# robustrobotics/flame

Hardware: AMD Instinct MI355X
Metric: NLTGV2 primal-dual iters/sec on 640x480 Delaunay graph; depth RMS vs CPU (higher is better)
Workload: dtype f32

## Files before the change

flame_amd/csrc/flame_nltgv2_test_options.h:

```cpp
#ifndef FLAME_NLTGV2_TEST_OPTIONS_H_
#define FLAME_NLTGV2_TEST_OPTIONS_H_

enum {
  FLAME_NLTGV2_OPT_BLOCK_WAVES = 103,
  FLAME_NLTGV2_OPT_UNROLL = 104,
  FLAME_NLTGV2_OPT_DUAL_PUBLISH = 106,
  FLAME_NLTGV2_OPT_PRESLEEP = 108,
  FLAME_NLTGV2_OPT_XCDS = 109,
  FLAME_NLTGV2_OPT_FAULT_INJECT = 110,
  FLAME_NLTGV2_OPT_POLL_GAP = 113
};

#endif
```

flame_amd/csrc/nltgv2_context.hip:

```cpp
#include "nltgv2_context.hpp"

namespace flame_hip {
namespace host {

int fail(flame_nltgv2_ctx* ctx, int status) {
  if (ctx) ctx->last_error = status;
  return status;
}

void request_open_stop(flame_nltgv2_ctx* ctx) {
  if (!ctx->open_inflight || ctx->open_stop_sent || !ctx->stop_dev.p || !ctx->ctl_stream) return;
  *ctx->h_stop = ctx->open_tag0;
  if (hipMemcpyAsync(ctx->stop_dev.p, ctx->h_stop, sizeof(unsigned), hipMemcpyHostToDevice, ctx->ctl_stream) != hipSuccess) (void)hipGetLastError();
  ctx->open_stop_sent = true;
}

hipError_t wait_solver_stream(flame_nltgv2_ctx* ctx) {
  request_open_stop(ctx);
  return hipStreamSynchronize(ctx->stream);
}

int ensure(flame_nltgv2_ctx* ctx, DevBuf& b, size_t bytes) {
  if (bytes == 0) bytes = 16;
  if (b.cap >= bytes) return 0;
// ... 31 lines not shown
  HIPCHK(ctx, hipSetDevice(ctx->device));
  ++ctx->call_seq;
  return 0;
}

void refresh_args(flame_nltgv2_ctx* ctx) {
  CanonArgs& c = ctx->c;
  c.V = ctx->L.V, c.E = ctx->L.E;
  c.pos = (float2*)ctx->pos.p;
  c.x = (float*)ctx->x.p, c.w1 = (float*)ctx->w1.p, c.w2 = (float*)ctx->w2.p;
  c.xb = (float*)ctx->xb.p, c.w1b = (float*)ctx->w1b.p, c.w2b = (float*)ctx->w2b.p;
  c.xp = (float*)ctx->xp.p, c.w1p = (float*)ctx->w1p.p, c.w2p = (float*)ctx->w2p.p;
  c.data = (float*)ctx->data.p, c.weight = (float*)ctx->weight.p;
  c.src = (int32_t*)ctx->src.p, c.dst = (int32_t*)ctx->dst.p;
  c.alpha = (float*)ctx->alpha.p, c.beta = (float*)ctx->beta.p;
  c.q1 = (float*)ctx->q1.p, c.q2 = (float*)ctx->q2.p, c.q3 = (float*)ctx->q3.p;
  c.row_ptr = (int32_t*)ctx->row_ptr.p, c.half = (uint32_t*)ctx->half.p;
  c.err = (int*)ctx->err.p;
  FusedArgs& f = ctx->f;
  f.n_slices = ctx->L.n_slices;
  f.n_slots = (ctx->L.rows + kRowPad) * kWave;
  f.slice_row = (int32_t*)ctx->slice_row.p, f.perm = (int32_t*)ctx->perm.p, f.pdeg = (int32_t*)ctx->pdeg.p;
  f.rec_nbr = (uint32_t*)ctx->rec_nbr.p, f.rec_edge = (int32_t*)ctx->rec_edge.p;
  f.edge_src_slot = (int32_t*)ctx->edge_src_slot.p;
  f.hrec = (int4*)ctx->hrec.p, f.hq = (float4*)ctx->hq.p;
  f.vstate = (float4*)ctx->vstate.p, f.vaux = (float2*)ctx->vaux.p;
  f.hq_out = (float4*)ctx->hq_alt.p, f.vstate_out = (float4*)ctx->vstate_alt.p;
  f.bar[0] = (float4*)ctx->bar0.p, f.bar[1] = (float4*)ctx->bar1.p;
  f.vprev = (float4*)ctx->vprev.p;
  f.xbuf = ctx->xbuf.p;
  f.tv_waves = (ctx->tv_built && ctx->L.tv_ok) ? ctx->L.tv_waves : 0;
  f.tv_slot = (int32_t*)ctx->tv_slot.p, f.tv_vid = (int32_t*)ctx->tv_vid.p;
  f.tv_meta = (uint32_t*)ctx->tv_meta.p, f.tv_wave = (uint32_t*)ctx->tv_wave.p;
  f.wg_count = ctx->L.wg_ok ? ctx->L.wg_count : 0;
  f.n_rec = ctx->L.n_rec;
  f.wg_lcap = ctx->L.wg_lcap, f.wg_slab_slots = ctx->L.wg_slab_slots;
  f.wg_rowpack = ctx->L.wg_rowpack ? 1 : 0;
  f.wg_slot = (int32_t*)ctx->wg_slot.p, f.wg_vid = (int32_t*)ctx->wg_vid.p, f.wg_meta = (uint32_t*)ctx->wg_meta.p;
  f.wg_nbr = (int32_t*)ctx->wg_nbr.p, f.wg_fetch = (int32_t*)ctx->wg_fetch.p, f.wg_info = (int32_t*)ctx->wg_info.p;
  f.abort_flag = (int*)ctx->abort_flag.p;
  f.err = (int*)ctx->err.p;
}

int h2d(flame_nltgv2_ctx* ctx, DevBuf& b, const void* src, size_t bytes) {
  if (bytes == 0) return 0;
  HIPCHK(ctx, hipMemcpyAsync(b.p, src, bytes, hipMemcpyHostToDevice, ctx->stream));
  return 0;
}

size_t records_capacity(const PackedLayout& L) {
  const size_t n_packed = (size_t)L.n_slices * kWave, n_rec = ((size_t)L.n_rec + kWave - 1) / kWave * kWave;
  return std::max(n_packed, n_rec);
}

int wait_raster(flame_nltgv2_ctx* ctx) {
  if (ctx->raster_inflight) {
    HIPCHK(ctx, hipStreamWaitEvent(ctx->stream, ctx->ev_raster_done, 0));
    ctx->raster_inflight = false;
  }
  return 0;
}

int ensure_canon(flame_nltgv2_ctx* ctx, const std::function<int()>* behind, int* behind_state) {
  bool unpacked = false, launched = false;
  if (behind_state) *behind_state = kBehindNotLaunched;
  if (ctx->pending.active) {
    const int rc = finish(ctx, true, &unpacked, behind, &launched);
    if (behind_state && launched) *behind_state = unpacked ? kBehindDone : kBehindSpoiled;
    if (rc) {
      if (unpacked) ctx->canon_valid = true;
      return rc;
    }
  }
  int rc0 = wait_raster(ctx);
  if (rc0) return rc0;
  if (ctx->canon_valid) return 0;
  if (!unpacked) LAUNCHCHK(ctx, launch_unpack_state(ctx->c, ctx->f, ctx->parity, ctx->have_prev, ctx->stream));
  ctx->canon_valid = true;
  return 0;
}

int ensure_fused(flame_nltgv2_ctx* ctx) {
  if (ctx->fused_valid) return 0;
  LAUNCHCHK(ctx, launch_pack_state(ctx->c, ctx->f, ctx->parity, ctx->static_stale, ctx->stream));
  ctx->static_stale = false;
  ctx->fused_valid = true;
  ctx->have_prev = false;
  return 0;
}


int staged_h2d(flame_nltgv2_ctx* ctx, const StageCopy* cp, size_t n, const StageFill* fills, size_t n_fills, int slot, hipStream_t stream,
               size_t* host_off) {
  if (!stream) stream = ctx->stream;
  flame_nltgv2_ctx::StageSlot& st = ctx->stage[slot];
  size_t total = 0;
  for (size_t i = 0; i < n; ++i) total += (cp[i].bytes + 255) & ~size_t(255);
  if (total >= (size_t)0xffffff00u) return fail(ctx, FLAME_NLTGV2_ERR_INVALID_ARG);
  if (total > st.cap) {
    request_open_stop(ctx);
    if (st.h) (void)hipHostFree(st.h);
    st.h = nullptr, st.cap = 0;
    const size_t want = total + total / 2;
    if (hipHostMalloc(&st.h, want, hipHostMallocDefault) != hipSuccess) {
      (void)hipGetLastError();
      return fail(ctx, FLAME_NLTGV2_ERR_OOM);
    }
    st.cap = want;
  }
  int rc = ensure(ctx, st.d, st.cap);
  if (rc) return rc;
  std::vector<ScatterTable> tables(1);
  auto push = [&](const ScatterEntry& e) {
    if (tables.back().n == kScatterMax) tables.emplace_back();
    ScatterTable& t = tables.back();
    t.e[t.n++] = e;
  };
  size_t off = 0;
  for (size_t i = 0; i < n; ++i) {
    if (host_off) host_off[i] = off;
    if (cp[i].bytes == 0) continue;
    std::memcpy(static_cast<char*>(st.h) + off, cp[i].src, cp[i].bytes);
    push(ScatterEntry{cp[i].b->p, (uint32_t)off, 0u, cp[i].bytes});
    off += (cp[i].bytes + 255) & ~size_t(255);
  }
  for (size_t i = 0; i < n_fills; ++i)
    if (fills[i].bytes) push(ScatterEntry{fills[i].dst, kScatterFill, fills[i].word, fills[i].bytes});
  if (off) HIPCHK(ctx, hipMemcpyAsync(st.d.p, st.h, off, hipMemcpyHostToDevice, stream));
  for (const ScatterTable& t : tables) LAUNCHCHK(ctx, launch_scatter(t, st.d.p, stream));
  return 0;
}

int topology_buffers(flame_nltgv2_ctx* ctx, bool want_e2, size_t n_wg_info, size_t n_wg_v0, size_t n_wg_vfirst, size_t n_wg2_info,
                     size_t n_wg2_vfirst) {
  const PackedLayout& L = ctx->L;
  const int32_t V = L.V, E = L.E;
  const size_t n_slots = (size_t)(L.rows + kRowPad) * kWave;
  if (n_slots > (size_t)0x7fffffff) return fail(ctx, FLAME_NLTGV2_ERR_INVALID_ARG);
  const size_t n_packed = (size_t)L.n_slices * kWave;
  const size_t lanes = (size_t)L.wg_count * kWave;
  const size_t fV = sizeof(float) * (size_t)V, fE = sizeof(float) * (size_t)E, iV = sizeof(int32_t) * (size_t)V;
  struct { DevBuf* b; size_t bytes; } req[] = {
      {&ctx->pos, 2 * fV}, {&ctx->src, fE}, {&ctx->dst, fE},
      {&ctx->row_ptr, sizeof(int32_t) * ((size_t)V + 1)}, {&ctx->half, 2 * fE},
      {&ctx->slice_row, sizeof(int32_t) * ((size_t)L.n_slices + 1)}, {&ctx->perm, sizeof(int32_t) * n_packed},
      {&ctx->pdeg, sizeof(int32_t) * n_packed}, {&ctx->iperm, iV}, {&ctx->order_m, iV}, {&ctx->rid_of, iV},
      {&ctx->rec_nbr, sizeof(uint32_t) * n_slots}, {&ctx->rec_edge, sizeof(int32_t) * n_slots}, {&ctx->edge_src_slot, fE},
      {&ctx->hrec, sizeof(int4) * n_slots}, {&ctx->hq, sizeof(float4) * n_slots},
      {&ctx->vstate, sizeof(float4) * n_packed}, {&ctx->vaux, sizeof(float2) * n_packed},
      {&ctx->hq_alt, sizeof(float4) * n_slots}, {&ctx->vstate_alt, sizeof(float4) * n_packed}, {&ctx->photo_err, fV},
      {&ctx->bar0, sizeof(float4) * n_packed}, {&ctx->bar1, sizeof(float4) * n_packed},
      {&ctx->vprev, sizeof(float4) * n_packed}, {&ctx->xbuf, kXbufBytesPerVertex * records_capacity(L) + 64},
      {&ctx->wg_v0, sizeof(int32_t) * n_wg_v0},
      {&ctx->wg_vfirst, n_wg_vfirst + 16}, {&ctx->abort_flag, sizeof(int)}, {&ctx->err, kErrBytes}, {&ctx->cost_out, 2 * sizeof(float)},
      {&ctx->wg_slot, sizeof(int32_t) * lanes}, {&ctx->wg_vid, sizeof(int32_t) * lanes}, {&ctx->wg_meta, sizeof(uint32_t) * lanes},
      {&ctx->wg_nbr, sizeof(int32_t) * lanes}, {&ctx->wg_fetch, sizeof(int32_t) * lanes},
      {&ctx->wg_info, sizeof(int32_t) * n_wg_info}};
  for (auto& r : req) {
    const int rc = ensure(ctx, *r.b, r.bytes);
    if (rc) return rc;
  }
  if (want_e2) {
    const size_t lanes2 = (size_t)L.wg2_count * kWave;
    struct { DevBuf* b; size_t bytes; } req2[] = {
        {&ctx->wg2_info, sizeof(int32_t) * n_wg2_info}, {&ctx->wg2_vfirst, n_wg2_vfirst + 16}, {&ctx->wg2_rmax, 64},
        {&ctx->wg2_slot, sizeof(int32_t) * 2 * lanes2}, {&ctx->wg2_nbr, sizeof(int32_t) * 2 * lanes2}, {&ctx->wg2_vid, sizeof(int32_t) * lanes2},
        {&ctx->wg2_meta, sizeof(uint32_t) * lanes2}, {&ctx->wg2_fetch, sizeof(int32_t) * lanes2}};
    for (auto& r : req2) {
      const int rc = ensure(ctx, *r.b, r.bytes);
      if (rc) return rc;
    }
  }
  ctx->topo++;
  ctx->layout_pos_saved = false;
  ctx->tv_built = ctx->wg2_built = false;
  drop_graphs(ctx);
  refresh_args(ctx);
  return 0;
}

void expansion_fills(const PackedLayout& L, void* rec_edge, void* rec_nbr, void* wg2_rmax, std::vector<StageFill>* fills) {
  fills->push_back(StageFill{(char*)rec_edge + sizeof(int32_t) * (size_t)L.rows * kWave, sizeof(int32_t) * kRowPad * kWave, 0xffffffffu});
  fills->push_back(StageFill{(char*)rec_nbr + sizeof(uint32_t) * (size_t)L.rows * kWave, sizeof(uint32_t) * kRowPad * kWave, 0u});
  if (wg2_rmax) fills->push_back(StageFill{wg2_rmax, 64, 0u});
}

void topology_fills(flame_nltgv2_ctx* ctx, bool want_e2, std::vector<StageFill>* fills, bool early) {
  const PackedLayout& L = ctx->L;
  const size_t n_slots = (size_t)(L.rows + kRowPad) * kWave, n_packed = (size_t)L.n_slices * kWave;
  const StageFill base[] = {
      {ctx->err.p, kErrBytes, 0u}, {ctx->abort_flag.p, sizeof(int), 0u}, {ctx->xbuf.p, kXbufBytesPerVertex * records_capacity(L) + 64, 0u},
      {ctx->hq_alt.p, sizeof(float4) * n_slots, 0u}, {ctx->vstate_alt.p, sizeof(float4) * n_packed, 0u}};
  fills->insert(fills->end(), base, base + sizeof(base) / sizeof(base[0]));
  if (!early) expansion_fills(L, ctx->rec_edge.p, ctx->rec_nbr.p, want_e2 ? ctx->wg2_rmax.p : nullptr, fills);
  if (ctx->place_base) {
    fills->push_back(StageFill{ctx->place_base, (size_t)2 * kPlacePages * 4096, 0u});
    fills->push_back(StageFill{(int*)ctx->place_fill.p + 2 * kPlacePages, 64, 0u});
  }
}

bool placement_applies(const flame_nltgv2_ctx* ctx, const PackedLayout& L) {
  return L.wg_ok && ctx->place_state == 1 && ctx->opt_place && L.wg_count > 2 * (ctx->prop.multiProcessorCount / 8) &&
         (ctx->opt_xcds == 0 || ctx->opt_xcds == 8);
}

ExpandTables live_tables(flame_nltgv2_ctx* ctx) {
  ExpandTables t;
  t.c = ctx->c, t.f = ctx->f;
  t.iperm = (const int32_t*)ctx->iperm.p, t.wg_v0 = (const int32_t*)ctx->wg_v0.p, t.order_m = (const int32_t*)ctx->order_m.p;
  t.rid_of = (const int32_t*)ctx->rid_of.p, t.wg_vfirst = (const uint8_t*)ctx->wg_vfirst.p;
  t.wg2_info = (int32_t*)ctx->wg2_info.p, t.wg2_vfirst = (const uint8_t*)ctx->wg2_vfirst.p;
  t.wg2_slot = (int32_t*)ctx->wg2_slot.p, t.wg2_vid = (int32_t*)ctx->wg2_vid.p, t.wg2_nbr = (int32_t*)ctx->wg2_nbr.p;
  t.wg2_fetch = (int32_t*)ctx->wg2_fetch.p, t.wg2_meta = (uint32_t*)ctx->wg2_meta.p, t.wg2_rmax = (int*)ctx->wg2_rmax.p;
  return t;
}

int expand_launches(flame_nltgv2_ctx* ctx, const PackedLayout& L, const ExpandTables& t, bool want_e2, hipStream_t stream) {
  LAUNCHCHK(ctx, launch_build_sell(t.c, t.f, t.iperm, stream));
  if (L.wg_ok) LAUNCHCHK(ctx, launch_build_patches(t.c, t.f, t.wg_v0, t.order_m, t.rid_of, t.wg_vfirst, t.iperm, stream));
  if (want_e2)
    LAUNCHCHK(ctx, launch_build_patches2(t.c, t.f, L.wg2_count, t.wg2_info, t.order_m, t.rid_of, t.wg2_vfirst, t.iperm, t.wg2_slot, t.wg2_vid,
                                         t.wg2_meta, t.wg2_nbr, t.wg2_fetch, t.wg2_rmax, stream));
  if (t.rec_off)
    LAUNCHCHK(ctx, launch_place_records(t.c, t.f, t.per_xcd, t.order_m, t.rid_of, t.place_patch, (int8_t*)(t.place_patch + t.stride),
                                        (const uint16_t*)ctx->place_rank.p, kPlacePages, t.place_fill, t.rec_off, (int)t.stride, stream));
  return 0;
}

int topology_expand(flame_nltgv2_ctx* ctx, bool want_e2, bool launched) {
  const PackedLayout& L = ctx->L;
  if (!launched) {
    const int rc = expand_launches(ctx, L, live_tables(ctx), want_e2, ctx->stream);
    if (rc) return rc;
  }
  ctx->pv2_args = Pv2Args{};
  ctx->wg2_usable = false;
  if (want_e2) {
    ctx->pv2_args.slot = (const int32_t*)ctx->wg2_slot.p, ctx->pv2_args.vid = (const int32_t*)ctx->wg2_vid.p;
    ctx->pv2_args.meta = (const uint32_t*)ctx->wg2_meta.p, ctx->pv2_args.nbr = (const int32_t*)ctx->wg2_nbr.p;
    ctx->pv2_args.fetch = (const int32_t*)ctx->wg2_fetch.p, ctx->pv2_args.info = (const int32_t*)ctx->wg2_info.p;
    ctx->pv2_args.count = L.wg2_count, ctx->pv2_args.lcap = L.wg2_lcap;
    if (ctx->pv2_occ == 0 || ctx->pv2_occ_lcap != L.wg2_lcap)
      ctx->pv2_occ = pv2_patches_per_cu(L.wg2_lcap, false), ctx->pv2_occ_verify = pv2_patches_per_cu(L.wg2_lcap, true), ctx->pv2_occ_lcap = L.wg2_lcap;
    ctx->wg2_built = true;
  }
  if (!launched && placement_applies(ctx, L)) {
    refresh_args(ctx);
    const int rc = place_records(ctx, (L.wg_count + 7) / 8);
    if (rc) return rc;
  }
  ctx->pending = flame_nltgv2_ctx::PendingRun{};
  ctx->tag_next = 1;
  ctx->xbuf_form = 0;
  ctx->static_stale = false;
  return 0;
}

bool wants_e2(const flame_nltgv2_ctx* ctx) { return wants_e2(ctx, ctx->L); }
bool wants_e2(const flame_nltgv2_ctx* ctx, const PackedLayout& L) {
  const int cus = ctx->prop.multiProcessorCount;
  const int64_t est_patches = L.wg_rowpack ? (int64_t)L.wg_count : ((static_cast<int64_t>(2) * L.E + L.V / 32) / 54 + 1);
  return L.wg_ok && L.max_degree <= 32 && ctx->opt_probe == 0 &&
         (ctx->opt_persistent == 6 || (ctx->opt_persistent == 1 && est_patches > (int64_t)kPv2FromPerCu * cus));
}

int upload_topology(flame_nltgv2_ctx* ctx, const flame_nltgv2_graph* g, const StageCopy* extra, size_t n_extra, bool long_lived) {
  const int32_t V = g->V, E = g->E;
  (void)long_lived;
  int rc = cancel_prepared(ctx);
  if (!rc) rc = wait_raster(ctx);
  if (rc) return rc;
  rc = build_layout(g, &ctx->L, false, true,
                        ctx->opt_persistent == 4 ? 0x7fffffff : kPvDensePerCu * ctx->prop.multiProcessorCount);
  if (rc) return fail(ctx, rc);
  if (ctx->L.wg_ok && ctx->L.wg_rowpack && ctx->opt_persistent != 4 && ctx->L.wg_count > kPvDensePerCu * ctx->prop.multiProcessorCount) {
    rc = build_layout(g, &ctx->L, false, false, 0);
    if (rc) return fail(ctx, rc);
  }
  bool want_e2 = wants_e2(ctx);
  if (want_e2) {
    build_patch_walk2(&ctx->L);
    want_e2 = ctx->L.wg2_ok && ctx->L.wg2_count <= kPv2WavesPerCu * ctx->prop.multiProcessorCount * 4;
  }
  const PackedLayout& L = ctx->L;
  rc = topology_buffers(ctx, want_e2, L.wg_info.size(), L.wg_v0.size(), L.wg_vfirst.size(), L.wg2_info.size(), L.wg2_vfirst.size());
  if (rc) return rc;
  const size_t n_packed = (size_t)L.n_slices * kWave;
  const size_t fV = sizeof(float) * (size_t)V, fE = sizeof(float) * (size_t)E, iV = sizeof(int32_t) * (size_t)V;
  std::vector<StageCopy> cp = {
      {&ctx->pos, g->pos, 2 * fV}, {&ctx->src, g->src, fE}, {&ctx->dst, g->dst, fE},
      {&ctx->row_ptr, L.row_ptr.data(), sizeof(int32_t) * ((size_t)V + 1)}, {&ctx->half, L.half.data(), 2 * fE},
      {&ctx->slice_row, L.slice_row.data(), sizeof(int32_t) * ((size_t)L.n_slices + 1)},
      {&ctx->perm, L.perm.data(), sizeof(int32_t) * n_packed}, {&ctx->pdeg, L.pdeg.data(), sizeof(int32_t) * n_packed},
      {&ctx->iperm, L.iperm.data(), iV}, {&ctx->order_m, L.order_m.data(), iV}, {&ctx->rid_of, L.rid_of.data(), iV},
      {&ctx->wg_info, L.wg_info.data(), sizeof(int32_t) * L.wg_info.size()},
      {&ctx->wg_v0, L.wg_v0.data(), sizeof(int32_t) * L.wg_v0.size()},
      {&ctx->wg_vfirst, L.wg_vfirst.data(), L.wg_vfirst.size()}};
  if (want_e2) {
    cp.push_back(StageCopy{&ctx->wg2_info, L.wg2_info.data(), sizeof(int32_t) * L.wg2_info.size()});
    cp.push_back(StageCopy{&ctx->wg2_vfirst, L.wg2_vfirst.data(), L.wg2_vfirst.size()});
  }
  cp.insert(cp.end(), extra, extra + n_extra);
  std::vector<StageFill> fills;
  topology_fills(ctx, want_e2, &fills);
  rc = staged_h2d(ctx, cp.data(), cp.size(), fills.data(), fills.size());
  if (rc) return rc;
  rc = topology_expand(ctx, want_e2);
  if (rc) return rc;
  ctx->h_src.assign(g->src, g->src + E);
  ctx->h_dst.assign(g->dst, g->dst + E);
  ctx->host_layout_valid = true;
  ctx->feat_dev_valid = false;
  HIPCHK(ctx, hipEventRecord(ctx->ev_topo_ready, ctx->stream));
  return 0;
}

int ensure_form_rows(flame_nltgv2_ctx* ctx, int form) {
  PackedLayout& L = ctx->L;
  if ((form == 4 && !ctx->wg2_built) || (form == 2 && !ctx->tv_built)) {
    const int rc = ensure_host_layout(ctx);
    if (rc) return rc;
  }
  if (form == 4 && !ctx->wg2_built) {
    build_patch_rows2(&L);
    ctx->pv2_args = Pv2Args{};
    if (L.wg2_ok) {
      struct { DevBuf* b; const void* src; size_t bytes; } cp[] = {
          {&ctx->wg2_slot, L.wg2_slot.data(), sizeof(int32_t) * L.wg2_slot.size()}, {&ctx->wg2_vid, L.wg2_vid.data(), sizeof(int32_t) * L.wg2_vid.size()},
          {&ctx->wg2_meta, L.wg2_meta.data(), sizeof(uint32_t) * L.wg2_meta.size()}, {&ctx->wg2_nbr, L.wg2_nbr.data(), sizeof(int32_t) * L.wg2_nbr.size()},
          {&ctx->wg2_fetch, L.wg2_fetch.data(), sizeof(int32_t) * L.wg2_fetch.size()}, {&ctx->wg2_info, L.wg2_info.data(), sizeof(int32_t) * L.wg2_info.size()}};
      HIPCHK(ctx, wait_solver_stream(ctx));
      for (auto& c : cp) {
        int rc = ensure(ctx, *c.b, c.bytes);
        if (!rc) rc = h2d(ctx, *c.b, c.src, c.bytes);
        if (rc) return rc;
      }
      HIPCHK(ctx, wait_solver_stream(ctx));
      ctx->pv2_args.slot = (const int32_t*)ctx->wg2_slot.p, ctx->pv2_args.vid = (const int32_t*)ctx->wg2_vid.p, ctx->pv2_args.meta = (const uint32_t*)ctx->wg2_meta.p;
      ctx->pv2_args.nbr = (const int32_t*)ctx->wg2_nbr.p, ctx->pv2_args.fetch = (const int32_t*)ctx->wg2_fetch.p, ctx->pv2_args.info = (const int32_t*)ctx->wg2_info.p;
      ctx->pv2_args.count = L.wg2_count, ctx->pv2_args.lcap = L.wg2_lcap;
      ctx->pv2_occ = pv2_patches_per_cu(L.wg2_lcap, false), ctx->pv2_occ_verify = pv2_patches_per_cu(L.wg2_lcap, true), ctx->pv2_occ_lcap = L.wg2_lcap;
    }
    ctx->wg2_built = true;
    ctx->wg2_usable = L.wg2_ok, ctx->wg2_checked_topo = ctx->topo;
  }
  if (form == 2 && !ctx->tv_built) {
    build_tv_rows(&L);
    struct { DevBuf* b; const void* src; size_t bytes; } cp[] = {
        {&ctx->tv_slot, L.tv_slot.data(), sizeof(int32_t) * L.tv_slot.size()}, {&ctx->tv_vid, L.tv_vid.data(), sizeof(int32_t) * L.tv_vid.size()},
        {&ctx->tv_meta, L.tv_meta.data(), sizeof(uint32_t) * L.tv_meta.size()}, {&ctx->tv_wave, L.tv_wave.data(), sizeof(uint32_t) * L.tv_wave.size()}};
    HIPCHK(ctx, wait_solver_stream(ctx));
    for (auto& c : cp) {
      int rc = ensure(ctx, *c.b, c.bytes);
      if (!rc) rc = h2d(ctx, *c.b, c.src, c.bytes);
      if (rc) return rc;
    }
    HIPCHK(ctx, wait_solver_stream(ctx));
    ctx->tv_built = true;
    refresh_args(ctx);
  }
  return 0;
}

bool params_ok(const flame_nltgv2_params* p) { return p != nullptr; }

}
}

extern "C" {

int flame_nltgv2_abi_version(void) { return FLAME_NLTGV2_ABI_VERSION; }

void flame_nltgv2_default_params(flame_nltgv2_params* p) {
  if (!p) return;
  p->data_factor = 0.1f, p->step_x = 0.001f, p->step_q = 125.0f;
  p->theta = 0.25f, p->x_min = 0.0f, p->x_max = 10.0f;
}

const char* flame_nltgv2_status_string(int status) {
  switch (status) {
    case FLAME_NLTGV2_OK: return "ok";
    case FLAME_NLTGV2_ERR_INVALID_ARG: return "invalid argument";
    case FLAME_NLTGV2_ERR_NO_DEVICE: return "no usable HIP device";
    case FLAME_NLTGV2_ERR_HIP: return "HIP runtime error";
    case FLAME_NLTGV2_ERR_NO_GRAPH: return "no graph uploaded";
    case FLAME_NLTGV2_ERR_NAN: return "dual variable became NaN/Inf (reference FLAME_ASSERT, h:174)";
    case FLAME_NLTGV2_ERR_OOM: return "out of device memory";
    case FLAME_NLTGV2_ERR_TIMEOUT: return "persistent run: neighbour wait timed out";
    case FLAME_NLTGV2_ERR_ASSERT: return "input on which the reference asserts (FLAME_ASSERT)";
    default: return "unknown status";
  }
}

int flame_nltgv2_create(flame_nltgv2_ctx** out, int device) {
  if (!out) return FLAME_NLTGV2_ERR_INVALID_ARG;
  *out = nullptr;
  int count = 0;
  if (hipGetDeviceCount(&count) != hipSuccess || count <= 0) return FLAME_NLTGV2_ERR_NO_DEVICE;
  if (device < 0 || device >= count) return FLAME_NLTGV2_ERR_NO_DEVICE;
  flame_nltgv2_ctx* ctx = new (std::nothrow) flame_nltgv2_ctx();
  if (!ctx) return FLAME_NLTGV2_ERR_OOM;
  ctx->device = device;
  bool ok = hipSetDevice(device) == hipSuccess;
  ok = ok && hipGetDeviceProperties(&ctx->prop, device) == hipSuccess;
  int prio_least = 0, prio_greatest = 0;
  ok = ok && hipDeviceGetStreamPriorityRange(&prio_least, &prio_greatest) == hipSuccess;
  ok = ok && hipStreamCreateWithPriority(&ctx->own_stream, hipStreamNonBlocking, prio_greatest) == hipSuccess;
  ok = ok && hipEventCreate(&ctx->ev0) == hipSuccess && hipEventCreate(&ctx->ev1) == hipSuccess;
  ok = ok && hipStreamCreateWithFlags(&ctx->topo_stream, hipStreamNonBlocking) == hipSuccess;
  ok = ok && hipStreamCreateWithFlags(&ctx->raster_stream, hipStreamNonBlocking) == hipSuccess;
  ok = ok && hipEventCreateWithFlags(&ctx->ev_canon, hipEventDisableTiming) == hipSuccess;
  ok = ok && hipEventCreateWithFlags(&ctx->ev_snap, hipEventDisableTiming) == hipSuccess;
  ok = ok && hipEventCreateWithFlags(&ctx->ev_raster_done, hipEventDisableTiming) == hipSuccess;
  ok = ok && hipEventCreateWithFlags(&ctx->ev_topo_ready, hipEventDisableTiming) == hipSuccess;
  ok = ok && hipEventCreate(&ctx->ev_mesh0) == hipSuccess && hipEventCreate(&ctx->ev_mesh1) == hipSuccess;
  ok = ok && hipEventCreate(&ctx->ev_dbg0) == hipSuccess && hipEventCreate(&ctx->ev_dbg1) == hipSuccess;
  ok = ok && hipEventCreateWithFlags(&ctx->ev_expanded, hipEventDisableTiming) == hipSuccess;
  ok = ok && hipEventCreateWithFlags(&ctx->ev_run[0], hipEventDisableTiming) == hipSuccess;
  ok = ok && hipEventCreateWithFlags(&ctx->ev_run[1], hipEventDisableTiming) == hipSuccess;
  ok = ok && hipHostMalloc((void**)&ctx->h_err, kErrBytes, hipHostMallocDefault) == hipSuccess;
  ok = ok && hipHostMalloc((void**)&ctx->h_cost, 2 * sizeof(float), hipHostMallocDefault) == hipSuccess;
  ok = ok && hipHostMalloc((void**)&ctx->h_stop, 64, hipHostMallocDefault) == hipSuccess;
  if (ctx->h_stop) *ctx->h_stop = 0u;
  ok = ok && hipStreamCreateWithPriority(&ctx->ctl_stream, hipStreamNonBlocking, -1) == hipSuccess;
  if (!ok) {
    flame_nltgv2_destroy(ctx);
    return FLAME_NLTGV2_ERR_HIP;
  }
  ctx->stream = ctx->own_stream;
  *ctx->h_err = 0;
  {
    static std::once_flag warm;
    if (!std::getenv("FLAME_NLTGV2_NO_WARM"))
    std::call_once(warm, [ctx] {
      warm_module_kernels(), warm_module_persistent(ctx->own_stream, cooperative_allowed()), warm_module_persistent_tv(), warm_module_persistent_pv2();
      warm_module_layout(), warm_module_topo();
    });
    if (!std::getenv("FLAME_NLTGV2_LAZY_CALIBRATION") && ctx->prop.multiProcessorCount >= 64 && place_calibrate_at_create(device) && place_calibrate(ctx) != 0) {
      ctx->last_error = 0, ctx->last_hip = 0;
      (void)hipGetLastError();
    }
    if (ctx->place_state < 0) ctx->place_state = 0;
  }
  ctx->all = {&ctx->pos, &ctx->x, &ctx->w1, &ctx->w2, &ctx->xb, &ctx->w1b, &ctx->w2b, &ctx->xp, &ctx->w1p,
              &ctx->w2p, &ctx->data, &ctx->weight, &ctx->src, &ctx->dst, &ctx->alpha, &ctx->beta, &ctx->q1,
              &ctx->q2, &ctx->q3, &ctx->row_ptr, &ctx->half, &ctx->slice_row, &ctx->perm, &ctx->pdeg,
              &ctx->rec_nbr, &ctx->rec_edge, &ctx->edge_src_slot, &ctx->hrec, &ctx->hq, &ctx->vstate, &ctx->hq_alt, &ctx->vstate_alt, &ctx->cost_terms, &ctx->run_tail,
              &ctx->vaux, &ctx->bar0, &ctx->bar1, &ctx->vprev, &ctx->xbuf, &ctx->abort_flag, &ctx->tv_slot, &ctx->tv_vid, &ctx->tv_meta, &ctx->tv_wave, &ctx->wg2_slot, &ctx->wg2_vid, &ctx->wg2_meta, &ctx->wg2_nbr, &ctx->wg2_fetch, &ctx->wg2_info, &ctx->wg2_vfirst, &ctx->wg2_rmax, &ctx->err,
              &ctx->cost_out, &ctx->img_ref, &ctx->img_cmp, &ctx->photo_err, &ctx->r_tris, &ctx->r_valid, &ctx->r_tvalid, &ctx->r_keys,
              &ctx->r_img, &ctx->r_cov, &ctx->r_vtx, &ctx->r_val, &ctx->wg_slot, &ctx->wg_vid, &ctx->wg_meta, &ctx->wg_nbr,
              &ctx->wg_fetch, &ctx->wg_info, &ctx->wg_v0, &ctx->probe, &ctx->snap_hq, &ctx->snap_vstate, &ctx->snap_bar, &ctx->iperm,
              &ctx->order_m, &ctx->rid_of, &ctx->stage[0].d, &ctx->stage[1].d, &ctx->sync_init, &ctx->sync_vmap, &ctx->sync_emap, &ctx->sync_need,
              &ctx->wg_vfirst, &ctx->place_pool, &ctx->place_rank, &ctx->place_fill, &ctx->place_rec_off, &ctx->place_patch, &ctx->place_meas, &ctx->progress};
  for (DevBuf* b : {&ctx->feat_stamp_d, &ctx->feat_key_d, &ctx->feat_val_d, &ctx->topo_scratch, &ctx->topo_dims, &ctx->layout_pos}) ctx->all.push_back(b);
  for (auto& b : ctx->nx) ctx->all.push_back(&b);
  for (auto& b : ctx->ex) ctx->all.push_back(&b);
  ctx->all.push_back(&ctx->pos_undo);
  for (DevBuf* b : {&ctx->m_P, &ctx->m_idepth, &ctx->m_normals, &ctx->m_tvalid, &ctx->m_nvalid, &ctx->m_tnormal, &ctx->m_offset, &ctx->m_cursor,
                    &ctx->m_incident, &ctx->m_keys, &ctx->m_img, &ctx->m_cov})
    ctx->all.push_back(b);
  for (DevBuf* b : {&ctx->d_gray, &ctx->d_idimg, &ctx->d_nimg, &ctx->d_w1map, &ctx->d_w2map, &ctx->d_keys, &ctx->d_cov}) ctx->all.push_back(b);
  ctx->all.push_back(&ctx->stop_dev);
  ctx->all.push_back(&ctx->place_patch_nx), ctx->all.push_back(&ctx->place_fill_nx);
  for (auto& b : ctx->sp_v) ctx->all.push_back(&b);
  for (auto& b : ctx->sp_q) ctx->all.push_back(&b);
  for (auto& b : ctx->sp_ab) ctx->all.push_back(&b);
  *out = ctx;
  return FLAME_NLTGV2_OK;
}

int flame_nltgv2_destroy(flame_nltgv2_ctx* ctx) {
  if (!ctx) return FLAME_NLTGV2_OK;
  (void)hipSetDevice(ctx->device);
  request_open_stop(ctx);
  if (ctx->stream) (void)hipStreamSynchronize(ctx->stream);
  place_pool_release(ctx);
  drop_graphs(ctx);
  for (DevBuf* b : ctx->all)
    if (b->p) (void)hipFree(b->p);
  if (ctx->h_err) (void)hipHostFree(ctx->h_err);
  if (ctx->h_cost) (void)hipHostFree(ctx->h_cost);
  if (ctx->h_keep) (void)hipHostFree(ctx->h_keep);
  if (ctx->h_stop) (void)hipHostFree(ctx->h_stop);
  if (ctx->ctl_stream) (void)hipStreamSynchronize(ctx->ctl_stream), (void)hipStreamDestroy(ctx->ctl_stream);
  for (auto& st : ctx->stage)
    if (st.h) (void)hipHostFree(st.h);
  if (ctx->topo_stream) (void)hipStreamSynchronize(ctx->topo_stream), (void)hipStreamDestroy(ctx->topo_stream);
  if (ctx->ev_topo_ready) (void)hipEventDestroy(ctx->ev_topo_ready);
  if (ctx->ev_expanded) (void)hipEventDestroy(ctx->ev_expanded);
  if (ctx->raster_stream) (void)hipStreamSynchronize(ctx->raster_stream), (void)hipStreamDestroy(ctx->raster_stream);
  if (ctx->ev_canon) (void)hipEventDestroy(ctx->ev_canon);
  if (ctx->ev_snap) (void)hipEventDestroy(ctx->ev_snap);
  if (ctx->ev_raster_done) (void)hipEventDestroy(ctx->ev_raster_done);
  for (hipEvent_t e : ctx->ev_run)
    if (e) (void)hipEventDestroy(e);
  if (ctx->h_img) (void)hipHostFree(ctx->h_img);
  if (ctx->h_mesh) (void)hipHostFree(ctx->h_mesh);
  if (ctx->ev_mesh0) (void)hipEventDestroy(ctx->ev_mesh0);
  if (ctx->ev_mesh1) (void)hipEventDestroy(ctx->ev_mesh1);
  if (ctx->h_dbg) (void)hipHostFree(ctx->h_dbg);
  if (ctx->ev_dbg0) (void)hipEventDestroy(ctx->ev_dbg0);
  if (ctx->ev_dbg1) (void)hipEventDestroy(ctx->ev_dbg1);
  if (ctx->h_dims) (void)hipHostFree(ctx->h_dims);
  if (ctx->ev0) (void)hipEventDestroy(ctx->ev0);
  if (ctx->ev1) (void)hipEventDestroy(ctx->ev1);
  if (ctx->own_stream) (void)hipStreamDestroy(ctx->own_stream);
  delete ctx;
  return FLAME_NLTGV2_OK;
}

int flame_nltgv2_set_stream(flame_nltgv2_ctx* ctx, void* hip_stream) {
  int rc = enter(ctx);
  if (rc) return rc;
  HIPCHK(ctx, wait_solver_stream(ctx));
  ctx->stream = hip_stream ? (hipStream_t)hip_stream : ctx->own_stream;
  return FLAME_NLTGV2_OK;
}

int flame_nltgv2_set_option(flame_nltgv2_ctx* ctx, int option, int value) {
  if (!ctx) return FLAME_NLTGV2_ERR_INVALID_ARG;
  switch (option) {
    case FLAME_NLTGV2_OPT_SOLVER:
      if (value != 0 && value != 1) return fail(ctx, FLAME_NLTGV2_ERR_INVALID_ARG);
      ctx->opt_solver = value;
      return 0;
    case FLAME_NLTGV2_OPT_USE_HIPGRAPH:
      ctx->opt_use_graph = value ? 1 : 0;
      return 0;
    case FLAME_NLTGV2_OPT_BLOCK_WAVES:
      if (value != 0 && value != 1 && value != 2 && value != 4) return fail(ctx, FLAME_NLTGV2_ERR_INVALID_ARG);
      ctx->opt_block_waves = value;
      return 0;
    case FLAME_NLTGV2_OPT_PERSISTENT:
      if (value < 0 || value > 6 || value == 2 || value == 5) return fail(ctx, FLAME_NLTGV2_ERR_INVALID_ARG);
      ctx->opt_persistent = value;
      return 0;
    case FLAME_NLTGV2_OPT_PLACEMENT:
      if (value < 0 || value > 1) return fail(ctx, FLAME_NLTGV2_ERR_INVALID_ARG);
      ctx->opt_place = value;
      return 0;
    case FLAME_NLTGV2_OPT_POLL_GAP:
      if (value < 0 || value > 256) return fail(ctx, FLAME_NLTGV2_ERR_INVALID_ARG);
      ctx->opt_poll_gap = value;
      return 0;
    case FLAME_NLTGV2_OPT_VERIFY_RECORDS:
      if (value < 0 || value > 2) return fail(ctx, FLAME_NLTGV2_ERR_INVALID_ARG);
      ctx->opt_verify = value;
      if (value != 2) ctx->persist_refused_topo = ctx->persist_backoff_topo = ~0ull;
      return 0;
    case FLAME_NLTGV2_OPT_PROBE:
      ctx->opt_probe = value ? 1 : 0;
      return 0;
    case FLAME_NLTGV2_OPT_DUAL_PUBLISH:
      if (value < 0 || value > 2) return fail(ctx, FLAME_NLTGV2_ERR_INVALID_ARG);
      ctx->opt_dual = value;
      return 0;
    case FLAME_NLTGV2_OPT_FAULT_INJECT:
      if (value < 0 || value > (1 << 24)) return fail(ctx, FLAME_NLTGV2_ERR_INVALID_ARG);
      ctx->opt_fault = value;
      if (value == 0) ctx->persist_refused_topo = ctx->persist_backoff_topo = ~0ull;
      return 0;
    case FLAME_NLTGV2_OPT_XCDS:
      if (value < 0 || value > 8) return fail(ctx, FLAME_NLTGV2_ERR_INVALID_ARG);
      ctx->opt_xcds = value;
      ctx->coop_checked_key = ~0ull;
      return 0;
    case FLAME_NLTGV2_OPT_PRESLEEP:
      if (value < 0 || value > 256) return fail(ctx, FLAME_NLTGV2_ERR_INVALID_ARG);
      ctx->opt_presleep = value;
      return 0;
    case FLAME_NLTGV2_OPT_MESH_STATE:
      if (value < 0 || value > 1) return fail(ctx, FLAME_NLTGV2_ERR_INVALID_ARG);
      ctx->opt_mesh_state = value;
      return 0;
    case FLAME_NLTGV2_OPT_COST_SUM:
      if (value < 0 || value > 1) return fail(ctx, FLAME_NLTGV2_ERR_INVALID_ARG);
      ctx->opt_cost_sum = value;
      return 0;
    case FLAME_NLTGV2_OPT_SYNC_PATH:
      if (value < 0 || value > 2) return fail(ctx, FLAME_NLTGV2_ERR_INVALID_ARG);
      ctx->opt_sync_path = value;
      return 0;
    case FLAME_NLTGV2_OPT_UNROLL:
      if (value != 0 && value != 4 && value != 8 && value != 16) return fail(ctx, FLAME_NLTGV2_ERR_INVALID_ARG);
      ctx->opt_unroll = value;
      return 0;
    default:
      return fail(ctx, FLAME_NLTGV2_ERR_INVALID_ARG);
  }
}


int flame_nltgv2_get_info(flame_nltgv2_ctx* ctx, flame_nltgv2_info* info) {
  if (!ctx || !info) return FLAME_NLTGV2_ERR_INVALID_ARG;
  std::memset(info, 0, sizeof(*info));
  info->abi_version = FLAME_NLTGV2_ABI_VERSION;
  info->device = ctx->device;
  info->V = ctx->L.V, info->E = ctx->L.E;
  info->n_slices = ctx->L.n_slices;
  info->max_degree = ctx->L.max_degree;
  info->padded_half_edges = ctx->L.rows * kWave;
  info->device_bytes = (int64_t)ctx->device_bytes;
  info->algorithmic_bytes_per_iter = 64ll * ctx->L.V + 40ll * ctx->L.E;
  info->compute_units = ctx->prop.multiProcessorCount;
  std::snprintf(info->device_name, sizeof(info->device_name), "%s", ctx->prop.name);
  std::snprintf(info->gcn_arch, sizeof(info->gcn_arch), "%s", ctx->prop.gcnArchName);
  info->last_run_path = ctx->last_run_path;
  info->he_waves = 0;
  if (ctx->have_graph && !ctx->tv_built && ctx->tv_counted_topo != ctx->topo) {
    if (ensure_host_layout(ctx) == 0) {
      ctx->L.tv_waves = 0;
      build_tv_rows(&ctx->L);
      ctx->tv_counted_topo = ctx->topo;
    }
  }
  info->tv_waves = ctx->L.tv_ok ? ctx->L.tv_waves : 0;
  info->patches = ctx->L.wg_ok ? ctx->L.wg_count : 0;
  info->tv_wave_capacity = kTvLdsWavesPerCu * ctx->prop.multiProcessorCount;
  info->last_run_groups = ctx->last_run_groups;
  info->timeouts_recovered = ctx->timeouts_recovered;
  info->torn_records_detected = ctx->torn_records_detected;
  info->last_sync_path = ctx->last_sync_path;
  info->last_run_waves_per_cu = ctx->last_run_waves_per_cu;
  info->reserved0 = 0, info->reserved1 = 0;
  info->replays_per_step = ctx->replays_per_step;
  return FLAME_NLTGV2_OK;
}

int flame_nltgv2_last_error(flame_nltgv2_ctx* ctx) { return ctx ? ctx->last_error : FLAME_NLTGV2_ERR_INVALID_ARG; }
int flame_nltgv2_last_hip_error(flame_nltgv2_ctx* ctx) { return ctx ? ctx->last_hip : 0; }

int flame_nltgv2_read_probe(flame_nltgv2_ctx* ctx, uint32_t* out, int64_t max_words, int64_t* n_words) {
  int rc = enter(ctx);
  if (rc) return rc;
  if (ctx->pending.active) {
    rc = finish(ctx);
    if (rc) return rc;
  }
  HIPCHK(ctx, wait_solver_stream(ctx));
  const int64_t have = (int64_t)ctx->probe_words;
  if (n_words) *n_words = have;
  if (out && ctx->probe.p) {
    const int64_t n = std::min(have, max_words);
    if (n > 0) HIPCHK(ctx, hipMemcpy(out, ctx->probe.p, sizeof(uint32_t) * (size_t)n, hipMemcpyDeviceToHost));
  }
  return FLAME_NLTGV2_OK;
}

int flame_nltgv2_layout_selftest(flame_nltgv2_ctx* ctx, int64_t* mismatches) {
  int rc = enter(ctx);
  if (rc) return rc;
  if (!ctx->have_graph) return fail(ctx, FLAME_NLTGV2_ERR_NO_GRAPH);
  if (!mismatches) return fail(ctx, FLAME_NLTGV2_ERR_INVALID_ARG);
  rc = ensure_canon(ctx);
  if (!rc) rc = ensure_host_layout(ctx);
  if (rc) return rc;
  const int32_t V = ctx->L.V, E = ctx->L.E;
  std::vector<float> pos(2 * (size_t)V);
  HIPCHK(ctx, hipMemcpyAsync(pos.data(), ctx->layout_pos_saved ? ctx->layout_pos.p : ctx->pos.p, sizeof(float) * pos.size(), hipMemcpyDeviceToHost, ctx->stream));
  HIPCHK(ctx, wait_solver_stream(ctx));
  flame_nltgv2_graph g{};
  g.V = V, g.E = E, g.pos = pos.data(), g.src = ctx->h_src.data(), g.dst = ctx->h_dst.data();
  PackedLayout H;
  rc = build_layout(&g, &H, true, ctx->L.wg_rowpack);
  if (rc) return fail(ctx, rc);
  int64_t bad = 0;
  auto cmp = [&](const DevBuf& b, const void* host, size_t bytes) -> int {
    if (bytes == 0) return 0;
    std::vector<uint32_t> d(bytes / 4);
    if (hipMemcpy(d.data(), b.p, bytes, hipMemcpyDeviceToHost) != hipSuccess) return 1;
    const uint32_t* h = static_cast<const uint32_t*>(host);
    for (size_t i = 0; i < d.size(); ++i) bad += d[i] != h[i];
    return 0;
  };
  const PackedLayout& L = ctx->L;
  bad += (H.rows != L.rows) + (H.n_slices != L.n_slices) + (H.wg_ok != L.wg_ok) + (H.wg_count != L.wg_count) +
         (H.wg_lcap != L.wg_lcap) + (H.wg_slab_slots != L.wg_slab_slots) + (H.n_rec != L.n_rec) +
         (H.wg_v0 != L.wg_v0) + (H.wg_vfirst != L.wg_vfirst) + (H.wg_rowpack != L.wg_rowpack);
  if (bad == 0) {
    const size_t iV = 4 * (size_t)V;
    int e = cmp(ctx->row_ptr, H.row_ptr.data(), iV + 4) | cmp(ctx->half, H.half.data(), 8 * (size_t)E) | cmp(ctx->order_m, H.order_m.data(), iV) |
            cmp(ctx->rid_of, H.rid_of.data(), iV) | cmp(ctx->iperm, H.iperm.data(), iV) | cmp(ctx->pdeg, H.pdeg.data(), 4 * H.pdeg.size()) |
            cmp(ctx->wg_v0, H.wg_v0.data(), 4 * H.wg_v0.size()) | cmp(ctx->wg_vfirst, H.wg_vfirst.data(), H.wg_vfirst.size() & ~size_t(3));
    if (e) return fail(ctx, FLAME_NLTGV2_ERR_HIP);
    std::vector<int32_t> hs(ctx->h_src.size()), hd(ctx->h_dst.size());
    if (E && (hipMemcpy(hs.data(), ctx->src.p, 4 * (size_t)E, hipMemcpyDeviceToHost) != hipSuccess ||
              hipMemcpy(hd.data(), ctx->dst.p, 4 * (size_t)E, hipMemcpyDeviceToHost) != hipSuccess))
      return fail(ctx, FLAME_NLTGV2_ERR_HIP);
    bad += (hs != ctx->h_src) + (hd != ctx->h_dst);
  }
  if (bad == 0) {
    const size_t n = (size_t)L.rows * kWave, lanes = (size_t)L.wg_count * kWave;
    int e = cmp(ctx->rec_nbr, H.rec_nbr.data(), 4 * n) | cmp(ctx->rec_edge, H.rec_edge.data(), 4 * n) |
            cmp(ctx->edge_src_slot, H.edge_src_slot.data(), 4 * (size_t)E) | cmp(ctx->perm, H.perm.data(), 4 * H.perm.size()) |
            cmp(ctx->slice_row, H.slice_row.data(), 4 * H.slice_row.size());
    if (L.wg_ok)
      e |= cmp(ctx->wg_slot, H.wg_slot.data(), 4 * lanes) | cmp(ctx->wg_vid, H.wg_vid.data(), 4 * lanes) |
           cmp(ctx->wg_meta, H.wg_meta.data(), 4 * lanes) | cmp(ctx->wg_nbr, H.wg_nbr.data(), 4 * lanes) |
           cmp(ctx->wg_fetch, H.wg_fetch.data(), 4 * lanes) | cmp(ctx->wg_info, H.wg_info.data(), 4 * H.wg_info.size());
    if (ctx->wg2_built) {
      build_patch_rows2(&H);
      bad += (H.wg2_ok != L.wg2_ok) + (H.wg2_count != L.wg2_count) + (H.wg2_lcap != L.wg2_lcap) + (H.wg2_vfirst != L.wg2_vfirst);
      if (bad == 0 && H.wg2_ok) {
        const size_t lanes2 = (size_t)H.wg2_count * kWave;
        e |= cmp(ctx->wg2_slot, H.wg2_slot.data(), 8 * lanes2) | cmp(ctx->wg2_nbr, H.wg2_nbr.data(), 8 * lanes2) |
             cmp(ctx->wg2_vid, H.wg2_vid.data(), 4 * lanes2) | cmp(ctx->wg2_meta, H.wg2_meta.data(), 4 * lanes2) |
             cmp(ctx->wg2_fetch, H.wg2_fetch.data(), 4 * lanes2) | cmp(ctx->wg2_info, H.wg2_info.data(), 4 * H.wg2_info.size());
      }
    }
    if (e) return fail(ctx, FLAME_NLTGV2_ERR_HIP);
  }
  if (bad == 0 && ctx->place_state == 1 && ctx->place_topo == ctx->topo && L.wg_ok) {
    const size_t stride = records_capacity(L);
    std::vector<int32_t> off(2 * stride);
    if (hipMemcpy(off.data(), ctx->place_rec_off.p, sizeof(int32_t) * off.size(), hipMemcpyDeviceToHost) != hipSuccess)
      return fail(ctx, FLAME_NLTGV2_ERR_HIP);
    std::vector<int32_t> patch_of_rec((size_t)V, -1);
    for (int32_t q = 0; q < H.wg_count; ++q)
      for (int32_t i = 0; i < (H.wg_info[(size_t)q * 4 + 2] & 0xffff); ++i) patch_of_rec[(size_t)H.wg_info[(size_t)q * 4] + i] = q;
    const int32_t per = ctx->place_per_xcd;
    for (int par = 0; par < 2; ++par) {
      std::vector<int32_t> used;
      for (int32_t u = 0; u < V; ++u) {
        const int32_t r = H.rid_of[(size_t)u], a = patch_of_rec[(size_t)r] / per;
        bool crosses = false;
        for (int32_t h = H.row_ptr[(size_t)u]; h < H.row_ptr[(size_t)u + 1] && !crosses; ++h)
          crosses = patch_of_rec[(size_t)H.rid_of[(size_t)H.half_nbr[(size_t)h]]] / per != a;
        const int32_t o = off[(size_t)par * stride + r];
        bad += crosses != (o >= 0);
        if (o < 0) continue;
        bad += (o & 15) != 0 || o < par * kPlacePages * 4096 || o >= (par + 1) * kPlacePages * 4096;
        used.push_back(o);
      }
      std::sort(used.begin(), used.end());
      for (size_t i = 1; i < used.size(); ++i) bad += used[i] == used[i - 1];
    }
  }
  *mismatches = bad;
  return FLAME_NLTGV2_OK;
}

int flame_nltgv2_placement_info(flame_nltgv2_ctx* ctx, int32_t* state, int32_t* placed_records, float* us) {
  int rc = enter(ctx);
  if (rc) return rc;
  if (state) *state = ctx->place_state;
  if (us) us[0] = ctx->place_best_us, us[1] = ctx->place_mean_us, us[2] = ctx->place_worst_us;
  if (placed_records) {
    *placed_records = 0;
    if (ctx->have_graph && ctx->place_state == 1 && ctx->place_topo == ctx->topo) {
      std::vector<int32_t> off((size_t)ctx->L.V);
      HIPCHK(ctx, hipMemcpyAsync(off.data(), ctx->place_rec_off.p, sizeof(int32_t) * off.size(), hipMemcpyDeviceToHost, ctx->stream));
      HIPCHK(ctx, wait_solver_stream(ctx));
      for (int32_t o : off) *placed_records += o >= 0;
    }
  }
  return FLAME_NLTGV2_OK;
}

int flame_nltgv2_pack_probe(const flame_nltgv2_graph* g, int32_t* perm, int32_t* slice_row, int32_t* rec_nbr,
                            int32_t* rec_edge, int64_t capacity_rows, int64_t* rows_out) {
  PackedLayout L;
  int rc = build_layout(g, &L);
  if (rc) return rc;
  if (rows_out) *rows_out = L.rows;
  if (perm) std::memcpy(perm, L.perm.data(), sizeof(int32_t) * L.perm.size());
  if (slice_row) std::memcpy(slice_row, L.slice_row.data(), sizeof(int32_t) * L.slice_row.size());
  if ((rec_nbr || rec_edge) && capacity_rows < L.rows) return FLAME_NLTGV2_ERR_INVALID_ARG;
  const size_t n = (size_t)L.rows * kWave;
  if (rec_nbr) std::memcpy(rec_nbr, L.rec_nbr.data(), sizeof(int32_t) * n);
  if (rec_edge) std::memcpy(rec_edge, L.rec_edge.data(), sizeof(int32_t) * n);
  return L.n_slices;
}

}
```

flame_amd/csrc/nltgv2_context.hpp:

```cpp
#ifndef FLAME_AMD_NLTGV2_CONTEXT_HPP_
#define FLAME_AMD_NLTGV2_CONTEXT_HPP_

#include <hip/hip_runtime.h>

#include <cstdio>
#include <cstdlib>
#include <cstring>
#include <algorithm>
#include <chrono>
#include <cmath>
#include <new>
#include <memory>
#include <mutex>
#include <functional>
#include <vector>

#include "flame_nltgv2.h"
#include "flame_nltgv2_test_options.h"
#include "nltgv2_kernels.h"
#include "nltgv2_pack.hpp"
#include "roctx_ranges.hpp"

namespace flame_hip {
namespace host {

constexpr int kGraphChunk = 256;
constexpr int kMaxCachedGraphs = 6;
constexpr int kTvLdsWavesPerCu = 16;
constexpr size_t kXbufBytesPerVertex = 8 * 16 + 4;
constexpr int kPv2FromPerCu = 14;
constexpr int kPv2PaceAbovePerCu = 10, kPv2DensePreSleep = 2, kPv2DenseGap = 2;
constexpr int kPv2MaxGroups = 2;
constexpr int kPv2WavesPerCu = 19;
constexpr int kCrowdedWavesPerCu = 16, kCrowdedTopologies = 64;
constexpr int kPvDensePerCu = 27;
constexpr int kPvPaceAbovePerCu = 13;
constexpr int kPvDensePreSleep = 3, kPvDenseGap = 2;
constexpr int kPvPaceMoreAbovePerCu = 23;
constexpr int kPvDenserPreSleep = 5, kPvDenserGap = 4;
constexpr int kPvPreSleep = 0;
constexpr int kPvPollGap = 2;
constexpr int kDualMinWavesPerCu = 0;
constexpr int kPreSleepTv = 2;
constexpr int32_t kFeatDirectMax = 1 << 22;
constexpr size_t kErrBytes = 16 * sizeof(int);
constexpr unsigned kMaxSpins = 1u << 20;

struct DevBuf {
  void* p = nullptr;
  size_t cap = 0;
};

struct CachedGraph {
  hipGraphExec_t exec = nullptr;
  int n = 0, parity = 0, unroll = 0, wpb = 0, gen = 0;
  uint64_t topo = 0;
  flame_nltgv2_params params{};
  uint64_t stamp = 0;
};

class FlatMap {
 public:
  FlatMap() = default;
  explicit FlatMap(size_t n) { reset(n); }
  void reset(size_t n) {
    size_t cap = 16;
    while (cap < 2 * n + 2) cap <<= 1;
    if (cap > slots_.size() || gen_ == 0xffffffffu) {
      slots_.assign(std::max(cap, slots_.size()), Slot{0, 0, 0});
      gen_ = 0;
    }
    mask_ = slots_.size() - 1;
    ++gen_;
  }
  std::pair<int32_t*, bool> emplace(uint64_t k, int32_t v) {
    size_t i = hash(k) & mask_;
    for (;; i = (i + 1) & mask_) {
      Slot& s = slots_[i];
      if (s.gen != gen_) {
        s = Slot{k, v, gen_};
        return {&s.val, true};
      }
      if (s.key == k) return {&s.val, false};
    }
  }
  const int32_t* find(uint64_t k) const {
    size_t i = hash(k) & mask_;
    for (;; i = (i + 1) & mask_) {
      const Slot& s = slots_[i];
      if (s.gen != gen_) return nullptr;
      if (s.key == k) return &s.val;
    }
  }

 private:
  struct Slot {
    uint64_t key;
    int32_t val;
    uint32_t gen;
  };
  static size_t hash(uint64_t z) {
    z = (z ^ (z >> 30)) * 0xbf58476d1ce4e5b9ull;
    z = (z ^ (z >> 27)) * 0x94d049bb133111ebull;
    return (size_t)(z ^ (z >> 31));
  }
  size_t mask_ = 0;
  uint32_t gen_ = 0;
  std::vector<Slot> slots_;
};

}
}

using namespace flame_hip;
using namespace flame_hip::host;

struct flame_nltgv2_ctx {
  int device = 0;
  hipStream_t own_stream = nullptr;
  hipStream_t stream = nullptr;
  hipEvent_t ev0 = nullptr, ev1 = nullptr;
  int last_error = 0;
  int last_hip = 0;
  hipDeviceProp_t prop{};

  bool have_graph = false;
  bool canon_valid = false, fused_valid = false, have_prev = false;
  DevBuf sp_v[9], sp_q[3], sync_init, sync_vmap, sync_emap, sync_need;
  DevBuf sp_ab[2];
  std::vector<int32_t> h_old_of_new, h_old_of_new_edge, h_old_edge_of_pair, h_first_pair_of_old, h_bucket_start, h_bucket_item, h_bucket_at;
  FlatMap feat_maps[3];
  int feat_cur = 0;
  bool feat_map_valid = false;
  std::vector<int32_t> feat_tab;
  std::vector<uint32_t> feat_stamp;
  uint32_t feat_stamp_now = 0;
  bool feat_tab_valid = false;
  int parity = 0;
  uint64_t topo = 0, stamp = 0;

  int opt_solver = 0, opt_use_graph = 1, opt_block_waves = 0, opt_unroll = 0, opt_persistent = 1, opt_dual = 1;
  int xbuf_form = 0;
  int opt_xcds = 0;
  bool photo_fused = false;
  PhotoGeometry photo_geo{};
  float photo_scale = 1.0f;
  int photo_border = 3;
  bool photo_fresh = false;
  float* export_ptr = nullptr;
  float export_scale = 1.0f;
  int opt_fault = 0;
  int opt_presleep = 0;
  int opt_poll_gap = 0;
  mutable int pv_occ = 0;
  mutable uint64_t pv_occ_topo = ~0ull;
  int opt_probe = 0;
  size_t probe_words = 0;
  uint32_t tag_next = 1;
  int last_run_path = 0, last_run_groups = 0;
  uint64_t persist_refused_topo = ~0ull;
  uint64_t persist_backoff_topo = ~0ull;
  int persist_backoff_left = 0, persist_timeout_streak = 0;
  int replaying = 0;
  uint64_t crowded_until_topo = 0;
  int last_run_waves_per_cu = 0;
  bool static_stale = false;
  uint64_t coop_checked_key = 0;
  int buf_gen = 0;
  int replay_attempt = 0;
  int replays_per_step = 0;
  int timeouts_recovered = 0;
  int torn_records_detected = 0;
  int opt_verify = 0;
  int opt_place = 1;
  int place_state = 0;
  uint64_t place_topo = ~0ull;
  int place_per_xcd = 0;
  char* place_base = nullptr;
  float place_best_us = 0.0f, place_mean_us = 0.0f, place_worst_us = 0.0f;
  DevBuf place_pool, place_rank, place_fill, place_rec_off, place_patch, place_meas;
  std::vector<uint16_t> place_rank_host;
  struct PendingOp {
    int kind = 0;
    flame_nltgv2_params params{};
    int n = 0;
    bool open = false;
    uint32_t tag0 = 0;
    float* dst = nullptr;
    float scale = 1.0f;
  };
  struct PendingRun {
    bool active = false;
    bool snapshotted = false;
    int parity_before = 0;
    bool have_prev_before = false;
    std::vector<PendingOp> ops;
  } pending;
  DevBuf snap_hq, snap_vstate, snap_bar;
  DevBuf iperm, order_m, rid_of;
  bool tv_built = false;
  bool wg2_built = false;
  Pv2Args pv2_args;
  int pv2_occ_lcap = -1;
  int pv2_occ = 0, pv2_occ_verify = 0;
  uint64_t wg2_checked_topo = ~0ull;
  bool wg2_usable = false;
  struct StageSlot {
    void* h = nullptr;
    size_t cap = 0;
    DevBuf d;
  } stage[2];

  PackedLayout L;
  std::vector<int32_t> h_src, h_dst, h_feat;
  DevBuf layout_pos;
  bool layout_pos_saved = false;
  bool host_layout_valid = true;
  uint64_t tv_counted_topo = ~0ull;
  int opt_mesh_state = 0;
  uint64_t snap_topo = ~0ull;
  hipEvent_t ev_snap = nullptr;
  int opt_cost_sum = 0;
  int opt_sync_path = 0;
  int last_sync_path = 0;
  DevBuf feat_stamp_d, feat_key_d, feat_val_d, topo_scratch, topo_dims;
  std::vector<int32_t> dup_key;
  std::vector<uint32_t> dup_stamp;
  uint32_t dup_now = 0;
  enum { NX_POS, NX_SRC, NX_DST, NX_ROW_PTR, NX_HALF, NX_ORDER_M, NX_RID_OF, NX_PERM, NX_IPERM, NX_PDEG, NX_SLICE_ROW, NX_WG_INFO, NX_WG_V0,
         NX_WG_VFIRST, NX_WG2_INFO, NX_WG2_VFIRST, NX_DATA, NX_WEIGHT, NX_COUNT };
  DevBuf nx[NX_COUNT];
  DevBuf* nx_live(int i) {
    DevBuf* const live[NX_COUNT] = {&pos, &src, &dst, &row_ptr, &half, &order_m, &rid_of, &perm, &iperm, &pdeg, &slice_row, &wg_info, &wg_v0,
                                    &wg_vfirst, &wg2_info, &wg2_vfirst, &data, &weight};
    return live[i];
  }
  enum { EX_REC_NBR, EX_REC_EDGE, EX_EDGE_SRC_SLOT, EX_WG_SLOT, EX_WG_VID, EX_WG_META, EX_WG_NBR, EX_WG_FETCH, EX_WG2_SLOT, EX_WG2_NBR,
         EX_WG2_VID, EX_WG2_META, EX_WG2_FETCH, EX_WG2_RMAX, EX_PLACE_REC_OFF, EX_COUNT };
  DevBuf ex[EX_COUNT];
  DevBuf* ex_live(int i) {
    DevBuf* const live[EX_COUNT] = {&rec_nbr, &rec_edge, &edge_src_slot, &wg_slot, &wg_vid, &wg_meta, &wg_nbr, &wg_fetch, &wg2_slot, &wg2_nbr,
                                    &wg2_vid, &wg2_meta, &wg2_fetch, &wg2_rmax, &place_rec_off};
    return live[i];
  }
  DevBuf place_patch_nx, place_fill_nx;
  hipEvent_t ev_expanded = nullptr;
  std::vector<char> prep_host;
  const void *prep_vmap = nullptr, *prep_emap = nullptr, *prep_init = nullptr;
  hipStream_t raster_stream = nullptr;
  hipEvent_t ev_canon = nullptr, ev_raster_done = nullptr;
  bool raster_inflight = false;
  float* h_img = nullptr;
  size_t h_img_cap = 0;
  int map_rows = 0, map_cols = 0;
  int img_pending_rows = 0, img_pending_cols = 0;
  int32_t tris_T = -1;
  uint64_t tris_topo = ~0ull;
  DevBuf m_P, m_idepth, m_normals, m_tvalid, m_nvalid, m_tnormal, m_offset, m_cursor, m_incident, m_keys, m_img, m_cov;
  char* h_mesh = nullptr;
  size_t h_mesh_cap = 0;
  struct MeshPending {
    bool active = false;
    int32_t V = 0, T = 0;
    int rows = 0, cols = 0;
    size_t off_idepth = 0, off_counts = 0, off_map = 0, off_valid = 0;
  } mesh_pending;
  hipEvent_t ev_mesh0 = nullptr, ev_mesh1 = nullptr;
  uint64_t tris_gen = 0, keys_gen = 0;
  DevBuf d_gray, d_idimg, d_nimg, d_w1map, d_w2map, d_keys, d_cov;
  char* h_dbg = nullptr;
  size_t h_dbg_cap = 0;
  struct DebugPending {
    bool active = false;
    int rows = 0, cols = 0;
    bool want_idepth = false, want_normals = false;
    size_t off_nimg = 0, off_w1 = 0, off_w2 = 0, off_gray = 0;
  } debug_pending;
  hipEvent_t ev_dbg0 = nullptr, ev_dbg1 = nullptr;
  hipStream_t topo_stream = nullptr;
  hipEvent_t ev_topo_ready = nullptr;
  struct PreparedSync {
    bool active = false, device = false;
    uint64_t topo = 0;
    int32_t V = 0, E = 0;
    bool has_init = false;
    int32_t check_sticky = 0, edges_unique = 0, init_from_map = 0;
    float sticky_threshold = 0.0f, init_graph_scale = 0.0f;
    size_t off[6] = {};
    std::chrono::steady_clock::time_point t_begin, t_enqueued;
  } prepared;
  int feat_tab_bits_d = 0;
  uint32_t feat_gen = 0;
  bool feat_dev_valid = false;
  TopoDims* h_dims = nullptr;
  CanonArgs c;
  FusedArgs f;
  std::vector<DevBuf*> all;
  DevBuf pos, x, w1, w2, xb, w1b, w2b, xp, w1p, w2p, data, weight, src, dst, alpha, beta, q1, q2, q3, row_ptr, half;
  DevBuf slice_row, perm, pdeg, rec_nbr, rec_edge, edge_src_slot, hrec, hq, vstate, vaux, bar0, bar1, vprev;
  DevBuf cost_terms;
  static constexpr int kTailSlots = 4;
  DevBuf run_tail;
  RunTail tail_sent[kTailSlots]{};
  bool tail_valid[kTailSlots] = {false, false, false, false};
  int tail_next = 0;
  hipEvent_t ev_run[2] = {nullptr, nullptr};
  int run_ev_pick = -1, run_ev_last = 0;
  bool run_ev_valid[2] = {false, false};
  bool track_runs = false;
  bool run_event_bound = false;
  uint64_t call_seq = 0, run_event_seq = 0;
  std::vector<float> h_terms;
  DevBuf hq_alt, vstate_alt;
  DevBuf xbuf, abort_flag, tv_slot, tv_vid, tv_meta, tv_wave, wg2_slot, wg2_vid, wg2_meta, wg2_nbr, wg2_fetch, wg2_info, wg2_vfirst, wg2_rmax;
  DevBuf wg_slot, wg_vid, wg_meta, wg_nbr, wg_fetch, wg_info, wg_v0, wg_vfirst, probe, progress;
  DevBuf err, cost_out, img_ref, img_cmp, photo_err, r_tris, r_valid, r_tvalid, r_keys, r_img, r_cov, r_vtx, r_val;
  int img_rows = 0, img_cols = 0, img_step = 0;
  int* h_err = nullptr;
  int last_expired[16] = {0};
  float* h_cost = nullptr;
  uint8_t* h_keep = nullptr;
  unsigned* h_stop = nullptr;
  DevBuf stop_dev;
  hipStream_t ctl_stream = nullptr;
  bool open_inflight = false;
  bool open_stop_sent = false;
  uint32_t open_tag0 = 0;
// ... 119 lines not shown
```

flame_amd/csrc/nltgv2_kernels.h:

```cpp
#pragma once

#include <hip/hip_runtime.h>
#include <hip/hip_ext.h>
#include <stdint.h>

namespace flame_hip {

struct SolverParams {
  float data_factor, step_x, step_q, theta, x_min, x_max;
};

struct PhotoGeometry {
  float KRKinv[9];
  float Kt[3];
};

struct PhotoFuse {
  const float2* pos = nullptr;
  const uint8_t* ref = nullptr;
  const uint8_t* cmp = nullptr;
  float* err = nullptr;
  PhotoGeometry geo{};
  float graph_scale = 1.0f;
  int rows = 0, cols = 0, step = 0, border = 0;
};

struct RunTail {
  float* export_out = nullptr;
  float export_scale = 1.0f;
  int reserved_ = 0;
  PhotoFuse photo;
  unsigned* progress = nullptr;
  const unsigned* stop_req = nullptr;
};

struct ProjectGeometry {
  float K[9], Kinv[9], KRKinv[9];
  float q[4];
  float t[3];
  float rx, ry, rw, rh;
};

struct CanonArgs {
  int V = 0, E = 0;
  float2* pos = nullptr;
  float *x = nullptr, *w1 = nullptr, *w2 = nullptr;
  float *xb = nullptr, *w1b = nullptr, *w2b = nullptr;
  float *xp = nullptr, *w1p = nullptr, *w2p = nullptr;
  float *data = nullptr, *weight = nullptr;
  int32_t *src = nullptr, *dst = nullptr;
  float *alpha = nullptr, *beta = nullptr;
  float *q1 = nullptr, *q2 = nullptr, *q3 = nullptr;
  int32_t* row_ptr = nullptr;
  uint32_t* half = nullptr;
  int* err = nullptr;
};

struct FusedArgs {
  hipEvent_t stop_event = nullptr;
  int open_run = 0;
  int n_slices = 0;
  int64_t n_slots = 0;
  int32_t* slice_row = nullptr;
  int32_t* perm = nullptr;
  int32_t* pdeg = nullptr;
  uint32_t* rec_nbr = nullptr;
  int32_t* rec_edge = nullptr;
  int32_t* edge_src_slot = nullptr;
  int4* hrec = nullptr;
  float4* hq = nullptr;
  float4* vstate = nullptr;
  float4* hq_out = nullptr;
  float4* vstate_out = nullptr;
  float2* vaux = nullptr;
  float4* bar[2] = {nullptr, nullptr};
  float4* vprev = nullptr;
  void* xbuf = nullptr;
  int tv_waves = 0;
  int32_t* tv_slot = nullptr;
  int32_t* tv_vid = nullptr;
  uint32_t* tv_meta = nullptr;
  uint32_t* tv_wave = nullptr;
  int wg_count = 0, wg_lcap = 0, wg_slab_slots = 0;
  int wg_rowpack = 0;
  int32_t* wg_slot = nullptr;
  int32_t* wg_vid = nullptr;
  uint32_t* wg_meta = nullptr;
  int32_t* wg_nbr = nullptr;
  int32_t* wg_fetch = nullptr;
  int32_t* wg_info = nullptr;
  int n_rec = 0;
  int wg_poll_gap = 1;
  char* place_pool = nullptr;
  const int32_t* rec_off = nullptr;
  int rec_off_stride = 0;
  unsigned* rot_word = nullptr;
  unsigned* probe = nullptr;
  int* abort_flag = nullptr;
  int* err = nullptr;
};
inline int persistent_rec_bytes(const FusedArgs& a) { return (a.n_rec > a.n_slices * 64 ? a.n_rec : a.n_slices * 64) * 16; }

int launch_fused_step(const FusedArgs& a, const SolverParams& p, int parity, bool write_prev, int unroll,
                      int waves_per_block, hipStream_t stream);
int launch_persistent_run(const FusedArgs& a, const SolverParams& p, int form, int wave_begin, int n_waves,
                          int parity_in, unsigned tag0, int n_iters, int waves_per_block, unsigned max_spins,
                          int presleep, int dual, int xcds, const RunTail* tail, bool cooperative,
                          hipStream_t stream);
constexpr int kPlacePages = 96;
int launch_place_calibrate(char* pool, int n_pages, int iters, unsigned* out, int* xcc_out, int* fail, hipStream_t s);
int launch_place_records(const CanonArgs& c, const FusedArgs& a, int per_xcd, const int32_t* order_m, const int32_t* rid_of,
                         int32_t* patch_of_rec, int8_t* cls, const uint16_t* ranking, int n_pages, int* fill, int32_t* rec_off,
                         int stride, hipStream_t s);
constexpr uint32_t kScatterFill = 0xffffffffu;
struct ScatterEntry {
  void* dst;
  uint32_t src_off;
  uint32_t fill;
  size_t bytes;
};
constexpr int kScatterMax = 48;
struct ScatterTable {
  int n = 0;
  ScatterEntry e[kScatterMax];
};
int launch_scatter(const ScatterTable& t, const void* blob, hipStream_t s);
struct CopyTable {
  int n = 0;
  struct { void* dst; const void* src; size_t bytes; } e[4];
};
int launch_copy_arrays(const CopyTable& t, hipStream_t s);
struct SyncArgs {
  int V = 0, E = 0;
  const int32_t* old_of_new = nullptr;
  const int32_t* old_of_new_edge = nullptr;
  const float* data = nullptr;
  const float* weight = nullptr;
  const float* init_x = nullptr;
  const float* init_map = nullptr;
  int map_rows = 0, map_cols = 0;
  int check_sticky = 0;
  float sticky_threshold = 0.0f;
  float graph_scale = 0.0f;
  const float* o[9] = {};
  float* n[9] = {};
  const float* oq[3] = {};
  float* nq[3] = {};
  const int32_t *src = nullptr, *dst = nullptr, *row_ptr = nullptr;
  const uint32_t* half = nullptr;
  const float2* pos = nullptr;
  float *alpha = nullptr, *beta = nullptr;
  uint8_t* need_nbr = nullptr;
};
int launch_sync_state(const SyncArgs& a, hipStream_t s);
int pv_patches_per_cu(const FusedArgs& a, bool verify);
struct Pv2Args {
  const int32_t* slot = nullptr;
  const int32_t* vid = nullptr;
  const uint32_t* meta = nullptr;
  const int32_t* nbr = nullptr;
  const int32_t* fetch = nullptr;
  const int32_t* info = nullptr;
  int count = 0, lcap = 0;
};
int launch_build_patches2(const CanonArgs& c, const FusedArgs& a, int n_patches, int32_t* wg_info, const int32_t* order_m, const int32_t* rid_tab,
                          const uint8_t* vfirst, const int32_t* iperm, int32_t* wg_slot, int32_t* wg_vid, uint32_t* wg_meta, int32_t* wg_nbr,
                          int32_t* wg_fetch, int* rmax, hipStream_t s);
int pv2_patches_per_cu(int lcap, bool verify);
int launch_persistent_pv2(const FusedArgs& a, const Pv2Args& w, const SolverParams& p, int wg_begin, int n_wgs, int parity_in, unsigned tag0,
                          int n_iters, unsigned max_spins, int poll_gap, int dual, const RunTail* tail, bool cooperative, hipStream_t stream);
int pv_real_waves_per_simd(bool verify_or_probe);
const void* persistent_tv_kernel(int waves_per_block, unsigned* lds_bytes);
int launch_build_sell(const CanonArgs& c, const FusedArgs& a, const int32_t* iperm, hipStream_t s);
int launch_build_patches(const CanonArgs& c, const FusedArgs& a, const int32_t* wg_v0, const int32_t* order_m,
                         const int32_t* rid_tab, const uint8_t* vfirst, const int32_t* iperm, hipStream_t s);
struct TopoDims {
  int32_t n_edges;
  int32_t n_keep;
  int32_t rows;
  int32_t max_degree;
  int32_t wg_count, wg_lcap;
  int32_t wg2_count, wg2_lcap;
  int32_t flags;
  int32_t pad_[7];
};
constexpr int32_t kTopoBadDegree = 1;
constexpr int32_t kTopoBadEdges = 2;
constexpr int kTopoInf = 0x7f7f7f7f;
struct TopoBuild {
  int V = 0, E = 0;
  int Vo = 0, Eo = 0;
  int n_slices = 0;
  const int32_t* fid = nullptr;
  const float2* pos = nullptr;
  const int32_t* tri_edges = nullptr;
  float minx = 0, miny = 0, sx = 0, sy = 0;
  const int32_t* o_row_ptr = nullptr;
  const uint32_t* o_half = nullptr;
  const int32_t *o_src = nullptr, *o_dst = nullptr;
  uint32_t* feat_stamp = nullptr;
  int32_t* feat_key = nullptr;
  int32_t* feat_val = nullptr;
  int tab_bits = 0;
  uint32_t gen_prev = 0, gen_new = 0;
  int32_t *old_edge = nullptr, *first_k = nullptr;
  int32_t* scan = nullptr;
  int32_t *deg = nullptr, *cur = nullptr;
  int cc_bits = 1;
  int32_t *parent = nullptr, *minid = nullptr;
  uint32_t* morton = nullptr;
  uint64_t* key_out = nullptr;
  int32_t* width = nullptr;
  uint8_t* wflag = nullptr;
  uint8_t* vf[2] = {nullptr, nullptr};
  int32_t* seg_count[2] = {nullptr, nullptr};
  void* sort_tmp = nullptr;
  size_t sort_tmp_bytes = 0;
  int* counters = nullptr;
  int32_t* old_of_new = nullptr;
  int32_t* old_of_new_edge = nullptr;
  int32_t *src = nullptr, *dst = nullptr;
  int32_t* row_ptr = nullptr;
  uint32_t* half = nullptr;
  int32_t *order_m = nullptr, *rid_of = nullptr, *perm = nullptr, *iperm = nullptr, *pdeg = nullptr, *slice_row = nullptr;
  int32_t *wg_info = nullptr, *wg_v0 = nullptr, *wg2_info = nullptr, *wg2_v0 = nullptr;
  uint8_t *wg_vfirst = nullptr, *wg2_vfirst = nullptr;
  TopoDims* dims = nullptr;
};
size_t topo_sort_temp_bytes(int V, int n_scan);
int launch_topo_feat_build(const int32_t* feat, int V, uint32_t* stamp, int32_t* key, int32_t* val, int tab_bits, uint32_t gen, hipStream_t s);
int launch_topo_sync_front(const TopoBuild& t, hipStream_t s);
int launch_topo_upload_front(const TopoBuild& t, hipStream_t s);
int launch_topo_back(const TopoBuild& t, hipStream_t s);

void warm_module_kernels();
void warm_module_persistent(hipStream_t stream, bool cooperative);
void warm_module_persistent_tv();
void warm_module_persistent_pv2();
void warm_module_layout();
void warm_module_topo();

int launch_save_prev(const CanonArgs& c, hipStream_t s);
int launch_dual(const CanonArgs& c, const SolverParams& p, hipStream_t s);
int launch_primal(const CanonArgs& c, const SolverParams& p, hipStream_t s);
int launch_extragradient(const CanonArgs& c, const SolverParams& p, hipStream_t s);
int launch_pack_static(const CanonArgs& c, const FusedArgs& a, hipStream_t s);
int launch_pack_state(const CanonArgs& c, const FusedArgs& a, int parity, bool with_static, hipStream_t s);
int launch_unpack_state(const CanonArgs& c, const FusedArgs& a, int parity, bool have_prev, hipStream_t s);
int launch_export(const CanonArgs& c, const FusedArgs& a, bool packed_current, float scale, float* dst,
                  hipStream_t s);
// ... 13 lines not shown
```

flame_amd/csrc/nltgv2_persistent.hip:

```cpp
#include "nltgv2_persistent_common.hpp"

namespace flame_hip {

namespace {


template <bool PROBE, bool VERIFY, bool OPEN = false>
__global__ void __launch_bounds__(64) __attribute__((amdgpu_num_sgpr(92)))
k_persistent_pv(const int wg_begin, const int n_wgs, const int wgs_per_xcd, const int lcap, const int slab_slots,
                const int32_t* __restrict__ wg_slot, const int32_t* __restrict__ wg_vid,
                const uint32_t* __restrict__ wg_meta, const int32_t* __restrict__ wg_nbr,
                const int32_t* __restrict__ wg_fetch, const int32_t* __restrict__ wg_info, const int4* hrec,
                const float4* hq, const float4* vstate,
                float4* hq_out, float4* vstate_out, const float2* vaux, const float4* bar_in, float4* bar_out, float4* vprev,
                void* xbuf, const int rec_bytes, const int dual_arg, const unsigned tag0, const int n_iters,
                const unsigned max_spins_arg, const int poll_gap_arg, const SolverParams p,
                int* __restrict__ err, int* __restrict__ abort_flag, const int32_t* __restrict__ perm,
                const RunTail* __restrict__ tail, unsigned* __restrict__ probe, char* place_pool,
                const int32_t* __restrict__ rec_off, const int rec_off_stride, unsigned* rot_word) {
  extern __shared__ float4 lds[];
  constexpr int T = 64;
  const unsigned max_spins = max_spins_arg & 0x7fffffffu;
  const int dual = dual_arg & 1, verify = VERIFY ? dual_arg >> 1 : 0;
  const int poll_gap = poll_gap_arg & 255, pv_presleep = (poll_gap_arg >> 8) & 255;
  const int lane = (int)threadIdx.x;
  int b = blockIdx.x;
  if (rot_word) {
    const unsigned want = (tag0 & 0x0fffffffu) << 4;
    if (b == 0 && lane == 0) __hip_atomic_store(rot_word, want | read_xcc_id(), __ATOMIC_RELAXED, __HIP_MEMORY_SCOPE_AGENT);
    unsigned v = 0;
    for (unsigned spins = 0;; ++spins) {
      v = __builtin_amdgcn_readfirstlane(__hip_atomic_load(rot_word, __ATOMIC_RELAXED, __HIP_MEMORY_SCOPE_AGENT));
      if ((v & ~15u) == want) break;
      if (spins > (max_spins_arg & 0x7fffffffu)) {
        if (lane == 0) {
          give_up(abort_flag, err, false);
          report_expired(err, 1, (int)blockIdx.x, -1, 0ull, -1, v, want);
        }
        return;
      }
      __builtin_amdgcn_s_sleep(2);
    }
    b += (int)(v & 7u);
    if (b >= (int)gridDim.x) b -= (int)gridDim.x;
  }
  const int xcd = b & 7, idx = b >> 3;
  if (idx >= wgs_per_xcd) return;
  if (xcd * wgs_per_xcd + idx >= n_wgs) return;
  const int wg = wg_begin + xcd * wgs_per_xcd + idx;
  const int rid_base = wg_info[4 * wg], n_fetch = wg_info[4 * wg + 1];
  const int count_flags = wg_info[4 * wg + 2];
  if ((count_flags & 0xffff) == 0) return;
  if (unsigned* const pg = tail->progress) {
    if (lane == 0) pg[n_wgs + (wg - wg_begin)] = (unsigned)(wall_clock64() / 100u) | 1u;
  }
  const int stride = wg_info[4 * wg + 3];
  const int rec_stride = lcap + T;
  const int o_ovfA = 2 * rec_stride + slab_slots;
  const __amdgpu_buffer_rsrc_t rx = make_rsrc(xbuf);

  constexpr int kPar = 2;
  const int S = rec_bytes, par = 2 * rec_bytes, tab_off = kPar * par;
  const unsigned xcc_want = (tag0 & 0x0fffffffu) << 4;
  const unsigned p0 = tag0 & 1u;

  const size_t hl = (size_t)wg * T + lane;
  const unsigned meta = wg_meta[hl];
  const int slot = wg_slot[hl];
  const int pv = wg_vid[hl];
  const int nbr_code = wg_nbr[hl];
  const int frid = (lane < n_fetch) ? wg_fetch[hl] : -1;
  const int loc = (int)((meta >> 13) & 2047u);
  const bool active = (meta & kWgActiveBit) != 0u;
  const bool valid = (meta & kWgValidBit) != 0u, publishes = (meta & kWgPublishBit) != 0u;
  const bool state_lane = (meta & kWgHeadBit) != 0u;
  const unsigned degx = (meta & kWgHeadBit) ? ((meta >> 6) & 127u) : (active ? 255u : 0u);
  const unsigned long long rm1 = __ballot(degx > 1u), rm2 = __ballot(degx > 2u), rm3 = __ballot(degx > 3u), rm4 = __ballot(degx > 4u),
                           rm5 = __ballot(degx > 5u), rm6 = __ballot(degx > 6u), rm7 = __ballot(degx > 7u), rm8 = __ballot(degx > 8u);
  const int nbr_idx = active ? ((nbr_code < 0) ? lcap + (nbr_code & 0x7fffffff) : nbr_code) : (valid ? loc : 0);

  int4 rec = make_int4(0, 0, 0, 0);
  float4 q = make_float4(0.f, 0.f, 0.f, 0.f);
  if (active) {
    rec = hrec[slot];
    q = hq[slot];
  }
  const bool is_target = rec.x < 0;
  const float alpha = __int_as_float(rec.y), dx = __int_as_float(rec.z), dy = __int_as_float(rec.w);
  const float beta = q.w;
  float q1 = q.x;
  v2f_t q23 = {q.y, q.z};
  const float as = is_target ? -alpha : alpha, bs = is_target ? -beta : beta, ac = is_target ? alpha : -alpha;
  const v2f_t P12 = {alpha * dx, alpha * dy};
  const v2f_t C2 = !active ? v2f_t{0.0f, 0.0f} : is_target ? v2f_t{beta, beta} : v2f_t{-dx, -dy};
  const float nbeta = -beta;

  float4 st = make_float4(0.f, 0.f, 0.f, 0.f), bs4 = make_float4(0.f, 0.f, 0.f, 0.f);
  float2 aux = make_float2(0.f, 0.f);
  if (valid) {
    st = vstate[pv];
    aux = vaux[pv];
    bs4 = bar_in[pv];
  }
  const float data = st.w;
  const float thr = p.step_x * (p.data_factor * aux.x);
  float x = st.x;
  v2f_t w12 = {st.y, st.z};
  float xb = bs4.x;
  v2f_t wb12 = {bs4.y, bs4.z};
  float x_prev = x;
  v2f_t w_prev = w12;
  bool ok = true;
  bool timed_out = n_fetch > T;
  bool torn = false;

  const int my_off = (rid_base + loc) << 4;
  const int rec_w = valid ? loc : o_ovfA + lane, rec_wstride = valid ? rec_stride : 0;

  lds[lcap + lane] = make_float4(0.f, 0.f, 0.f, 0.f);
  lds[rec_stride + lcap + lane] = make_float4(0.f, 0.f, 0.f, 0.f);

  int off0 = (frid >= 0) ? (frid << 4) : 0;
  bool fetch_remote = frid >= 0;
  if (dual) {
    const unsigned my_xcc = read_xcc_id();
    if (state_lane && publishes)
      __builtin_amdgcn_raw_buffer_store_b32((int)(xcc_want | my_xcc), rx, tab_off + (my_off >> 2), 0, kAuxSc1);
    if (n_fetch > 0 && !timed_out) {
      bool pend = frid >= 0;
      unsigned g0 = 0, spins = 0;
      for (;;) {
        if (pend) {
          int o = tab_off + (frid << 2);
          asm volatile("" : "+v"(o)::"memory");
          g0 = (unsigned)__builtin_amdgcn_raw_buffer_load_b32(rx, o, 0, kAuxSc1);
          pend = ((g0 & ~15u) != xcc_want);
        }
        if (!__any(pend)) break;
        if (++spins > max_spins) {
          timed_out = true;
          const unsigned long long pm = __ballot(pend);
          const int fl = __ffsll((long long)pm) - 1;
          const int ff = __shfl(frid, fl, 64);
          const unsigned gs = (unsigned)__shfl((int)g0, fl, 64);
          if (lane == 0) report_expired(err, 2, wg, -1, pm, ff, gs, xcc_want);
          break;
        }
        __builtin_amdgcn_s_sleep(2);
      }
      if (!timed_out && frid >= 0 && (g0 & 15u) == my_xcc) off0 += S, fetch_remote = false;
    }
  }
  const unsigned long long fetch_mask = __ballot(frid >= 0);
  const bool mute = (max_spins_arg >> 31) != 0u && wg == wg_begin;
  const bool pub_lane = state_lane && publishes;
  const char* const xb_base = static_cast<const char*>(xbuf);
  const bool placed = place_pool != nullptr;
  int pub0 = -1, pub1 = -1;
  const char* src0 = xb_base + off0;
  const char* src1 = xb_base + off0 + par;
  if (placed) {
    if (pub_lane) pub0 = rec_off[rid_base + loc], pub1 = rec_off[rec_off_stride + rid_base + loc];
    if (fetch_remote) {
      const int o0 = rec_off[frid], o1 = rec_off[rec_off_stride + frid];
      if (o0 >= 0) src0 = place_pool + o0;
      if (o1 >= 0) src1 = place_pool + o1;
    }
  }
  char* const xb_w = static_cast<char*>(xbuf);
  char* const pa0 = pub0 >= 0 ? place_pool + pub0 : xb_w + my_off;
  char* const pa1 = pub1 >= 0 ? place_pool + pub1 : xb_w + my_off + par;
  auto publish = [&](const v4i_t o, char* pa, const int so) {
    asm volatile("global_store_dwordx4 %0, %1, off sc1" ::"v"(pa), "v"(o) : "memory");
    if (dual) __builtin_amdgcn_raw_buffer_store_b128(o, rx, my_off + S, so, 0);
  };
  {
    lds[(p0 ? rec_wstride : 0) + rec_w] = make_float4(xb, wb12.x, wb12.y, __uint_as_float(tag0));
    if (pub_lane && !mute) {
      v4i_t o;
      o.x = __float_as_int(xb), o.y = __float_as_int(wb12.x), o.z = __float_as_int(wb12.y), o.w = (int)tag0;
      publish(o, p0 ? pa1 : pa0, (int)(tag0 & (kPar - 1)) * par);
    }
  }
  lds_wave_sync();
  const unsigned lds_addr0 = (unsigned)(size_t)(lds);
  unsigned pr_t0 = 0;
  if (PROBE) pr_t0 = (unsigned)clock64();

  auto step = [&](const unsigned s, const unsigned rd_nbr, const unsigned dst, const int wr_rec, const int fetch_area, const int it,
                  const char* const src2, char* const pub2, const int rd_rec) {
    float4 own = make_float4(0.f, 0.f, 0.f, 0.f);
    own = lds[rd_rec];
    const int so_out = (int)((s + 1u) & (kPar - 1)) * par;
    const char* const src = src2;
    v4f_t nbv;
    unsigned rounds = 0;
    for (int z = 0; z < pv_presleep; ++z) __builtin_amdgcn_s_sleep(1);
    {
      unsigned cnt, keep, pend_lo, tagv, tagf, gapk;
      unsigned long long pnarrow, exec_saved;
      const unsigned own_slot = dst + 16u * (unsigned)lane;
      const unsigned f_sleep = (poll_gap & 1) ? 1u + (((unsigned)poll_gap >> 4) & 15u) : 0u, f_narrow = (unsigned)((poll_gap >> 1) & 1);
#define PV_POLL_U                                                                                         \
  asm volatile("s_setprio 0\n\t"                                                                        \
               "s_mov_b64 %[ex], exec\n\t"                                                             \
               "s_mov_b32 %[keep], m0\n\t"                                                              \
               "s_mov_b32 m0, %[dst]\n\t"                                                               \
               "s_mov_b32 %[cnt], 0\n\t"                                                                \
               "s_mov_b64 %[pn], %[fm]\n\t"                                                             \
               "1:\n\t"                                                                                 \
               "s_mov_b64 exec, %[pn]\n\t"                                                              \
               "global_load_lds_dwordx4 %[src], off sc1\n\t"                                            \
               "s_mov_b64 exec, %[ex]\n\t"                                                              \
               "s_mov_b32 %[k], %[fs]\n\t"                                                             \
               "4:\n\t"                                                                                 \
               "s_cmp_eq_u32 %[k], 0\n\t"                                                               \
               "s_cbranch_scc1 3f\n\t"                                                                  \
               "s_sleep 1\n\t"                                                                          \
               "s_sub_u32 %[k], %[k], 1\n\t"                                                            \
               "s_branch 4b\n\t"                                                                        \
               "3:\n\t"                                                                                 \
               "ds_read_b32 %[t], %[ra] offset:12\n\t"                                                  \
               "ds_read_b32 %[t2], %[fa] offset:12\n\t"                                                 \
               "ds_read_b128 %[nb], %[ra]\n\t"                                                          \
               "s_add_u32 %[cnt], %[cnt], 1\n\t"                                                        \
               "s_waitcnt lgkmcnt(0)\n\t"                                                               \
               "v_cmp_ne_u32_e32 vcc, %[tag], %[t2]\n\t"                                                \
               "s_and_b64 %[pn], vcc, %[fm]\n\t"                                                        \
               "s_cmp_eq_u32 %[fn], 0\n\t"                                                              \
               "s_cselect_b64 %[pn], %[fm], %[pn]\n\t"                                                  \
               "v_cmp_ne_u32_e32 vcc, %[tag], %[t]\n\t"                                                 \
               "s_cmp_lt_u32 %[cnt], 64\n\t"                                                            \
               "s_cbranch_vccz 2f\n\t"                                                                  \
               "s_cbranch_scc1 1b\n\t"                                                                  \
               "2:\n\t"                                                                                 \
               "s_setprio 3\n\t"                                                                        \
               "s_or_b32 %[pl], vcc_lo, vcc_hi\n\t"                                                     \
               "s_mov_b32 m0, %[keep]"                                                                   \
               : [keep] "=&s"(keep), [cnt] "=&s"(cnt), [pl] "=&s"(pend_lo), [nb] "=&v"(nbv), [t] "=&v"(tagv), \
                 [t2] "=&v"(tagf), [pn] "=&s"(pnarrow), [k] "=&s"(gapk), [ex] "=&s"(exec_saved)            \
               : [src] "v"(src), [dst] "s"(dst), [ra] "v"(rd_nbr), [fa] "v"(own_slot), [tag] "s"(s), [fm] "s"(fetch_mask), \
                 [fs] "s"(f_sleep), [fn] "s"(f_narrow)                                                     \
               : "vcc", "scc", "memory")
      PV_POLL_U;
      rounds += cnt;
      if (__builtin_expect(pend_lo != 0u, 0)) {
        for (unsigned outer = 0;;) {
          const int ab = __hip_atomic_load(abort_flag, __ATOMIC_RELAXED, __HIP_MEMORY_SCOPE_AGENT);
          if (ab != 0 || ++outer > (max_spins >> 4)) {
            timed_out = true;
            if (ab == 0) {
              const unsigned long long pm = __ballot(tagv != s);
              const int fl = __ffsll((long long)pm) - 1;
              const int ni = __shfl(nbr_idx, fl, 64);
              const int ff = ni >= lcap ? __shfl(frid, ni - lcap, 64) : -2 - ni;
              const unsigned gs = (unsigned)__shfl((int)tagv, fl, 64);
              if (lane == 0) report_expired(err, 3, wg, it, pm, ff, gs, s);
            }
            break;
          }
          PV_POLL_U;
          rounds += cnt;
          if (pend_lo == 0u) break;
        }
      }
#undef PV_POLL_U
    }
    if (VERIFY && verify && !timed_out) {
      const bool bad = fetch_record_torn(frid, src, &lds[fetch_area + lane], s, verify, it, wg, wg_begin, lane);
      if (__any(bad)) torn = timed_out = true;
    }
    unsigned pr_t1 = 0;
    if (PROBE) pr_t1 = (unsigned)clock64();
    xb = own.x, wb12 = v2f_t{own.y, own.z};
    const v2f_t nbw = {nbv.y, nbv.z};
    const float d0 = xb - nbv.x;
    const v2f_t d12 = wb12 - nbw;
    const v2f_t wbi = is_target ? nbw : wb12;
    float K1 = as * d0;
    const v2f_t m12 = P12 * wbi;
    K1 -= m12.x;
    K1 -= m12.y;
    const v2f_t K23 = bs * d12;
    const float q1r = q1 + p.step_q * K1;
    const v2f_t q23r = q23 + p.step_q * K23;
    q1 = __builtin_fminf(__builtin_fmaxf(q1r, -1.0f), 1.0f);
    q23.x = __builtin_fminf(__builtin_fmaxf(q23r.x, -1.0f), 1.0f);
    q23.y = __builtin_fminf(__builtin_fmaxf(q23r.y, -1.0f), 1.0f);
    const float u1 = q1 * p.step_x;
    const v2f_t u23 = q23 * p.step_x;
    const float cx = u1 * ac;
    const v2f_t M2 = is_target ? u23 : v2f_t{cx, cx};
    const v2f_t a12 = M2 * C2;
    v2f_t b12 = u23 * nbeta;
    b12 = is_target ? v2f_t{-0.0f, -0.0f} : b12;
    float X = x;
    v2f_t Wa = w12;
    {
      float W1 = (w12.x + a12.x) + b12.x, W2 = (w12.y + a12.y) + b12.y;
      X = x + cx;
#define PV_ADDS(J)                                                                                    \
  "v_add_f32_dpp %[X], %[cx], %[X] row_shl:" #J " row_mask:0xf bank_mask:0xf\n\t"                      \
  "v_add_f32_dpp %[W1], %[a1], %[W1] row_shl:" #J " row_mask:0xf bank_mask:0xf\n\t"                    \
  "v_add_f32_dpp %[W2], %[a2], %[W2] row_shl:" #J " row_mask:0xf bank_mask:0xf\n\t"                    \
  "v_add_f32_dpp %[W1], %[b1], %[W1] row_shl:" #J " row_mask:0xf bank_mask:0xf\n\t"                    \
  "v_add_f32_dpp %[W2], %[b2], %[W2] row_shl:" #J " row_mask:0xf bank_mask:0xf\n\t"
#define PV_RM(J, M) "s_mov_b64 exec, %[" #M "]\n\t" PV_ADDS(J)
#define PV_ROW(L)                                                                                     \
  "s_nop 1\n\t"                                                                                       \
  "v_readlane_b32 %[s0], %[X], 0\n\t"                                                                 \
  "v_readlane_b32 %[s1], %[W1], 0\n\t"                                                                \
  "v_readlane_b32 %[s2], %[W2], 0\n\t"                                                                \
  "s_nop 3\n\t"                                                                                       \
  "v_writelane_b32 %[X], %[s0], " #L "\n\t"                                                           \
  "v_writelane_b32 %[W1], %[s1], " #L "\n\t"                                                          \
  "v_writelane_b32 %[W2], %[s2], " #L "\n\t"                                                          \
  "s_sub_u32 %[s0], %[md], " #L "\n\t"                                                                \
  "s_min_u32 %[s0], %[s0], 16\n\t"                                                                    \
  "s_bfm_b64 exec, %[s0], " #L "\n\t"                                                                 \
  "s_nop 4\n\t"                                                                                       \
  "v_add_f32 %[X], %[X], %[cx]\n\t"                                                                   \
  "v_add_f32 %[W1], %[W1], %[a1]\n\t"                                                                 \
  "v_add_f32 %[W2], %[W2], %[a2]\n\t"                                                                 \
  "v_add_f32 %[W1], %[W1], %[b1]\n\t"                                                                 \
  "v_add_f32 %[W2], %[W2], %[b2]\n\t"                                                                 \
  "s_nop 1\n\t"                                                                                       \
  PV_ADDS(1)                                                                                          \
  "s_cmp_le_u32 %[s0], 2\n\t"                                                                         \
  "s_cbranch_scc1 1" #L "f\n\t"                                                                       \
  PV_ADDS(2) PV_ADDS(3)                                                                               \
  "s_cmp_le_u32 %[s0], 4\n\t"                                                                         \
  "s_cbranch_scc1 1" #L "f\n\t"                                                                       \
  PV_ADDS(4) PV_ADDS(5) PV_ADDS(6) PV_ADDS(7)                                                         \
  "s_cmp_le_u32 %[s0], 8\n\t"                                                                         \
  "s_cbranch_scc1 1" #L "f\n\t"                                                                       \
  PV_ADDS(8) PV_ADDS(9) PV_ADDS(10) PV_ADDS(11) PV_ADDS(12) PV_ADDS(13) PV_ADDS(14) PV_ADDS(15)       \
  "1" #L ":\n\t"                                                                                      \
  "s_nop 1\n\t"                                                                                       \
  "v_readlane_b32 %[s0], %[X], " #L "\n\t"                                                            \
  "v_readlane_b32 %[s1], %[W1], " #L "\n\t"                                                           \
  "v_readlane_b32 %[s2], %[W2], " #L "\n\t"                                                           \
  "s_nop 3\n\t"                                                                                       \
  "v_writelane_b32 %[X], %[s0], 0\n\t"                                                                \
  "v_writelane_b32 %[W1], %[s1], 0\n\t"                                                               \
  "v_writelane_b32 %[W2], %[s2], 0\n\t"
      unsigned long long exec_saved;
      unsigned row_s0, row_s1, row_s2;
      asm volatile("s_mov_b64 %[ex], exec\n\t"
                   "s_nop 1\n\t"
                   PV_RM(1, m1) PV_RM(2, m2) PV_RM(3, m3) PV_RM(4, m4) PV_RM(5, m5) PV_RM(6, m6) PV_RM(7, m7)
                   "s_cmp_le_u32 %[md], 8\n\t"
                   "s_cbranch_scc1 9f\n\t"
                   PV_RM(8, m8) PV_ADDS(9)
                   "s_cmp_le_u32 %[md], 10\n\t"
                   "s_cbranch_scc1 9f\n\t"
                   PV_ADDS(10) PV_ADDS(11)
                   "s_cmp_le_u32 %[md], 12\n\t"
                   "s_cbranch_scc1 9f\n\t"
                   PV_ADDS(12) PV_ADDS(13) PV_ADDS(14) PV_ADDS(15)
                   "s_cmp_le_u32 %[md], 16\n\t"
                   "s_cbranch_scc1 9f\n\t"
                   PV_ROW(16)
                   "s_cmp_le_u32 %[md], 32\n\t"
                   "s_cbranch_scc1 9f\n\t"
                   PV_ROW(32)
                   "s_cmp_le_u32 %[md], 48\n\t"
                   "s_cbranch_scc1 9f\n\t"
                   PV_ROW(48)
                   "9:\n\t"
                   "s_mov_b64 exec, %[ex]"
                   : [X] "+v"(X), [W1] "+v"(W1), [W2] "+v"(W2), [ex] "=&s"(exec_saved), [s0] "=&s"(row_s0), [s1] "=&s"(row_s1), [s2] "=&s"(row_s2)
                   : [cx] "v"(cx), [a1] "v"(a12.x), [a2] "v"(a12.y), [b1] "v"(b12.x), [b2] "v"(b12.y), [md] "s"(stride),
                     [m1] "s"(rm1), [m2] "s"(rm2), [m3] "s"(rm3), [m4] "s"(rm4), [m5] "s"(rm5), [m6] "s"(rm6), [m7] "s"(rm7), [m8] "s"(rm8)
                   : "scc");
#undef PV_ROW
#undef PV_RM
#undef PV_ADDS
      Wa = v2f_t{W1, W2};
    }
    const VertexNext vn = vertex_update(p, X, Wa, x, w12, data, thr);
    const float xn = vn.xn, nb = vn.nb;
    const v2f_t wbn = vn.wbn;
    if (pub_lane) {
      v4i_t o;
      o.x = __float_as_int(nb), o.y = __float_as_int(wbn.x), o.z = __float_as_int(wbn.y), o.w = (int)(s + 1u);
      publish(o, pub2, so_out);
    }
    __builtin_amdgcn_s_setprio(0);
    if (state_lane || !valid) lds[wr_rec] = make_float4(nb, wbn.x, wbn.y, __uint_as_float(s + 1u));
    ok = ok && (__builtin_fabsf(q1r) <= 3.402823466e+38f) && (__builtin_fabsf(q23r.x) <= 3.402823466e+38f) &&
         (__builtin_fabsf(q23r.y) <= 3.402823466e+38f);
    x_prev = x, w_prev = w12;
    x = xn, w12 = Wa;
    xb = nb, wb12 = wbn;
    if (PROBE) {
      const unsigned pr_t2 = (unsigned)clock64();
      if (lane == 0 && probe) {
        unsigned* o = probe + ((size_t)wg * n_iters + it) * 8;
        o[0] = read_hw_id(), o[1] = read_xcc_id(), o[2] = pr_t1 - pr_t0, o[3] = pr_t2 - pr_t1;
        o[4] = rounds, o[5] = pr_t0, o[6] = (unsigned)wall_clock64(), o[7] = (unsigned)stride | ((unsigned)n_fetch << 8);
      }
      pr_t0 = pr_t2;
    }
  };

  const int areaA = p0 ? rec_stride : 0, areaB = p0 ? 0 : rec_stride;
  const unsigned rdA_nbr = lds_addr0 + 16u * (unsigned)(areaA + nbr_idx), rdB_nbr = lds_addr0 + 16u * (unsigned)(areaB + nbr_idx);
  const unsigned dstA = __builtin_amdgcn_readfirstlane(lds_addr0 + 16u * (unsigned)(areaA + lcap));
  const unsigned dstB = __builtin_amdgcn_readfirstlane(lds_addr0 + 16u * (unsigned)(areaB + lcap));
  const int wrA_rec = (valid ? areaA : 0) + rec_w, wrB_rec = (valid ? areaB : 0) + rec_w;
  const char* const srcA = p0 ? src1 : src0;
  const char* const srcB = p0 ? src0 : src1;
  char* const pubA = p0 ? pa1 : pa0;
  char* const pubB = p0 ? pa0 : pa1;
  int it = 0;
  if (OPEN) {
    const bool decides = wg == wg_begin + n_wgs / 2;
    const unsigned* const stop_req = tail->stop_req;
    unsigned* const stop_word = reinterpret_cast<unsigned*>(err) + 12;
    unsigned stop_at = 0u;
    for (; it + 1 < n_iters && !timed_out; it += 2) {
      if (((unsigned)it & (kOpenCheck - 1u)) == 0u) open_run_check(stop_at, decides, stop_req, stop_word, tag0, it, n_iters, lane);
      if (stop_at != 0u && stop_at - tag0 <= (unsigned)it) break;
      step(tag0 + (unsigned)it, rdA_nbr, dstA, wrB_rec, areaA + lcap, it, srcA, pubB, wrA_rec);
      if (timed_out) break;
      step(tag0 + (unsigned)it + 1u, rdB_nbr, dstB, wrA_rec, areaB + lcap, it + 1, srcB, pubA, wrB_rec);
    }
    if (decides && lane == 0 && !timed_out) reinterpret_cast<unsigned*>(err)[13] = tag0 + (unsigned)it;
  } else {
    for (; it + 1 < n_iters && !timed_out; it += 2) {
      step(tag0 + (unsigned)it, rdA_nbr, dstA, wrB_rec, areaA + lcap, it, srcA, pubB, wrA_rec);
      if (timed_out) break;
      step(tag0 + (unsigned)it + 1u, rdB_nbr, dstB, wrA_rec, areaB + lcap, it + 1, srcB, pubA, wrB_rec);
    }
    if (it < n_iters && !timed_out) step(tag0 + (unsigned)it, rdA_nbr, dstA, wrB_rec, areaA + lcap, it, srcA, pubB, wrA_rec);
  }
  asm volatile("s_waitcnt vmcnt(0)" ::: "memory");

  if (timed_out) {
    if (lane == 0) {
      give_up(abort_flag, err, torn);
      unsigned* const pg = tail->progress;
      if (pg) pg[wg - wg_begin] = 0x80000000u | (unsigned)(it + 1);
    }
    return;
  }

  if (state_lane) write_back_vertex(pv, x, w12, xb, wb12, x_prev, w_prev, data, vstate_out, bar_out, vprev, perm, tail);
  if (active) hq_out[slot] = make_float4(q1, q23.x, q23.y, beta);
  if (!ok && active) atomicOr(err, 1);
}

}

int pv_real_waves_per_simd(bool verify_or_probe) {
  return verify_or_probe ? 5 : 7;
}

static unsigned pv_lds_bytes(int lcap, int slab_slots) { return 16u * (unsigned)(2 * (lcap + 64) + slab_slots + 64); }

int pv_patches_per_cu(const FusedArgs& a, bool verify) {
  if (!a.wg_rowpack) return 0;
  const size_t ldsv = pv_lds_bytes(a.wg_lcap, a.wg_slab_slots);
  int n = 0;
  const void* fv = verify ? (const void*)k_persistent_pv<false, true> : (const void*)k_persistent_pv<false, false>;
  if (hipOccupancyMaxActiveBlocksPerMultiprocessor(&n, fv, 64, ldsv) != hipSuccess) {
    (void)hipGetLastError();
    return 0;
  }
  return n < 4 * pv_real_waves_per_simd(verify) ? n : 4 * pv_real_waves_per_simd(verify);
}

int launch_persistent_run(const FusedArgs& a, const SolverParams& p, int form, int wave_begin, int n_waves,
                          int parity_in, unsigned tag0, int n_iters, int waves_per_block, unsigned max_spins,
                          int presleep, int dual, int xcds, const RunTail* tail, bool cooperative,
                          hipStream_t stream) {
  if (n_waves <= 0 || n_iters <= 0) return (int)hipSuccess;
  if (xcds < 1 || xcds > 8) xcds = 8;
  int wpx = (n_waves + xcds - 1) / xcds;
  const int bpx = (wpx + waves_per_block - 1) / waves_per_block;
  const dim3 grid((unsigned)(bpx * 8)), block((unsigned)(64 * waves_per_block));
  if (form != 2 && form != 3) return (int)hipErrorInvalidValue;
  const int32_t* i0 = a.tv_slot;
  const int32_t* i1 = a.tv_vid;
  const uint32_t* i2 = a.tv_meta;
  const void* i3 = (const void*)a.tv_wave;
  const int4* hrec = a.hrec;
  const float4* hq = a.hq;
  const float4* vstate = a.vstate;
  float4* hq_out = a.hq_out;
  float4* vstate_out = a.vstate_out;
  const float2* vaux = a.vaux;
  const float4* bin = a.bar[parity_in];
  float4* bout = a.bar[parity_in ^ 1];
  float4* vprev = a.vprev;
  void* xbuf = a.xbuf;
  int rec_bytes = persistent_rec_bytes(a);
  SolverParams pp = p;
  int* err = a.err;
  int* abort_flag = a.abort_flag;
  const int32_t* perm = a.perm;
  void* args[] = {&wave_begin, &n_waves, &wpx, &i0, &i1, &i2, &i3, &hrec, &hq, &vstate, &hq_out, &vstate_out, &vaux,
                  &bin, &bout, &vprev, &xbuf, &rec_bytes, &dual, &tag0, &n_iters, &max_spins, &presleep, &pp, &err,
                  &abort_flag, &perm, &tail};
  if (form == 3) {
    int wgx = (n_waves + xcds - 1) / xcds;
    const dim3 gv((unsigned)(wgx * 8)), bv(64u);
    int lcap = a.wg_lcap, slab_slots = a.wg_slab_slots, poll_gap = a.wg_poll_gap;
    const int32_t *w0 = a.wg_slot, *w1 = a.wg_vid, *w3 = a.wg_nbr, *w4 = a.wg_fetch, *w5 = a.wg_info;
    const uint32_t* w2 = a.wg_meta;
    unsigned* probe = a.probe;
    char* place_pool = (a.rec_off && wave_begin == 0 && xcds == 8) ? a.place_pool : nullptr;
    const int32_t* rec_off = a.rec_off;
    int rec_off_stride = a.rec_off_stride;
    unsigned* rot_word = place_pool ? a.rot_word : nullptr;
    const unsigned ldsv = pv_lds_bytes(lcap, slab_slots);
    void* vargs[] = {&wave_begin, &n_waves, &wgx, &lcap, &slab_slots, &w0, &w1, &w2, &w3, &w4, &w5, &hrec, &hq, &vstate,
                     &hq_out, &vstate_out, &vaux, &bin, &bout, &vprev, &xbuf, &rec_bytes, &dual, &tag0, &n_iters,
                     &max_spins, &poll_gap, &pp, &err, &abort_flag, &perm, &tail, &probe, &place_pool, &rec_off, &rec_off_stride, &rot_word};
    const bool vr = (dual >> 1) != 0;
    if (!a.wg_rowpack) return (int)hipErrorInvalidConfiguration;
    const void* fv = probe ? (const void*)k_persistent_pv<true, true>
                           : vr ? (const void*)k_persistent_pv<false, true>
                                : a.open_run ? (const void*)k_persistent_pv<false, false, true> : (const void*)k_persistent_pv<false, false>;
    if (cooperative) return (int)hipLaunchCooperativeKernel(fv, gv, bv, vargs, ldsv, stream);
    return (int)hipExtLaunchKernel(fv, gv, bv, vargs, ldsv, stream, nullptr, a.stop_event, 0);
  }
  unsigned lds_bytes = 0u;
  const void* fn = persistent_tv_kernel(waves_per_block, &lds_bytes);
  if (cooperative) return (int)hipLaunchCooperativeKernel(fn, grid, block, args, lds_bytes, stream);
  return (int)hipExtLaunchKernel(fn, grid, block, args, lds_bytes, stream, nullptr, a.stop_event, 0);
}

namespace {
__global__ void k_warm_cooperative() {}
}
void warm_module_persistent(hipStream_t stream, bool cooperative) {
  hipFuncAttributes fa;
  if (hipFuncGetAttributes(&fa, (const void*)k_persistent_pv<false, false>) != hipSuccess) (void)hipGetLastError();
  FusedArgs a;
  a.wg_rowpack = 1, a.wg_lcap = 16;
  (void)pv_patches_per_cu(a, false);
  void* no_args[] = {nullptr};
  if (cooperative && hipLaunchCooperativeKernel((const void*)k_warm_cooperative, dim3(8), dim3(64), no_args, 0, stream) != hipSuccess) (void)hipGetLastError();
}

}
```

flame_amd/csrc/nltgv2_persistent_common.hpp:

```cpp
#ifndef FLAME_AMD_NLTGV2_PERSISTENT_COMMON_HPP_
#define FLAME_AMD_NLTGV2_PERSISTENT_COMMON_HPP_

#include "nltgv2_device.hpp"

namespace flame_hip {
namespace {

constexpr unsigned kWgActiveBit = 1u << 25, kWgValidBit = 1u << 26, kWgPublishBit = 1u << 27, kWgHeadBit = 1u << 28;
typedef float v2f_t __attribute__((ext_vector_type(2)));
typedef float v4f_t __attribute__((ext_vector_type(4)));

__device__ __forceinline__ void lds_wave_sync() {
  asm volatile("s_waitcnt lgkmcnt(0)" ::: "memory");
}
__device__ __forceinline__ unsigned read_hw_id() {
  unsigned v;
  asm volatile("s_getreg_b32 %0, hwreg(HW_REG_HW_ID)" : "=s"(v));
  return v;
}

__device__ __forceinline__ void report_expired(int* err, int which, int wg, int it, unsigned long long pend, int frid, unsigned seen,
                                               unsigned want) {
  if (atomicCAS(&err[1], 0, which) == 0) {
    err[2] = wg, err[3] = it, err[4] = (int)(unsigned)pend, err[5] = (int)(unsigned)(pend >> 32), err[6] = frid;
    err[7] = (int)seen, err[8] = (int)want, err[9] = (int)read_xcc_id(), err[10] = (int)read_hw_id();
  }
}

__device__ __forceinline__ void give_up(int* abort_flag, int* err, bool torn) {
  __hip_atomic_store(abort_flag, 1, __ATOMIC_RELAXED, __HIP_MEMORY_SCOPE_AGENT);
  atomicOr(err, torn ? 4 : 2);
}

constexpr unsigned kOpenMargin = 128u, kOpenCheck = 64u;

__device__ __forceinline__ void open_run_check(unsigned& stop_at, const bool decides, const unsigned* const stop_req, unsigned* const stop_word,
                                               const unsigned tag0, const int it, const int n_iters, const int lane) {
  if (decides && stop_at == 0u && stop_req &&
      (unsigned)__builtin_amdgcn_readfirstlane((int)__hip_atomic_load(stop_req, __ATOMIC_RELAXED, __HIP_MEMORY_SCOPE_AGENT)) == tag0) {
    stop_at = tag0 + (unsigned)it + kOpenMargin;
    if (lane == 0) {
      __hip_atomic_store(stop_word, stop_at, __ATOMIC_RELAXED, __HIP_MEMORY_SCOPE_AGENT);
      __hip_atomic_store(const_cast<unsigned*>(stop_req), 0u, __ATOMIC_RELAXED, __HIP_MEMORY_SCOPE_AGENT);
    }
  }
  if (stop_at == 0u) {
    const unsigned w = (unsigned)__builtin_amdgcn_readfirstlane((int)__hip_atomic_load(stop_word, __ATOMIC_RELAXED, __HIP_MEMORY_SCOPE_AGENT));
    if (w > tag0 && w - tag0 <= (unsigned)n_iters + kOpenMargin) stop_at = w;
  }
}

__device__ __forceinline__ bool fetch_record_torn(const int frid, const char* const src, const float4* const lds_slot, const unsigned s,
                                                  const int verify, const int it, const int wg, const int wg_begin, const int lane) {
  v4i_t g2 = {0, 0, 0, 0};
  if (frid >= 0) {
    asm volatile("global_load_dwordx4 %0, %1, off sc1\n\ts_waitcnt vmcnt(0)" : "=&v"(g2) : "v"(src) : "memory");
  }
  const float4 l4 = *lds_slot;
  if ((verify & 2) && it == 2 && wg == wg_begin && lane == 0) g2.x ^= 0x00400000;
  return frid >= 0 && (g2.x != __float_as_int(l4.x) || g2.y != __float_as_int(l4.y) || g2.z != __float_as_int(l4.z) ||
                       (unsigned)g2.w != s || __float_as_uint(l4.w) != s);
}

struct VertexNext {
  float xn, nb;
  v2f_t wbn;
};
__device__ __forceinline__ VertexNext vertex_update(const SolverParams& p, const float X, const v2f_t Wa, const float x, const v2f_t w12,
                                                    const float data, const float thr) {
  VertexNext n;
  const float diff = X - data, x_dn = X - thr, x_up = X + thr;
  float xn = (diff < -thr) ? x_up : data;
  xn = (diff > thr) ? x_dn : xn;
  xn = (xn < p.x_min) ? p.x_min : xn;
  xn = (xn > p.x_max) ? p.x_max : xn;
  float nb = xn + p.theta * (xn - x);
  nb = (nb < p.x_min) ? p.x_min : nb;
  nb = (nb > p.x_max) ? p.x_max : nb;
  n.xn = xn, n.nb = nb;
  n.wbn = Wa + p.theta * (Wa - w12);
  return n;
}

__device__ __forceinline__ void write_back_vertex(const int pv, const float x, const v2f_t w12, const float xb, const v2f_t wb12,
                                                  const float x_prev, const v2f_t w_prev, const float data, float4* vstate_out,
                                                  float4* bar_out, float4* vprev, const int32_t* __restrict__ perm,
                                                  const RunTail* __restrict__ tail) {
  vstate_out[pv] = make_float4(x, w12.x, w12.y, data);
  bar_out[pv] = make_float4(xb, wb12.x, wb12.y, 0.0f);
  vprev[pv] = make_float4(x_prev, w_prev.x, w_prev.y, 0.0f);
  float* const export_out = tail->export_out;
  float* const photo_err = tail->photo.err;
  if (export_out || photo_err) {
    const int o = perm[pv];
    if (o >= 0 && export_out) export_out[o] = x * tail->export_scale;
    if (o >= 0 && photo_err) {
      const PhotoFuse& photo = tail->photo;
      photo_err[o] = photo_residual_at(photo.pos[o], x * photo.graph_scale, photo.geo, photo.ref, photo.cmp, photo.rows,
                                       photo.cols, photo.step, photo.border);
    }
  }
}

}
}

#endif
```

flame_amd/csrc/nltgv2_run.hip:

```cpp
#include "nltgv2_context.hpp"

namespace flame_hip {
namespace host {

void pick_config(const flame_nltgv2_ctx* ctx, int* unroll, int* wpb) {
  const bool small = ctx->L.n_slices <= 8 * ctx->prop.multiProcessorCount;
  *unroll = ctx->opt_unroll ? ctx->opt_unroll : (small ? 8 : 4);
  *wpb = ctx->opt_block_waves ? ctx->opt_block_waves : (small ? 1 : 4);
}

struct WaveGroup {
  int begin, count;
};

int ensure_form_rows(flame_nltgv2_ctx* ctx, int form);
int plan_groups(flame_nltgv2_ctx* ctx, int form, int total, int cap, const std::vector<int32_t>& cw, std::vector<WaveGroup>* groups);

bool cooperative_allowed() {
  static const bool ok = [] {
    if (std::getenv("FLAME_NLTGV2_NO_COOPERATIVE")) return false;
    if (std::getenv("FLAME_NLTGV2_COOPERATIVE")) return true;
    if (std::getenv("ROCP_TOOL_LIBRARIES")) return false;
    if (void* h = dlopen("librocprofiler-sdk.so.1", RTLD_NOLOAD | RTLD_LAZY)) {
      dlclose(h);
// ... 231 lines not shown
  std::vector<uint16_t> rank;
  float best = 0.f, mean = 0.f, worst = 0.f;
};
std::mutex& g_place_mu = *new std::mutex;
std::vector<PlacePool>& g_place_free = *new std::vector<PlacePool>;
std::vector<int>& g_place_seen = *new std::vector<int>;
}

bool place_calibrate_at_create(int device) {
  std::lock_guard<std::mutex> lock(g_place_mu);
  bool first = true;
  for (int d : g_place_seen) first = first && d != device;
  if (first) g_place_seen.push_back(device);
  for (const PlacePool& e : g_place_free)
    if (e.device == device) return true;
  return first;
}

void place_pool_release(flame_nltgv2_ctx* ctx) {
  if (!ctx->place_pool.p || ctx->place_state != 1 || ctx->place_rank_host.empty()) return;
  PlacePool e;
  e.device = ctx->device, e.mem = ctx->place_pool.p, e.rank.swap(ctx->place_rank_host);
  e.best = ctx->place_best_us, e.mean = ctx->place_mean_us, e.worst = ctx->place_worst_us;
  ctx->device_bytes -= ctx->place_pool.cap;
  ctx->place_pool = DevBuf{};
  ctx->place_base = nullptr, ctx->place_state = 0;
  std::lock_guard<std::mutex> lock(g_place_mu);
  g_place_free.push_back(std::move(e));
}

int place_calibrate(flame_nltgv2_ctx* ctx) {
  ctx->place_state = -1;
  constexpr int P = kPlacePages, kIters = 12;
  const size_t pool_bytes = (size_t)2 * P * 4096;
  if (!ctx->place_pool.p && !std::getenv("FLAME_NLTGV2_RECALIBRATE")) {
    PlacePool e;
    {
      std::lock_guard<std::mutex> lock(g_place_mu);
      for (size_t i = 0; i < g_place_free.size(); ++i)
        if (g_place_free[i].device == ctx->device) {
          e = std::move(g_place_free[i]);
          g_place_free.erase(g_place_free.begin() + (long)i);
          break;
        }
    }
    if (e.mem) {
      ctx->place_pool.p = e.mem, ctx->place_pool.cap = pool_bytes + 4096;
      ctx->device_bytes += ctx->place_pool.cap;
      ctx->place_best_us = e.best, ctx->place_mean_us = e.mean, ctx->place_worst_us = e.worst;
      ctx->place_rank_host.swap(e.rank);
      int rc = ensure(ctx, ctx->place_rank, sizeof(uint16_t) * 2 * 64 * P);
      if (!rc) rc = ensure(ctx, ctx->place_fill, sizeof(int) * (2 * P + 16 + 128));
      if (rc) return rc;
      ctx->place_base = reinterpret_cast<char*>((reinterpret_cast<uintptr_t>(ctx->place_pool.p) + 4095) & ~uintptr_t(4095));
      HIPCHK(ctx, hipMemsetAsync(ctx->place_base, 0, pool_bytes, ctx->stream));
      HIPCHK(ctx, hipMemsetAsync(ctx->place_fill.p, 0, sizeof(int) * (2 * P + 16 + 128), ctx->stream));
      HIPCHK(ctx, hipMemcpyAsync(ctx->place_rank.p, ctx->place_rank_host.data(), sizeof(uint16_t) * ctx->place_rank_host.size(), hipMemcpyHostToDevice,
                                 ctx->stream));
      HIPCHK(ctx, wait_solver_stream(ctx));
      ctx->place_state = 1;
      return 0;
    }
  }
  int rc = ensure(ctx, ctx->place_pool, pool_bytes + 4096);
  if (!rc) rc = ensure(ctx, ctx->place_meas, sizeof(unsigned) * 64 * 2 * P + sizeof(int) * 64 + sizeof(int));
  if (!rc) rc = ensure(ctx, ctx->place_rank, sizeof(uint16_t) * 2 * 64 * P);
  if (!rc) rc = ensure(ctx, ctx->place_fill, sizeof(int) * (2 * P + 16 + 128));
  if (rc) return rc;
  ctx->place_base = reinterpret_cast<char*>((reinterpret_cast<uintptr_t>(ctx->place_pool.p) + 4095) & ~uintptr_t(4095));
  unsigned* d_out = (unsigned*)ctx->place_meas.p;
  int* d_xcc = (int*)(d_out + (size_t)64 * 2 * P);
  int* d_fail = d_xcc + 64;
  HIPCHK(ctx, hipMemsetAsync(ctx->place_base, 0, pool_bytes, ctx->stream));
  HIPCHK(ctx, hipMemsetAsync(ctx->place_meas.p, 0, sizeof(unsigned) * 64 * 2 * P + sizeof(int) * 65, ctx->stream));
  HIPCHK(ctx, hipMemsetAsync(ctx->place_fill.p, 0, sizeof(int) * (2 * P + 16 + 128), ctx->stream));
  LAUNCHCHK(ctx, launch_place_calibrate(ctx->place_base, 2 * P, kIters, d_out, d_xcc, d_fail, ctx->stream));
  std::vector<unsigned> out((size_t)64 * 2 * P);
  int xcc[65];
  HIPCHK(ctx, hipMemcpyAsync(out.data(), d_out, sizeof(unsigned) * out.size(), hipMemcpyDeviceToHost, ctx->stream));
  HIPCHK(ctx, hipMemcpyAsync(xcc, d_xcc, sizeof(int) * 65, hipMemcpyDeviceToHost, ctx->stream));
  HIPCHK(ctx, wait_solver_stream(ctx));
  HIPCHK(ctx, hipMemsetAsync(ctx->place_base, 0, pool_bytes, ctx->stream));
  if (xcc[64] != 0) return 0;
  std::vector<unsigned> lat((size_t)64 * 2 * P, 0u);
  bool have[64] = {false};
  for (int b = 8; b < 64; ++b) {
    const int x = b & 7, j = b >> 3, pb = ((8 - j) & 7) * 8 + ((x + j) & 7);
    const int from = xcc[pb], to = xcc[b];
    if (from < 0 || from > 7 || to < 0 || to > 7 || from == to) return 0;
    for (int pg = 0; pg < 2 * P; ++pg) {
      const unsigned t = out[(size_t)b * 2 * P + pg];
      if (t == 0u || t > (1u << 24)) return 0;
      lat[(size_t)(from * 8 + to) * 2 * P + pg] = t;
    }
    have[from * 8 + to] = true;
  }
  for (int a = 0; a < 8; ++a)
    for (int b = 0; b < 8; ++b)
      if (a != b && !have[a * 8 + b]) return 0;
  std::vector<uint16_t> rank((size_t)2 * 64 * P);
  double best = 0.0, mean = 0.0, worst = 0.0;
  for (int par = 0; par < 2; ++par)
    for (int c = 0; c < 64; ++c) {
      uint16_t* r = &rank[((size_t)par * 64 + c) * P];
      for (int t = 0; t < P; ++t) r[t] = (uint16_t)t;
      if (c / 8 == c % 8) continue;
      const unsigned* l = &lat[(size_t)c * 2 * P + (size_t)par * P];
      std::stable_sort(r, r + P, [&](uint16_t u, uint16_t v) { return l[u] < l[v]; });
      double m = 0.0;
      for (int t = 0; t < P; ++t) m += l[t];
      best += l[r[0]], worst += l[r[P - 1]], mean += m / P;
    }
  if (std::getenv("FLAME_NLTGV2_TRACE")) {
    for (int a = 0; a < 8; ++a) {
      std::fprintf(stderr, "[flame_nltgv2] hand-off from XCD %d to 0..7, best page (us):", a);
      for (int b = 0; b < 8; ++b) {
        if (a == b) { std::fprintf(stderr, "   -  "); continue; }
        const unsigned* l = &lat[(size_t)(a * 8 + b) * 2 * P];
        unsigned best_t = ~0u, worst_t = 0u;
        for (int t = 0; t < P; ++t) best_t = std::min(best_t, l[t]), worst_t = std::max(worst_t, l[t]);
        std::fprintf(stderr, " %.3f/%.3f", best_t / (100.0 * kIters), worst_t / (100.0 * kIters));
      }
      std::fprintf(stderr, "\n");
    }
  }
  const double to_us = 1.0 / (100.0 * kIters) / (2.0 * 56.0);
  ctx->place_best_us = (float)(best * to_us), ctx->place_mean_us = (float)(mean * to_us), ctx->place_worst_us = (float)(worst * to_us);
  HIPCHK(ctx, hipMemcpyAsync(ctx->place_rank.p, rank.data(), sizeof(uint16_t) * rank.size(), hipMemcpyHostToDevice, ctx->stream));
  HIPCHK(ctx, wait_solver_stream(ctx));
  ctx->place_state = 1;
  ctx->place_rank_host.swap(rank);
  return 0;
}

int place_records(flame_nltgv2_ctx* ctx, int per_xcd) {
  const size_t stride = records_capacity(ctx->L);
  int rc = ensure(ctx, ctx->place_rec_off, sizeof(int32_t) * 2 * stride);
  if (!rc) rc = ensure(ctx, ctx->place_patch, sizeof(int32_t) * stride + stride);
  if (rc) return rc;
  LAUNCHCHK(ctx, launch_place_records(ctx->c, ctx->f, per_xcd, (const int32_t*)ctx->order_m.p, (const int32_t*)ctx->rid_of.p,
                                      (int32_t*)ctx->place_patch.p, (int8_t*)((int32_t*)ctx->place_patch.p + stride),
                                      (const uint16_t*)ctx->place_rank.p, kPlacePages, (int*)ctx->place_fill.p,
                                      (int32_t*)ctx->place_rec_off.p, (int)stride, ctx->stream));
  ctx->place_topo = ctx->topo, ctx->place_per_xcd = per_xcd;
  return 0;
}

static bool open_run_applies(const flame_nltgv2_ctx* ctx, int form, const std::vector<WaveGroup>& groups) {
  if (groups.size() != 1) return false;
  const int cus = ctx->prop.multiProcessorCount;
  return (form == 3 && groups[0].count <= 20 * cus) || (form == 4 && groups[0].count <= 14 * cus);
}

int enqueue_run(flame_nltgv2_ctx* ctx, const flame_nltgv2_params* p, int n) {
  if (n <= 0) return 0;
  if (ctx->open_inflight) {
    const int rc0 = finish(ctx);
    if (rc0) return rc0;
  }
  if (ctx->opt_solver == 1) {
    int rc = ensure_canon(ctx);
    if (rc) return rc;
    const SolverParams sp = to_sp(p);
    for (int it = 0; it < n; ++it) {
      LAUNCHCHK(ctx, launch_save_prev(ctx->c, ctx->stream));
      LAUNCHCHK(ctx, launch_dual(ctx->c, sp, ctx->stream));
      LAUNCHCHK(ctx, launch_primal(ctx->c, sp, ctx->stream));
      LAUNCHCHK(ctx, launch_extragradient(ctx->c, sp, ctx->stream));
    }
    ctx->fused_valid = false;
    ctx->last_run_path = 4;
    if (ctx->replaying == 0) ctx->iters_total += n;
    if (ctx->export_ptr) LAUNCHCHK(ctx, launch_export(ctx->c, ctx->f, false, ctx->export_scale, ctx->export_ptr, ctx->stream));
    return enqueue_photo_sweep(ctx, false);
  }
  if (ctx->opt_mesh_state == 1 && ctx->canon_valid) {
    HIPCHK(ctx, hipEventRecord(ctx->ev_snap, ctx->stream));
    ctx->snap_topo = ctx->topo;
  }
  int rc = ensure_fused(ctx);
  if (rc) return rc;
  if (ctx->pending.active) {
    if (ctx->pending.ops.size() >= kMaxChain) {
      rc = finish(ctx);
    } else {
      rc = snapshot_chain_start(ctx);
    }
    if (rc) return rc;
  }
  int unroll, wpb;
  pick_config(ctx, &unroll, &wpb);
  std::vector<WaveGroup> groups;
  const int form = plan_persistent(ctx, n, &groups, true);
  const bool open_run = ctx->want_open != 0 && open_run_applies(ctx, form, groups) && !ctx->pending.active && ctx->opt_probe == 0 &&
                        ctx->opt_verify == 0 && ctx->replaying == 0 && (n & 1) == 0 && ctx->h_stop != nullptr && ctx->ctl_stream != nullptr;
  if (ctx->want_open != 0 && !open_run) {
    ctx->want_open = 0;
    return 0;
  }
  if (form != 0) {
    if ((uint64_t)ctx->tag_next + (uint64_t)n >= 0x07ff0000ull || (ctx->xbuf_form != 0 && ctx->xbuf_form != form)) {
      const size_t bytes = kXbufBytesPerVertex * records_capacity(ctx->L);
      HIPCHK(ctx, hipMemsetAsync(ctx->xbuf.p, 0, bytes, ctx->stream));
      if (ctx->place_base) {
        HIPCHK(ctx, hipMemsetAsync(ctx->place_base, 0, (size_t)2 * kPlacePages * 4096, ctx->stream));
        HIPCHK(ctx, hipMemsetAsync((int*)ctx->place_fill.p + 2 * kPlacePages, 0, 64, ctx->stream));
      }
      HIPCHK(ctx, hipMemsetAsync((int*)ctx->err.p + 12, 0, 2 * sizeof(int), ctx->stream));
      ctx->tag_next = 1;
    }
    ctx->xbuf_form = form;
    const uint32_t tag0 = ctx->tag_next + 2;
    const uint64_t key = ctx->topo * 1024 + (uint64_t)form * 64 + (ctx->opt_verify != 0 ? 16 : 0) + (ctx->opt_probe != 0 ? 8 : 0) +
                         (ctx->opt_dual == 2 ? 4 : ctx->opt_dual == 1 ? 2 : 0) + (ctx->opt_xcds > 0 ? 1 : 0);
    const RunTail* tail_dev = nullptr;
    {
      RunTail want;
      std::memset(static_cast<void*>(&want), 0, sizeof want);
      want.export_out = ctx->export_ptr, want.export_scale = ctx->export_scale;
      if (open_run) {
        const bool fresh = ctx->stop_dev.p == nullptr;
        rc = ensure(ctx, ctx->stop_dev, 64);
        if (rc) return rc;
        if (fresh) HIPCHK(ctx, hipMemsetAsync(ctx->stop_dev.p, 0, 64, ctx->stream));
        ctx->open_tag0 = tag0;
      }
      want.stop_req = open_run ? (const unsigned*)ctx->stop_dev.p : nullptr;
      const PhotoFuse pf = photo_target(ctx);
      std::memcpy(static_cast<void*>(&want.photo), &pf, sizeof pf);
      if (form == 3 && std::getenv("FLAME_NLTGV2_TRACE")) {
        rc = ensure(ctx, ctx->progress, 2 * sizeof(unsigned) * (size_t)ctx->L.wg_count);
        if (rc) return rc;
        HIPCHK(ctx, hipMemsetAsync(ctx->progress.p, 0, 2 * sizeof(unsigned) * (size_t)ctx->L.wg_count, ctx->stream));
        want.progress = (unsigned*)ctx->progress.p;
      }
      constexpr size_t kTailStride = (sizeof(RunTail) + 255) / 256 * 256;
      rc = ensure(ctx, ctx->run_tail, kTailStride * flame_nltgv2_ctx::kTailSlots);
      if (rc) return rc;
      int slot = -1;
      for (int i = 0; i < flame_nltgv2_ctx::kTailSlots && slot < 0; ++i)
        if (ctx->tail_valid[i] && std::memcmp(&want, &ctx->tail_sent[i], sizeof(RunTail)) == 0) slot = i;
      if (slot < 0) {
        slot = ctx->tail_next, ctx->tail_next = (ctx->tail_next + 1) % flame_nltgv2_ctx::kTailSlots;
        HIPCHK(ctx, hipMemcpyAsync((char*)ctx->run_tail.p + kTailStride * (size_t)slot, &want, sizeof(RunTail), hipMemcpyHostToDevice, ctx->stream));
        ctx->tail_sent[slot] = want;
        ctx->tail_valid[slot] = true;
      }
      tail_dev = (const RunTail*)((const char*)ctx->run_tail.p + kTailStride * (size_t)slot);
    }
    int e = 0;
    for (const WaveGroup& gr : groups) {
      const bool carries = &gr == &groups.back() && ctx->coop_checked_key == key && ctx->run_ev_pick >= 0 && ctx->ev_run[ctx->run_ev_pick] != nullptr;
      ctx->f.stop_event = carries ? ctx->ev_run[ctx->run_ev_pick] : nullptr;
      const int pw = gr.count <= 4 * ctx->prop.multiProcessorCount ? 1 : 4;
      const int dual = (ctx->opt_dual == 2 || (ctx->opt_dual == 1 && gr.count > kDualMinWavesPerCu * ctx->prop.multiProcessorCount) ? 1 : 0) |
                       (ctx->opt_verify == 2 ? 6 : ctx->opt_verify == 1 ? 2 : 0);
      const int cus_per_xcd = ctx->prop.multiProcessorCount / 8;
      const bool one_xcd = form == 3 && gr.count <= 2 * cus_per_xcd;
      const int xcds = ctx->opt_xcds > 0 ? ctx->opt_xcds : one_xcd ? 1 : 8;
      const int presleep = ctx->opt_presleep > 0 ? ctx->opt_presleep - 1 : kPreSleepTv;
      const unsigned spins_arg = (ctx->opt_fault > 0 && (ctx->replaying == 0 || ctx->opt_fault >= (1 << 22)))
                                     ? (0x80000000u | (unsigned)(ctx->opt_fault & ((1 << 22) - 1))) : kMaxSpins;
      if (form == 3) {
        const bool dense = gr.count > kPvPaceAbovePerCu * ctx->prop.multiProcessorCount;
        const bool denser = gr.count > kPvPaceMoreAbovePerCu * ctx->prop.multiProcessorCount;
        const int dense_gap = denser ? kPvDenserGap : kPvDenseGap, dense_pre = denser ? kPvDenserPreSleep : kPvDensePreSleep;
        const int gap = ctx->opt_poll_gap > 0 ? ctx->opt_poll_gap - 1 : dense ? (3 | ((dense_gap - 1) << 4)) : kPvPollGap;
        ctx->f.wg_poll_gap = gap | ((ctx->opt_presleep > 0 ? ctx->opt_presleep - 1 : dense ? dense_pre : kPvPreSleep) << 8);
        ctx->f.rec_off = nullptr, ctx->f.place_pool = nullptr;
        if (ctx->opt_place && groups.size() == 1 && gr.begin == 0 && xcds == 8 && (dual & 1)) {
          if (ctx->place_state == 0) {
            rc = place_calibrate(ctx);
            if (rc) return rc;
          }
          const int per_xcd = (gr.count + xcds - 1) / xcds;
          if (ctx->place_state == 1 && (ctx->place_topo != ctx->topo || ctx->place_per_xcd != per_xcd)) {
            rc = place_records(ctx, per_xcd);
            if (rc) return rc;
          }
          if (ctx->place_state == 1) {
            ctx->f.place_pool = ctx->place_base, ctx->f.rec_off = (const int32_t*)ctx->place_rec_off.p;
            ctx->f.rec_off_stride = (int)records_capacity(ctx->L);
            ctx->f.rot_word = (unsigned*)ctx->place_fill.p + 2 * kPlacePages;
          }
        }
        ctx->f.probe = nullptr;
        if (ctx->opt_probe) {
          const size_t words = (size_t)ctx->L.wg_count * (size_t)n * 8;
          rc = ensure(ctx, ctx->probe, words * sizeof(unsigned));
          if (rc) return rc;
          ctx->f.probe = (unsigned*)ctx->probe.p;
          ctx->probe_words = words;
          HIPCHK(ctx, hipMemsetAsync(ctx->probe.p, 0, words * sizeof(unsigned), ctx->stream));
        }
      }
      if (form == 4) {
        const bool dense = gr.count > kPv2PaceAbovePerCu * ctx->prop.multiProcessorCount;
        const int gap = ctx->opt_poll_gap > 0 ? ctx->opt_poll_gap - 1 : dense ? (3 | ((kPv2DenseGap - 1) << 4)) : kPvPollGap;
        const int poll_gap = gap | ((ctx->opt_presleep > 0 ? ctx->opt_presleep - 1 : dense ? kPv2DensePreSleep : kPvPreSleep) << 8);
        ctx->f.open_run = open_run ? 1 : 0;
        e = launch_persistent_pv2(ctx->f, ctx->pv2_args, to_sp(p), gr.begin, gr.count, ctx->parity, tag0, n, spins_arg, poll_gap, dual,
                                  tail_dev, cooperative_allowed() && ctx->coop_checked_key != key, ctx->stream);
        ctx->f.open_run = 0;
        if (e != 0) break;
        continue;
      }
      ctx->f.open_run = open_run ? 1 : 0;
      e = launch_persistent_run(ctx->f, to_sp(p), form, gr.begin, gr.count, ctx->parity, tag0, n, pw, spins_arg, presleep, dual,
                                xcds, tail_dev, cooperative_allowed() && ctx->coop_checked_key != key, ctx->stream);
      ctx->f.open_run = 0;
      if (e != 0) break;
    }
    ctx->run_event_bound = e == 0 && ctx->f.stop_event != nullptr;
    ctx->f.stop_event = nullptr;
    ctx->tag_next = tag0 + (uint32_t)n;
    if (e == 0) {
      if (!ctx->pending.active) {
        ctx->pending.active = true, ctx->pending.snapshotted = false;
        ctx->pending.ops.clear();
        ctx->pending.parity_before = ctx->parity, ctx->pending.have_prev_before = ctx->have_prev;
      }
      {
        flame_nltgv2_ctx::PendingOp op;
        op.kind = 0, op.params = *p, op.n = n;
        op.open = open_run, op.tag0 = tag0;
        op.dst = ctx->export_ptr, op.scale = ctx->export_scale;
        ctx->pending.ops.push_back(op);
      }
      ctx->photo_fresh = photo_target(ctx).err != nullptr;
      ctx->open_inflight = open_run, ctx->open_stop_sent = false;
      if (open_run) ctx->want_open = 2;
      if (!open_run && ctx->replaying == 0) ctx->iters_total += n;
      std::swap(ctx->hq, ctx->hq_alt);
      std::swap(ctx->vstate, ctx->vstate_alt);
      ctx->buf_gen ^= 1;
      refresh_args(ctx);
      ctx->coop_checked_key = key;
      ctx->last_run_path = form == 4 ? 7 : form == 3 ? 6 : 5;
      ctx->last_run_groups = (int)groups.size();
      ctx->last_run_waves_per_cu = 0;
      for (const WaveGroup& gr : groups) ctx->last_run_waves_per_cu = std::max(ctx->last_run_waves_per_cu, (gr.count + ctx->prop.multiProcessorCount - 1) / ctx->prop.multiProcessorCount);
      ctx->parity ^= 1;
      ctx->have_prev = true;
      ctx->canon_valid = false;
      return 0;
    }
    if (std::getenv("FLAME_NLTGV2_TRACE")) std::fprintf(stderr, "[flame_nltgv2] persistent launch refused: hip error %d (%s), form %d, pv_occ %d\n", e, hipGetErrorString((hipError_t)e), form, ctx->pv_occ);
    (void)hipGetLastError();
    ctx->persist_refused_topo = ctx->topo;
    if (groups.size() > 1 && !ctx->pending.active) {
      HIPCHK(ctx, hipMemsetAsync(ctx->abort_flag.p, 0xff, sizeof(int), ctx->stream));
      HIPCHK(ctx, wait_solver_stream(ctx));
      HIPCHK(ctx, hipMemsetAsync(ctx->err.p, 0, kErrBytes, ctx->stream));
      HIPCHK(ctx, hipMemsetAsync(ctx->abort_flag.p, 0, sizeof(int), ctx->stream));
    }
  }
  if (ctx->pending.active) {
    flame_nltgv2_ctx::PendingOp op;
    op.kind = 0, op.params = *p, op.n = n;
    op.dst = ctx->export_ptr, op.scale = ctx->export_scale;
    ctx->pending.ops.push_back(op);
  }
  int left = n;
  while (left > 0) {
    const int chunk = left >= kGraphChunk ? kGraphChunk : left;
    if (ctx->opt_use_graph && chunk >= 4) {
      hipGraphExec_t exec = nullptr;
      rc = get_graph(ctx, p, chunk, ctx->parity, unroll, wpb, &exec);
      if (rc) return rc;
      HIPCHK(ctx, hipGraphLaunch(exec, ctx->stream));
      ctx->last_run_path = 2;
    } else {
      rc = enqueue_fused_eager(ctx, p, chunk, ctx->parity, unroll, wpb, true);
      if (rc) return rc;
      ctx->last_run_path = 3;
    }
    ctx->parity ^= (chunk & 1);
    left -= chunk;
  }
  ctx->have_prev = true;
  ctx->canon_valid = false;
  if (ctx->replaying == 0) ctx->iters_total += n;
  if (ctx->export_ptr) LAUNCHCHK(ctx, launch_export(ctx->c, ctx->f, true, ctx->export_scale, ctx->export_ptr, ctx->stream));
  return enqueue_photo_sweep(ctx, true);
}

void trace_expired_wait(flame_nltgv2_ctx* ctx) {
  const int* e = ctx->h_err;
  static const char* const kWhich[] = {"?", "rotation word", "XCC table", "step records"};
  std::fprintf(stderr, "[flame_nltgv2] persistent run taken back (flags %d): first expired wait = %s, patch %d, step %d, lanes waiting %08x%08x, "
               "first of them for record %d (tag seen %u, wanted %u), on XCC %d hw_id %08x\n", e[0], kWhich[e[1] & 3], e[2], e[3], (unsigned)e[5],
               (unsigned)e[4], e[6], (unsigned)e[7], (unsigned)e[8], e[9], (unsigned)e[10]);
  if (!ctx->progress.p || ctx->L.wg_count <= 0) return;
  std::vector<unsigned> pg((size_t)2 * ctx->L.wg_count);
  if (hipMemcpy(pg.data(), ctx->progress.p, sizeof(unsigned) * pg.size(), hipMemcpyDeviceToHost) != hipSuccess) return;
  size_t silent = 0, left = 0;
  unsigned lo = ~0u, hi = 0;
  int first_silent = -1;
  const size_t n_p = (size_t)ctx->L.wg_count;
  {
    unsigned t_lo = ~0u, t_hi = 0;
    size_t started = 0, late = 0;
    for (size_t i = 0; i < n_p; ++i)
      if (pg[n_p + i]) ++started, t_lo = std::min(t_lo, pg[n_p + i]), t_hi = std::max(t_hi, pg[n_p + i]);
    int first_late = -1;
    for (size_t i = 0; i < n_p; ++i)
      if (pg[n_p + i] && pg[n_p + i] - t_lo > 10000u) {
        if (first_late < 0) first_late = (int)i;
        ++late;
      }
    std::fprintf(stderr, "[flame_nltgv2]   %zu of %zu patches started, over %u us; %zu of them more than 10 ms after the first (first such patch: %d)\n",
                 started, n_p, started ? t_hi - t_lo : 0u, late, first_late);
  }
  for (size_t i = 0; i < n_p; ++i) {
    if (pg[i] == 0) {
      if (first_silent < 0) first_silent = (int)i;
      ++silent;
    } else {
      ++left, lo = std::min(lo, pg[i] & 0x7fffffffu), hi = std::max(hi, pg[i] & 0x7fffffffu);
    }
  }
  std::fprintf(stderr, "[flame_nltgv2]   %zu patches left through an expired wait (in steps %u..%u), %zu wrote nothing (finished, or never ran; first: %d)\n",
               left, left ? lo - 1 : 0, left ? hi - 1 : 0, silent, first_silent);
}

int finish(flame_nltgv2_ctx* ctx, bool unpack_behind, bool* unpacked, const std::function<int()>* behind_fn, bool* behind_launched) {
  const bool open_run = ctx->open_inflight;
  if (open_run) {
    request_open_stop(ctx);
    ctx->open_inflight = false, ctx->open_stop_sent = false;
  }
  HIPCHK(ctx, hipMemcpyAsync(ctx->h_err, ctx->err.p, kErrBytes, hipMemcpyDeviceToHost, ctx->stream));
  bool behind = false;
  if (unpack_behind && ctx->pending.active && !ctx->canon_valid && !ctx->replaying) {
    const int rc = wait_raster(ctx);
    if (rc) return rc;
    LAUNCHCHK(ctx, launch_unpack_state(ctx->c, ctx->f, ctx->parity, ctx->have_prev, ctx->stream));
    behind = true;
    if (behind_fn) {
      const int rc2 = (*behind_fn)();
      if (rc2) return rc2;
      if (behind_launched) *behind_launched = true;
    }
  }
  HIPCHK(ctx, wait_solver_stream(ctx));
  flame_nltgv2_ctx::PendingRun run;
  std::swap(run, ctx->pending);
  if (open_run && !run.ops.empty() && run.ops.back().open) {
    flame_nltgv2_ctx::PendingOp& op = run.ops.back();
    const uint32_t done = (uint32_t)ctx->h_err[13], decided = (uint32_t)ctx->h_err[12];
    int n_done = op.n;
    if (!(*ctx->h_err & 6)) {
      if (done > op.tag0 && done - op.tag0 <= (uint32_t)op.n) n_done = (int)(done - op.tag0);
    } else {
      n_done = (decided > op.tag0 && decided - op.tag0 <= (uint32_t)op.n) ? (int)(decided - op.tag0) : std::min(op.n, 256);
    }
    op.n = n_done, op.open = false;
    ctx->iters_total += n_done;
    ctx->last_open_iters = n_done;
  }
  if (*ctx->h_err & 6) {
    if (*ctx->h_err & 4) ctx->torn_records_detected++;
    std::memcpy(ctx->last_expired, ctx->h_err, kErrBytes);
    if (std::getenv("FLAME_NLTGV2_TRACE")) trace_expired_wait(ctx);
    if (!run.active) {
      ctx->have_graph = false;
      return fail(ctx, FLAME_NLTGV2_ERR_TIMEOUT);
    }
    if (run.snapshotted) {
      const size_t n_slots = (size_t)(ctx->L.rows + kRowPad) * kWave, n_packed = (size_t)ctx->L.n_slices * kWave;
      HIPCHK(ctx, hipMemcpyAsync(ctx->hq.p, ctx->snap_hq.p, sizeof(float4) * n_slots, hipMemcpyDeviceToDevice, ctx->stream));
      HIPCHK(ctx, hipMemcpyAsync(ctx->vstate.p, ctx->snap_vstate.p, sizeof(float4) * n_packed, hipMemcpyDeviceToDevice, ctx->stream));
      HIPCHK(ctx, hipMemcpyAsync(ctx->f.bar[run.parity_before], ctx->snap_bar.p, sizeof(float4) * n_packed, hipMemcpyDeviceToDevice,
                                 ctx->stream));
    } else {
      std::swap(ctx->hq, ctx->hq_alt);
      std::swap(ctx->vstate, ctx->vstate_alt);
      ctx->buf_gen ^= 1;
      refresh_args(ctx);
    }
    ctx->parity = run.parity_before;
    ctx->have_prev = run.have_prev_before;
    ctx->fused_valid = true, ctx->canon_valid = false;
    const int attempt = ctx->replay_attempt;
    if (attempt == 0) {
      ctx->persist_timeout_streak = (ctx->persist_backoff_topo == ctx->topo) ? std::min(ctx->persist_timeout_streak + 1, 9) : 1;
      ctx->persist_backoff_topo = ctx->topo;
      ctx->persist_backoff_left = 4 << (ctx->persist_timeout_streak - 1);
      if (!(*ctx->h_err & 4)) {
        ctx->timeouts_recovered++;
        if (ctx->last_run_waves_per_cu > kCrowdedWavesPerCu) ctx->crowded_until_topo = ctx->topo + 1 + kCrowdedTopologies;
      }
    } else {
      ctx->replays_per_step++;
    }
    HIPCHK(ctx, hipMemsetAsync(ctx->err.p, 0, kErrBytes, ctx->stream));
    HIPCHK(ctx, hipMemsetAsync(ctx->abort_flag.p, 0, sizeof(int), ctx->stream));
    ctx->replaying = (attempt == 0 && !(*ctx->h_err & 4) && ctx->opt_persistent != 0 && !std::getenv("FLAME_NLTGV2_REPLAY_PER_STEP")) ? 1 : 2;
    ctx->replay_attempt = attempt + 1;
    int replay_rc = 0;
    float* const export_now = ctx->export_ptr;
    const float export_scale_now = ctx->export_scale;
    for (const flame_nltgv2_ctx::PendingOp& op : run.ops) {
      if (op.kind == 0) {
        ctx->export_ptr = op.dst, ctx->export_scale = op.scale;
        replay_rc = enqueue_run(ctx, &op.params, op.n);
        ctx->export_ptr = export_now, ctx->export_scale = export_scale_now;
      } else {
        const int e = launch_export(ctx->c, ctx->f, true, op.scale, op.dst, ctx->stream);
        if (e) ctx->last_hip = e, ctx->last_error = FLAME_NLTGV2_ERR_HIP, replay_rc = FLAME_NLTGV2_ERR_HIP;
      }
      if (replay_rc) break;
    }
    ctx->replaying = 0;
    if (replay_rc) {
      ctx->replay_attempt = 0;
      return replay_rc;
    }
    const int rc2 = finish(ctx);
    ctx->replay_attempt = 0;
    return rc2;
  }
  if (run.active && ctx->last_run_path >= 5) ctx->persist_timeout_streak = 0;
  if (*ctx->h_err != 0) {
    HIPCHK(ctx, hipMemsetAsync(ctx->err.p, 0, kErrBytes, ctx->stream));
    if (unpacked) *unpacked = behind && !(behind_launched && *behind_launched);
    return fail(ctx, FLAME_NLTGV2_ERR_NAN);
  }
  if (unpacked) *unpacked = behind;
  return 0;
}

int snapshot_chain_start(flame_nltgv2_ctx* ctx) {
  if (!ctx->pending.active || ctx->pending.snapshotted) return 0;
  const size_t n_slots = (size_t)(ctx->L.rows + kRowPad) * kWave, n_packed = (size_t)ctx->L.n_slices * kWave;
  int rc = ensure(ctx, ctx->snap_hq, sizeof(float4) * n_slots);
  if (!rc) rc = ensure(ctx, ctx->snap_vstate, sizeof(float4) * n_packed);
  if (!rc) rc = ensure(ctx, ctx->snap_bar, sizeof(float4) * n_packed);
  if (rc) return rc;
  CopyTable t;
  t.n = 3;
  t.e[0] = {ctx->snap_hq.p, ctx->hq_alt.p, sizeof(float4) * n_slots};
  t.e[1] = {ctx->snap_vstate.p, ctx->vstate_alt.p, sizeof(float4) * n_packed};
  t.e[2] = {ctx->snap_bar.p, ctx->f.bar[ctx->pending.parity_before], sizeof(float4) * n_packed};
  LAUNCHCHK(ctx, launch_copy_arrays(t, ctx->stream));
  ctx->pending.snapshotted = true;
  return 0;
}

}
}

extern "C" {

int flame_nltgv2_run_async(flame_nltgv2_ctx* ctx, const flame_nltgv2_params* p, int n_iters) {
  flame_hip::RoctxRange roctx_range_("flame_nltgv2_run_async");
  int rc = enter(ctx);
  if (rc) return rc;
  if (!ctx->have_graph) return fail(ctx, FLAME_NLTGV2_ERR_NO_GRAPH);
  if (!params_ok(p) || n_iters < 0) return fail(ctx, FLAME_NLTGV2_ERR_INVALID_ARG);
  if (n_iters == 0) return 0;
  const int idx = ctx->run_ev_last ^ 1;
  ctx->run_ev_pick = idx;
  ctx->run_event_bound = false;
  rc = enqueue_run(ctx, p, n_iters);
  ctx->run_ev_pick = -1;
  if (rc) return rc;
  bool stands = ctx->run_event_bound;
  if (!stands && ctx->track_runs) {
    HIPCHK(ctx, hipEventRecord(ctx->ev_run[idx], ctx->stream));
    stands = true;
  }
  ctx->run_ev_valid[idx] = stands;
  ctx->run_ev_last = idx;
  ctx->run_event_seq = ctx->call_seq;
  return 0;
}

int flame_nltgv2_run_open(flame_nltgv2_ctx* ctx, const flame_nltgv2_params* p, int max_iters, int32_t* opened) {
  flame_hip::RoctxRange roctx_range_("flame_nltgv2_run_open");
  int rc = enter(ctx);
  if (rc) return rc;
  if (opened) *opened = 0;
  if (!ctx->have_graph) return fail(ctx, FLAME_NLTGV2_ERR_NO_GRAPH);
  if (!params_ok(p) || max_iters < 0 || (max_iters & 1)) return fail(ctx, FLAME_NLTGV2_ERR_INVALID_ARG);
  if (max_iters == 0) return 0;
  if (ctx->pending.active) {
    std::vector<WaveGroup> groups;
    const int form = plan_persistent(ctx, max_iters, &groups, false);
    if (!open_run_applies(ctx, form, groups) || ctx->opt_probe != 0 || ctx->opt_verify != 0 || !ctx->h_stop || !ctx->ctl_stream) return 0;
  }
  if (ctx->pending.active) {
    rc = finish(ctx);
    if (rc) return rc;
  }
  const int idx = ctx->run_ev_last ^ 1;
  ctx->run_ev_pick = idx;
  ctx->run_event_bound = false;
// ... 136 lines not shown
```

flame_amd/regularizer.py:

```python
from __future__ import annotations

import ctypes as C
import os

import numpy as np

_HERE = os.path.dirname(os.path.abspath(__file__))
_LIB = None

_FP = C.POINTER(C.c_float)
_IP = C.POINTER(C.c_int32)

OPT_SOLVER, OPT_USE_HIPGRAPH, OPT_PERSISTENT, OPT_PROBE, OPT_VERIFY_RECORDS, OPT_PLACEMENT, OPT_SYNC_PATH, OPT_COST_SUM, OPT_MESH_STATE = 1, 2, 5, 12, 14, 16, 17, 18, 19
OPT_BLOCK_WAVES, OPT_UNROLL, OPT_DUAL_PUBLISH, OPT_PRESLEEP, OPT_XCDS, OPT_FAULT_INJECT, OPT_POLL_GAP = 103, 104, 106, 108, 109, 110, 113
RUN_PATHS = {0: "none", 1: "persistent (the lane-per-half-edge form, retired in round 3)", 2: "per-step hipGraph", 3: "per-step eager", 4: "canonical 4-sweep",
             5: "persistent-tv", 6: "persistent-pv", 7: "persistent-pv2"}
ERR_NAN = -5

VERTEX_STATE = ("x", "w1", "w2", "x_bar", "w1_bar", "w2_bar", "x_prev", "w1_prev", "w2_prev")
EDGE_STATE = ("q1", "q2", "q3")


def _rows_contiguous_u8(a) -> bool:
    return a.dtype == np.uint8 and a.ndim == 2 and a.strides[1] == 1 and a.strides[0] >= max(a.shape[1], 1)


class NLTGV2Error(RuntimeError):
    def __init__(self, status: int, what: str):
        super().__init__(f"{what}: status {status} ({status_string(status)})")
        self.status = status


class Params(C.Structure):

    _fields_ = [(n, C.c_float) for n in ("data_factor", "step_x", "step_q", "theta", "x_min", "x_max")]

    def __init__(self, data_factor=0.1, step_x=0.001, step_q=125.0, theta=0.25, x_min=0.0, x_max=10.0):
        super().__init__(data_factor, step_x, step_q, theta, x_min, x_max)


class MeshFilterParams(C.Structure):

    _fields_ = [("do_oblique_triangle_filter", C.c_int32), ("oblique_normal_thresh", C.c_float),
                ("oblique_idepth_diff_factor", C.c_float), ("oblique_idepth_diff_abs", C.c_float),
                ("do_edge_length_filter", C.c_int32), ("edge_length_thresh", C.c_float),
                ("do_idepth_triangle_filter", C.c_int32), ("min_triangle_idepth", C.c_float)]

    def __init__(self, do_oblique_triangle_filter=True, oblique_normal_thresh=1.39626, oblique_idepth_diff_factor=0.35,
                 oblique_idepth_diff_abs=0.1, do_edge_length_filter=True, edge_length_thresh=0.333,
                 do_idepth_triangle_filter=True, min_triangle_idepth=0.01):
        super().__init__(int(bool(do_oblique_triangle_filter)), oblique_normal_thresh, oblique_idepth_diff_factor,
                         oblique_idepth_diff_abs, int(bool(do_edge_length_filter)), edge_length_thresh,
                         int(bool(do_idepth_triangle_filter)), min_triangle_idepth)


class _MeshOutputsView(C.Structure):
    _fields_ = [("V", C.c_int32), ("T", C.c_int32), ("tri_valid", C.POINTER(C.c_uint8)), ("normals", _FP), ("vtx_idepth", _FP),
                ("n_valid", C.c_int32), ("rows", C.c_int32), ("cols", C.c_int32), ("filtered_map", _FP),
                ("filtered_coverage", C.c_int32), ("device_ms", C.c_float)]


class DebugImageParams(C.Structure):

    _fields_ = [("scene_color_scale", C.c_float), ("flip", C.c_int32), ("want_idepthmap", C.c_int32), ("want_normals", C.c_int32)]

    def __init__(self, scene_color_scale=1.0, flip=False, want_idepthmap=True, want_normals=True):
        super().__init__(scene_color_scale, int(bool(flip)), int(bool(want_idepthmap)), int(bool(want_normals)))


class _DebugImagesView(C.Structure):
    _fields_ = [("rows", C.c_int32), ("cols", C.c_int32), ("idepthmap_img", C.POINTER(C.c_uint8)), ("normals_img", C.POINTER(C.c_uint8)),
                ("w1_map", _FP), ("w2_map", _FP), ("device_ms", C.c_float)]


class _Graph(C.Structure):
    _fields_ = (
        [("V", C.c_int32), ("E", C.c_int32), ("pos", _FP)]
        + [(n, _FP) for n in VERTEX_STATE + ("data_term", "data_weight")]
        + [("src", _IP), ("dst", _IP)]
        + [(n, _FP) for n in ("alpha", "beta") + EDGE_STATE]
    )


class _SyncInput(C.Structure):
    _fields_ = [("V", C.c_int32), ("feat_id", _IP), ("pos", _FP), ("data_term", _FP), ("data_weight", _FP),
                ("init_x", _FP), ("E", C.c_int32), ("edges", _IP), ("check_sticky_obstacles", C.c_int32),
                ("sticky_threshold", C.c_float), ("init_graph_scale", C.c_float), ("edges_unique", C.c_int32),
                ("init_from_map", C.c_int32)]


class _Projection(C.Structure):
    _fields_ = [("K", C.c_float * 9), ("Kinv", C.c_float * 9), ("KRKinv", C.c_float * 9), ("q_ref_to_cmp", C.c_float * 4),
                ("t_ref_to_cmp", C.c_float * 3), ("region_x", C.c_float), ("region_y", C.c_float), ("region_w", C.c_float),
                ("region_h", C.c_float)]


class _Info(C.Structure):
    _fields_ = [
        ("abi_version", C.c_int32), ("device", C.c_int32), ("V", C.c_int32), ("E", C.c_int32),
        ("n_slices", C.c_int32), ("max_degree", C.c_int32), ("padded_half_edges", C.c_int64),
        ("device_bytes", C.c_int64), ("algorithmic_bytes_per_iter", C.c_int64), ("compute_units", C.c_int32),
        ("device_name", C.c_char * 64), ("gcn_arch", C.c_char * 32), ("last_run_path", C.c_int32), ("he_waves", C.c_int32), ("tv_waves", C.c_int32),
        ("tv_wave_capacity", C.c_int32), ("last_run_groups", C.c_int32), ("timeouts_recovered", C.c_int32),
        ("patches", C.c_int32), ("torn_records_detected", C.c_int32), ("last_sync_path", C.c_int32),
        ("last_run_waves_per_cu", C.c_int32), ("reserved0", C.c_int32), ("reserved1", C.c_int32), ("replays_per_step", C.c_int32),
    ]


def library_path() -> str:
    return os.environ.get("FLAME_AMD_LIBRARY") or os.path.join(_HERE, "libflame_nltgv2_hip.so")


ABI_SYMBOLS = (
    "flame_nltgv2_default_params", "flame_nltgv2_create", "flame_nltgv2_destroy", "flame_nltgv2_set_stream", "flame_nltgv2_stream_wait_run", "flame_nltgv2_runs_in_flight", "flame_nltgv2_run_open", "flame_nltgv2_iterations",
    "flame_nltgv2_upload_graph", "flame_nltgv2_update_data", "flame_nltgv2_upload_state", "flame_nltgv2_run",
    "flame_nltgv2_run_async", "flame_nltgv2_sync", "flame_nltgv2_run_timed", "flame_nltgv2_save_prev",
    "flame_nltgv2_dual_step", "flame_nltgv2_primal_step", "flame_nltgv2_extragradient_step", "flame_nltgv2_step",
    "flame_nltgv2_costs", "flame_nltgv2_download_state", "flame_nltgv2_export_idepth_device",
    "flame_nltgv2_export_idepth_device_async", "flame_nltgv2_set_export_target",
    "flame_nltgv2_set_option", "flame_nltgv2_get_info", "flame_nltgv2_last_error", "flame_nltgv2_last_hip_error",
    "flame_nltgv2_status_string", "flame_nltgv2_abi_version", "flame_nltgv2_pack_probe", "flame_nltgv2_read_probe", "flame_nltgv2_layout_selftest", "flame_nltgv2_placement_info",
    "flame_nltgv2_photo_set_images", "flame_nltgv2_photo_residual", "flame_nltgv2_photo_fuse",
    "flame_nltgv2_photo_residual_last", "flame_nltgv2_sync_graph", "flame_nltgv2_sync_prepare", "flame_nltgv2_sync_commit",
    "flame_nltgv2_get_topology", "flame_nltgv2_graph_size", "flame_nltgv2_set_feature_ids", "flame_nltgv2_interpolate_mesh",
    "flame_nltgv2_interpolate_mesh_begin", "flame_nltgv2_interpolate_mesh_end",
    "flame_nltgv2_interpolate_mesh_arrays", "flame_nltgv2_project_graph", "flame_nltgv2_rescale_data",
    "flame_delaunay_triangulate",
    "flame_nltgv2_default_mesh_filter_params", "flame_nltgv2_oblique_cos_bound", "flame_nltgv2_mesh_outputs_begin",
    "flame_nltgv2_mesh_outputs_end", "flame_nltgv2_mesh_outputs",
    "flame_nltgv2_default_debug_image_params", "flame_nltgv2_debug_images_begin", "flame_nltgv2_debug_images_end",
    "flame_nltgv2_debug_images",
)


def load_library():
    global _LIB
    if _LIB is not None:
        return _LIB
    path = library_path()
    if not os.path.exists(path):
        raise NLTGV2Error(-2, f"HIP library not built: {path} (run __graft_entry__.build())")
    L = C.CDLL(path)
    ctx = C.c_void_p
    PP, GP = C.POINTER(Params), C.POINTER(_Graph)
    sig = {
        "flame_nltgv2_default_params": (None, [PP]),
        "flame_nltgv2_create": (C.c_int, [C.POINTER(ctx), C.c_int]),
        "flame_nltgv2_destroy": (C.c_int, [ctx]),
        "flame_nltgv2_set_stream": (C.c_int, [ctx, C.c_void_p]),
        "flame_nltgv2_stream_wait_run": (C.c_int, [ctx, C.c_void_p]),
        "flame_nltgv2_runs_in_flight": (C.c_int, [ctx, C.POINTER(C.c_int32)]),
        "flame_nltgv2_run_open": (C.c_int, [ctx, C.POINTER(Params), C.c_int, C.POINTER(C.c_int32)]),
        "flame_nltgv2_iterations": (C.c_int, [ctx, C.POINTER(C.c_int64), C.POINTER(C.c_int32)]),
        "flame_nltgv2_upload_graph": (C.c_int, [ctx, GP]),
        "flame_nltgv2_update_data": (C.c_int, [ctx, _FP, _FP]),
        "flame_nltgv2_upload_state": (C.c_int, [ctx, GP]),
        "flame_nltgv2_run": (C.c_int, [ctx, PP, C.c_int]),
        "flame_nltgv2_run_async": (C.c_int, [ctx, PP, C.c_int]),
        "flame_nltgv2_sync": (C.c_int, [ctx]),
        "flame_nltgv2_run_timed": (C.c_int, [ctx, PP, C.c_int, _FP]),
        "flame_nltgv2_save_prev": (C.c_int, [ctx]),
        "flame_nltgv2_dual_step": (C.c_int, [ctx, PP]),
        "flame_nltgv2_primal_step": (C.c_int, [ctx, PP]),
        "flame_nltgv2_extragradient_step": (C.c_int, [ctx, PP]),
        "flame_nltgv2_step": (C.c_int, [ctx, PP]),
        "flame_nltgv2_costs": (C.c_int, [ctx, PP, _FP, _FP]),
        "flame_nltgv2_download_state": (C.c_int, [ctx, GP]),
        "flame_nltgv2_export_idepth_device": (C.c_int, [ctx, C.c_void_p, C.c_float]),
        "flame_nltgv2_export_idepth_device_async": (C.c_int, [ctx, C.c_void_p, C.c_float]),
        "flame_nltgv2_set_export_target": (C.c_int, [ctx, C.c_void_p, C.c_float]),
        "flame_nltgv2_set_option": (C.c_int, [ctx, C.c_int, C.c_int]),
        "flame_nltgv2_get_info": (C.c_int, [ctx, C.POINTER(_Info)]),
        "flame_nltgv2_last_error": (C.c_int, [ctx]),
        "flame_nltgv2_last_hip_error": (C.c_int, [ctx]),
        "flame_nltgv2_status_string": (C.c_char_p, [C.c_int]),
        "flame_nltgv2_abi_version": (C.c_int, []),
        "flame_nltgv2_layout_selftest": (C.c_int, [ctx, C.POINTER(C.c_int64)]),
        "flame_nltgv2_placement_info": (C.c_int, [ctx, C.POINTER(C.c_int32), C.POINTER(C.c_int32), C.POINTER(C.c_float)]),
        "flame_nltgv2_pack_probe": (C.c_int, [GP, _IP, _IP, _IP, _IP, C.c_int64, C.POINTER(C.c_int64)]),
        "flame_nltgv2_read_probe": (C.c_int, [ctx, C.POINTER(C.c_uint32), C.c_int64, C.POINTER(C.c_int64)]),
        "flame_nltgv2_photo_set_images": (C.c_int, [ctx, C.POINTER(C.c_uint8), C.POINTER(C.c_uint8), C.c_int, C.c_int, C.c_int]),
        "flame_nltgv2_photo_residual": (C.c_int, [ctx, _FP, _FP, C.c_float, C.c_int, _FP]),
        "flame_nltgv2_photo_fuse": (C.c_int, [ctx, _FP, _FP, C.c_float, C.c_int, C.c_int]),
        "flame_nltgv2_photo_residual_last": (C.c_int, [ctx, _FP]),
        "flame_nltgv2_sync_graph": (C.c_int, [ctx, C.POINTER(_SyncInput)]),
        "flame_nltgv2_sync_prepare": (C.c_int, [ctx, C.POINTER(_SyncInput)]),
        "flame_nltgv2_sync_commit": (C.c_int, [ctx]),
        "flame_nltgv2_get_topology": (C.c_int, [ctx, _IP, _IP, _IP]),
        "flame_nltgv2_graph_size": (C.c_int, [ctx, C.POINTER(C.c_int32), C.POINTER(C.c_int32)]),
        "flame_nltgv2_set_feature_ids": (C.c_int, [ctx, _IP]),
        "flame_delaunay_triangulate": (C.c_int, [_FP, C.c_int32, _IP, C.c_int32, _IP, _IP, C.c_int32, _IP]),
        "flame_nltgv2_project_graph": (C.c_int, [ctx, C.POINTER(_Projection), C.c_float, C.POINTER(C.c_uint8), _FP]),
        "flame_nltgv2_rescale_data": (C.c_int, [ctx, C.c_float, _FP, PP]),
        "flame_nltgv2_interpolate_mesh": (C.c_int, [ctx, _IP, C.c_int32, C.POINTER(C.c_uint8), C.c_int, C.c_int, C.c_float,
                                                    _FP, _IP]),
        "flame_nltgv2_interpolate_mesh_begin": (C.c_int, [ctx, _IP, C.c_int32, C.POINTER(C.c_uint8), C.c_int, C.c_int, C.c_float]),
        "flame_nltgv2_interpolate_mesh_end": (C.c_int, [ctx, C.POINTER(_FP), _IP]),
        "flame_nltgv2_interpolate_mesh_arrays": (C.c_int, [ctx, _IP, C.c_int32, _FP, _FP, C.c_int32, C.POINTER(C.c_uint8),
                                                           C.POINTER(C.c_uint8), C.c_int, C.c_int, _FP, _IP]),
        "flame_nltgv2_default_mesh_filter_params": (None, [C.POINTER(MeshFilterParams)]),
        "flame_nltgv2_oblique_cos_bound": (C.c_float, [C.c_float]),
        "flame_nltgv2_mesh_outputs_begin": (C.c_int, [ctx, _IP, C.c_int32, _FP, C.POINTER(MeshFilterParams), C.c_int, C.c_int,
                                                      C.c_float, C.c_int]),
        "flame_nltgv2_mesh_outputs_end": (C.c_int, [ctx, C.POINTER(_MeshOutputsView)]),
        "flame_nltgv2_mesh_outputs": (C.c_int, [ctx, _IP, C.c_int32, _FP, C.POINTER(MeshFilterParams), C.c_int, C.c_int, C.c_float,
                                                C.POINTER(C.c_uint8), _FP, _FP, _IP, _FP, _IP]),
        "flame_nltgv2_default_debug_image_params": (None, [C.POINTER(DebugImageParams)]),
        "flame_nltgv2_debug_images_begin": (C.c_int, [ctx, C.c_void_p, C.c_void_p, C.c_int, _FP, C.POINTER(DebugImageParams), C.c_int,
                                                      C.c_int]),
        "flame_nltgv2_debug_images_end": (C.c_int, [ctx, C.POINTER(_DebugImagesView)]),
        "flame_nltgv2_debug_images": (C.c_int, [ctx, C.c_void_p, C.c_void_p, C.c_int, _FP, C.POINTER(DebugImageParams), C.c_int, C.c_int,
                                                C.POINTER(C.c_uint8), C.POINTER(C.c_uint8), _FP, _FP]),
    }
    for name, (res, args) in sig.items():
        fn = getattr(L, name)
        fn.restype, fn.argtypes = res, args
    _LIB = L
    return L


def status_string(status: int) -> str:
    try:
        return load_library().flame_nltgv2_status_string(int(status)).decode()
    except Exception:
        return "?"


def _as(arr, dtype, n, name):
    a = np.ascontiguousarray(arr, dtype=dtype)
    if a.size != n:
        raise ValueError(f"{name}: expected {n} elements, got {a.size}")
    return a


def _graph_view(g: dict, keep: list, need_all=True) -> _Graph:
    V, E = int(g["V"]), int(g["E"])
    cg = _Graph()
    cg.V, cg.E = V, E
    sizes = {"pos": 2 * V, "data_term": V, "data_weight": V, "src": E, "dst": E, "alpha": E, "beta": E}
    sizes.update({k: V for k in VERTEX_STATE})
    sizes.update({k: E for k in EDGE_STATE})
    for name, ctype in _Graph._fields_[2:]:
        if name not in g or g[name] is None:
            if need_all and not name.endswith("_prev"):
                raise KeyError(name)
            continue
        dt = np.int32 if ctype is _IP else np.float32
        a = _as(g[name], dt, sizes[name], name)
        keep.append(a)
        setattr(cg, name, a.ctypes.data_as(ctype))
    return cg


def delaunay(pos, out=None):
    L = load_library()
    p = np.ascontiguousarray(pos, np.float32).reshape(-1, 2)
    n = p.shape[0]
    nt, ne = C.c_int32(0), C.c_int32(0)
# ... 410 lines not shown
```

include/flame_nltgv2.h:

```cpp
#ifndef FLAME_NLTGV2_H_
#define FLAME_NLTGV2_H_

#include <stdint.h>

#ifdef __cplusplus
extern "C" {
#endif

#define FLAME_NLTGV2_ABI_VERSION 7

typedef struct flame_nltgv2_ctx flame_nltgv2_ctx;

typedef enum flame_nltgv2_status {
  FLAME_NLTGV2_OK = 0,
  FLAME_NLTGV2_ERR_INVALID_ARG = -1,
  FLAME_NLTGV2_ERR_NO_DEVICE = -2,
  FLAME_NLTGV2_ERR_HIP = -3,
  FLAME_NLTGV2_ERR_NO_GRAPH = -4,
  FLAME_NLTGV2_ERR_NAN = -5,
  FLAME_NLTGV2_ERR_OOM = -6,
  FLAME_NLTGV2_ERR_TIMEOUT = -7,
  FLAME_NLTGV2_ERR_ASSERT = -8
} flame_nltgv2_status;

// ... 56 lines not shown
  float region_x, region_y, region_w, region_h;
} flame_nltgv2_projection;
int flame_nltgv2_project_graph(flame_nltgv2_ctx* ctx, const flame_nltgv2_projection* pr, float graph_scale,
                               uint8_t* keep_out, float* pos_out);
int flame_nltgv2_rescale_data(flame_nltgv2_ctx* ctx, float graph_scale, float* new_graph_scale, flame_nltgv2_params* params);

int flame_nltgv2_update_data(flame_nltgv2_ctx* ctx, const float* data_term, const float* data_weight);

int flame_nltgv2_upload_state(flame_nltgv2_ctx* ctx, const flame_nltgv2_graph* state);

int flame_nltgv2_run(flame_nltgv2_ctx* ctx, const flame_nltgv2_params* p, int n_iters);
int flame_nltgv2_run_async(flame_nltgv2_ctx* ctx, const flame_nltgv2_params* p, int n_iters);
int flame_nltgv2_sync(flame_nltgv2_ctx* ctx);
int flame_nltgv2_run_timed(flame_nltgv2_ctx* ctx, const flame_nltgv2_params* p, int n_iters, float* elapsed_ms);

int flame_nltgv2_save_prev(flame_nltgv2_ctx* ctx);
int flame_nltgv2_dual_step(flame_nltgv2_ctx* ctx, const flame_nltgv2_params* p);
int flame_nltgv2_primal_step(flame_nltgv2_ctx* ctx, const flame_nltgv2_params* p);
int flame_nltgv2_extragradient_step(flame_nltgv2_ctx* ctx, const flame_nltgv2_params* p);
int flame_nltgv2_step(flame_nltgv2_ctx* ctx, const flame_nltgv2_params* p);

int flame_nltgv2_costs(flame_nltgv2_ctx* ctx, const flame_nltgv2_params* p, float* smoothness, float* data);

int flame_nltgv2_download_state(flame_nltgv2_ctx* ctx, flame_nltgv2_graph* out);

int flame_nltgv2_export_idepth_device(flame_nltgv2_ctx* ctx, void* dst_device, float scale);
int flame_nltgv2_export_idepth_device_async(flame_nltgv2_ctx* ctx, void* dst_device, float scale);
int flame_nltgv2_set_export_target(flame_nltgv2_ctx* ctx, void* dst_device, float scale);
int flame_nltgv2_stream_wait_run(flame_nltgv2_ctx* ctx, void* hip_stream);
int flame_nltgv2_runs_in_flight(flame_nltgv2_ctx* ctx, int32_t* n_out);
int flame_nltgv2_run_open(flame_nltgv2_ctx* ctx, const flame_nltgv2_params* p, int max_iters, int32_t* opened);
int flame_nltgv2_iterations(flame_nltgv2_ctx* ctx, int64_t* total, int32_t* open_in_flight);

int flame_nltgv2_interpolate_mesh(flame_nltgv2_ctx* ctx, const int32_t* triangles, int32_t T, const uint8_t* tri_valid,
                                  int rows, int cols, float graph_scale, float* idepthmap_out, int32_t* coverage_out);
int flame_nltgv2_interpolate_mesh_begin(flame_nltgv2_ctx* ctx, const int32_t* triangles, int32_t T, const uint8_t* tri_valid,
                                        int rows, int cols, float graph_scale);
int flame_nltgv2_interpolate_mesh_end(flame_nltgv2_ctx* ctx, const float** map_out, int32_t* coverage_out);
int flame_nltgv2_interpolate_mesh_arrays(flame_nltgv2_ctx* ctx, const int32_t* triangles, int32_t T,
                                         const float* vertices_xy, const float* values, int32_t V,
                                         const uint8_t* vtx_valid, const uint8_t* tri_valid, int rows, int cols,
                                         float* img_out, int32_t* coverage_out);

typedef struct flame_nltgv2_mesh_filter_params {
  int32_t do_oblique_triangle_filter;
  float oblique_normal_thresh;
  float oblique_idepth_diff_factor;
  float oblique_idepth_diff_abs;
  int32_t do_edge_length_filter;
  float edge_length_thresh;
  int32_t do_idepth_triangle_filter;
  float min_triangle_idepth;
} flame_nltgv2_mesh_filter_params;
void flame_nltgv2_default_mesh_filter_params(flame_nltgv2_mesh_filter_params* p);

float flame_nltgv2_oblique_cos_bound(float oblique_normal_thresh);

typedef struct flame_nltgv2_mesh_outputs_view {
  int32_t V, T;
  const uint8_t* tri_valid;
  const float* normals;
  const float* vtx_idepth;
  int32_t n_valid;
  int32_t rows, cols;
  const float* filtered_map;
  int32_t filtered_coverage;
  float device_ms;
} flame_nltgv2_mesh_outputs_view;

int flame_nltgv2_mesh_outputs_begin(flame_nltgv2_ctx* ctx, const int32_t* triangles, int32_t T, const float* Kinv,
                                    const flame_nltgv2_mesh_filter_params* filter, int rows, int cols, float graph_scale,
                                    int want_filtered_map);
int flame_nltgv2_mesh_outputs_end(flame_nltgv2_ctx* ctx, flame_nltgv2_mesh_outputs_view* out);
int flame_nltgv2_mesh_outputs(flame_nltgv2_ctx* ctx, const int32_t* triangles, int32_t T, const float* Kinv,
                              const flame_nltgv2_mesh_filter_params* filter, int rows, int cols, float graph_scale,
                              uint8_t* tri_valid_out, float* normals_out, float* vtx_idepth_out, int32_t* n_valid_out,
                              float* filtered_map_out, int32_t* filtered_coverage_out);

typedef struct flame_nltgv2_debug_image_params {
  float   scene_color_scale;
  int32_t flip;
  int32_t want_idepthmap;
  int32_t want_normals;
} flame_nltgv2_debug_image_params;
void flame_nltgv2_default_debug_image_params(flame_nltgv2_debug_image_params* p);

typedef struct flame_nltgv2_debug_images_view {
  int32_t rows, cols;
  const uint8_t* idepthmap_img;
  const uint8_t* normals_img;
  const float* w1_map;
  const float* w2_map;
  float device_ms;
} flame_nltgv2_debug_images_view;

int flame_nltgv2_debug_images_begin(flame_nltgv2_ctx* ctx, const uint8_t* img_host, const void* img_device, int step_bytes,
                                    const float* K, const flame_nltgv2_debug_image_params* params, int rows, int cols);
int flame_nltgv2_debug_images_end(flame_nltgv2_ctx* ctx, flame_nltgv2_debug_images_view* out);
int flame_nltgv2_debug_images(flame_nltgv2_ctx* ctx, const uint8_t* img_host, const void* img_device, int step_bytes, const float* K,
                              const flame_nltgv2_debug_image_params* params, int rows, int cols, uint8_t* idepthmap_img_out,
                              uint8_t* normals_img_out, float* w1_map_out, float* w2_map_out);

int flame_delaunay_triangulate(const float* xy, int32_t n, int32_t* triangles, int32_t tri_capacity,
                               int32_t* n_triangles, int32_t* edges, int32_t edge_capacity, int32_t* n_edges);

int flame_nltgv2_photo_set_images(flame_nltgv2_ctx* ctx, const uint8_t* ref, const uint8_t* cmp, int rows, int cols,
                                  int step_bytes);
int flame_nltgv2_photo_residual(flame_nltgv2_ctx* ctx, const float* KRKinv, const float* Kt, float graph_scale,
                                int border, float* err_out);
int flame_nltgv2_photo_fuse(flame_nltgv2_ctx* ctx, const float* KRKinv, const float* Kt, float graph_scale, int border,
                            int enable);
int flame_nltgv2_photo_residual_last(flame_nltgv2_ctx* ctx, float* err_out);

enum {
  FLAME_NLTGV2_OPT_SOLVER = 1,
  FLAME_NLTGV2_OPT_USE_HIPGRAPH = 2,
  FLAME_NLTGV2_OPT_PERSISTENT = 5,
  FLAME_NLTGV2_OPT_PROBE = 12,
  FLAME_NLTGV2_OPT_VERIFY_RECORDS = 14,
  FLAME_NLTGV2_OPT_PLACEMENT = 16,

  FLAME_NLTGV2_OPT_SYNC_PATH = 17,

  FLAME_NLTGV2_OPT_COST_SUM = 18,

  FLAME_NLTGV2_OPT_MESH_STATE = 19,

  FLAME_NLTGV2_OPT_EXPERIMENTAL = 100
};
int flame_nltgv2_set_option(flame_nltgv2_ctx* ctx, int option, int value);

typedef struct flame_nltgv2_info {
  int32_t abi_version;
  int32_t device;
  int32_t V, E;
  int32_t n_slices;
  int32_t max_degree;
  int64_t padded_half_edges;
  int64_t device_bytes;
  int64_t algorithmic_bytes_per_iter;
  int32_t compute_units;
  char device_name[64];
  char gcn_arch[32];
  int32_t last_run_path;
  int32_t he_waves;
  int32_t tv_waves;
  int32_t tv_wave_capacity;
  int32_t last_run_groups;
  int32_t timeouts_recovered;
  int32_t patches;
  int32_t torn_records_detected;
  int32_t last_sync_path;
  int32_t last_run_waves_per_cu;
  int32_t reserved0, reserved1;
  int32_t replays_per_step;
} flame_nltgv2_info;
int flame_nltgv2_get_info(flame_nltgv2_ctx* ctx, flame_nltgv2_info* info);

int flame_nltgv2_last_error(flame_nltgv2_ctx* ctx);
int flame_nltgv2_last_hip_error(flame_nltgv2_ctx* ctx);
const char* flame_nltgv2_status_string(int status);
int flame_nltgv2_abi_version(void);

int flame_nltgv2_read_probe(flame_nltgv2_ctx* ctx, uint32_t* out, int64_t max_words, int64_t* n_words);

int flame_nltgv2_placement_info(flame_nltgv2_ctx* ctx, int32_t* state, int32_t* placed_records, float* us);

int flame_nltgv2_layout_selftest(flame_nltgv2_ctx* ctx, int64_t* mismatches);
int flame_nltgv2_pack_probe(const flame_nltgv2_graph* g, int32_t* perm, int32_t* slice_row,
                            int32_t* rec_nbr, int32_t* rec_edge, int64_t capacity_rows, int64_t* rows_out);

#ifdef __cplusplus
}
#endif
#endif
```

Measured before the change: 1.087 million.

## Let a running persistent kernel take over the next queued run's iterations

Adds a take-over protocol so that a persistent solver kernel nearing the end of its run can read a host-posted descriptor for the next identical run and keep iterating, instead of exiting and relaunching. The next kernel checks a claim ring on entry and returns immediately when its predecessor has already claimed its work. The aim is to remove kernel launch, drain and refill gaps between back-to-back runs. In exchange it adds a device-side decision and poll point, extra ring memory and more complex correctness conditions. Stale-configuration detection relies on a checksum plus a config hash.

```diff
diff --git a/flame_amd/csrc/flame_nltgv2_test_options.h b/flame_amd/csrc/flame_nltgv2_test_options.h
--- a/flame_amd/csrc/flame_nltgv2_test_options.h
+++ b/flame_amd/csrc/flame_nltgv2_test_options.h
@@ -8,7 +8,8 @@
   FLAME_NLTGV2_OPT_PRESLEEP = 108,
   FLAME_NLTGV2_OPT_XCDS = 109,
   FLAME_NLTGV2_OPT_FAULT_INJECT = 110,
-  FLAME_NLTGV2_OPT_POLL_GAP = 113
+  FLAME_NLTGV2_OPT_POLL_GAP = 113,
+  FLAME_NLTGV2_OPT_TAKEOVER = 114
 };
 
 #endif
diff --git a/flame_amd/csrc/nltgv2_context.hip b/flame_amd/csrc/nltgv2_context.hip
--- a/flame_amd/csrc/nltgv2_context.hip
+++ b/flame_amd/csrc/nltgv2_context.hip
@@ -207,7 +207,7 @@
       {&ctx->bar0, sizeof(float4) * n_packed}, {&ctx->bar1, sizeof(float4) * n_packed},
       {&ctx->vprev, sizeof(float4) * n_packed}, {&ctx->xbuf, kXbufBytesPerVertex * records_capacity(L) + 64},
       {&ctx->wg_v0, sizeof(int32_t) * n_wg_v0},
-      {&ctx->wg_vfirst, n_wg_vfirst + 16}, {&ctx->abort_flag, sizeof(int)}, {&ctx->err, kErrBytes}, {&ctx->cost_out, 2 * sizeof(float)},
+      {&ctx->wg_vfirst, n_wg_vfirst + 16}, {&ctx->abort_flag, sizeof(int)}, {&ctx->err, kErrBytes + sizeof(unsigned) * kTkRingWords}, {&ctx->cost_out, 2 * sizeof(float)},
       {&ctx->wg_slot, sizeof(int32_t) * lanes}, {&ctx->wg_vid, sizeof(int32_t) * lanes}, {&ctx->wg_meta, sizeof(uint32_t) * lanes},
       {&ctx->wg_nbr, sizeof(int32_t) * lanes}, {&ctx->wg_fetch, sizeof(int32_t) * lanes},
       {&ctx->wg_info, sizeof(int32_t) * n_wg_info}};
@@ -473,7 +473,7 @@
   ok = ok && hipEventCreateWithFlags(&ctx->ev_expanded, hipEventDisableTiming) == hipSuccess;
   ok = ok && hipEventCreateWithFlags(&ctx->ev_run[0], hipEventDisableTiming) == hipSuccess;
   ok = ok && hipEventCreateWithFlags(&ctx->ev_run[1], hipEventDisableTiming) == hipSuccess;
-  ok = ok && hipHostMalloc((void**)&ctx->h_err, kErrBytes, hipHostMallocDefault) == hipSuccess;
+  ok = ok && hipHostMalloc((void**)&ctx->h_err, kErrBytes + 16, hipHostMallocDefault) == hipSuccess;
   ok = ok && hipHostMalloc((void**)&ctx->h_cost, 2 * sizeof(float), hipHostMallocDefault) == hipSuccess;
   ok = ok && hipHostMalloc((void**)&ctx->h_stop, 64, hipHostMallocDefault) == hipSuccess;
   if (ctx->h_stop) *ctx->h_stop = 0u;
@@ -594,6 +594,10 @@
       if (value < 0 || value > 1) return fail(ctx, FLAME_NLTGV2_ERR_INVALID_ARG);
       ctx->opt_place = value;
       return 0;
+    case FLAME_NLTGV2_OPT_TAKEOVER:
+      if (value < 0 || value > 1) return fail(ctx, FLAME_NLTGV2_ERR_INVALID_ARG);
+      ctx->opt_takeover = value;
+      return 0;
     case FLAME_NLTGV2_OPT_POLL_GAP:
       if (value < 0 || value > 256) return fail(ctx, FLAME_NLTGV2_ERR_INVALID_ARG);
       ctx->opt_poll_gap = value;
@@ -677,7 +681,7 @@
   info->torn_records_detected = ctx->torn_records_detected;
   info->last_sync_path = ctx->last_sync_path;
   info->last_run_waves_per_cu = ctx->last_run_waves_per_cu;
-  info->reserved0 = 0, info->reserved1 = 0;
+  info->runs_taken_over = ctx->runs_taken_over, info->reserved1 = 0;
   info->replays_per_step = ctx->replays_per_step;
   return FLAME_NLTGV2_OK;
 }
diff --git a/flame_amd/csrc/nltgv2_context.hpp b/flame_amd/csrc/nltgv2_context.hpp
--- a/flame_amd/csrc/nltgv2_context.hpp
+++ b/flame_amd/csrc/nltgv2_context.hpp
@@ -43,6 +43,7 @@
 constexpr int kDualMinWavesPerCu = 0;
 constexpr int kPreSleepTv = 2;
 constexpr int32_t kFeatDirectMax = 1 << 22;
+static_assert(kTkRingAtErrWord == 16u, "the take-over ring lies right behind the error block");
 constexpr size_t kErrBytes = 16 * sizeof(int);
 constexpr unsigned kMaxSpins = 1u << 20;
 
@@ -173,6 +174,16 @@
   int torn_records_detected = 0;
   int opt_verify = 0;
   int opt_place = 1;
+  int opt_takeover = 1;
+  unsigned* tk_ring_ready = nullptr;
+  uint32_t tk_seq = 0, tk_cfg = 0;
+  std::vector<unsigned char> tk_config;
+  bool tk_prev_valid = false, tk_prev_may = false;
+  uint64_t tk_prev_call = 0;
+  uint64_t tail_epoch = 0;
+  int tk_desc_pending = 0;
+  uint32_t tk_count_seen = 0;
+  int32_t runs_taken_over = 0;
   int place_state = 0;
   uint64_t place_topo = ~0ull;
   int place_per_xcd = 0;
diff --git a/flame_amd/csrc/nltgv2_kernels.h b/flame_amd/csrc/nltgv2_kernels.h
--- a/flame_amd/csrc/nltgv2_kernels.h
+++ b/flame_amd/csrc/nltgv2_kernels.h
@@ -40,6 +40,14 @@
   float t[3];
   float rx, ry, rw, rh;
 };
+
+constexpr unsigned kTkRingAtErrWord = 16u;
+constexpr unsigned kTkRingSlots = 512u, kTkDescWord0 = kTkRingSlots, kTkCountWord = 5u * kTkRingSlots, kTkRingWords = 5u * kTkRingSlots + 16u;
+constexpr unsigned kTkTakesPart = 1u, kTkMayTake = 2u, kTkContested = 4u, kTkCfgShift = 3u, kTkCfgMask = 511u, kTkSeqShift = 12u, kTkSeqMask = (1u << 20) - 1u;
+constexpr int kTkMinIters = 160;
+__host__ __device__ inline unsigned tk_check_word(const unsigned seq, const unsigned n, const unsigned cfg) {
+  return (seq * 0x9e3779b1u) ^ (n * 0x85ebca6bu) ^ (cfg * 0xc2b2ae35u) ^ 0x5bd1e995u;
+}
 
 struct CanonArgs {
   int V = 0, E = 0;
@@ -96,6 +104,7 @@
   int rec_off_stride = 0;
   unsigned* rot_word = nullptr;
   unsigned* probe = nullptr;
+  unsigned tk_word = 0;
   int* abort_flag = nullptr;
   int* err = nullptr;
 };
diff --git a/flame_amd/csrc/nltgv2_persistent.hip b/flame_amd/csrc/nltgv2_persistent.hip
--- a/flame_amd/csrc/nltgv2_persistent.hip
+++ b/flame_amd/csrc/nltgv2_persistent.hip
@@ -17,9 +17,19 @@
                 const unsigned max_spins_arg, const int poll_gap_arg, const SolverParams p,
                 int* __restrict__ err, int* __restrict__ abort_flag, const int32_t* __restrict__ perm,
                 const RunTail* __restrict__ tail, unsigned* __restrict__ probe, char* place_pool,
-                const int32_t* __restrict__ rec_off, const int rec_off_stride, unsigned* rot_word) {
+                const int32_t* __restrict__ rec_off, const int rec_off_stride, unsigned* rot_word,
+                const unsigned tk_word) {
   extern __shared__ float4 lds[];
   constexpr int T = 64;
+  constexpr bool kTakeOver = !PROBE && !VERIFY && !OPEN;
+  if (kTakeOver && (tk_word & kTkTakesPart)) {
+    if (tk_word & kTkContested) {
+      if (takeover_claimed(tk_ring_of(err), tk_word >> kTkSeqShift, (int)threadIdx.x)) return;
+    } else if (blockIdx.x == 0 && threadIdx.x == 0) {
+      __hip_atomic_store(tk_ring_of(err) + ((tk_word >> kTkSeqShift) & (kTkRingSlots - 1u)), ((tk_word >> kTkSeqShift) << 2) | kTkClaimSelf, __ATOMIC_RELAXED,
+                         __HIP_MEMORY_SCOPE_AGENT);
+    }
+  }
   const unsigned max_spins = max_spins_arg & 0x7fffffffu;
   const int dual = dual_arg & 1, verify = VERIFY ? dual_arg >> 1 : 0;
   const int poll_gap = poll_gap_arg & 255, pv_presleep = (poll_gap_arg >> 8) & 255;
@@ -151,6 +161,7 @@
       if (!timed_out && frid >= 0 && (g0 & 15u) == my_xcc) off0 += S, fetch_remote = false;
     }
   }
+  timed_out = __builtin_amdgcn_readfirstlane((int)timed_out) != 0;
   const unsigned long long fetch_mask = __ballot(frid >= 0);
   const bool mute = (max_spins_arg >> 31) != 0u && wg == wg_begin;
   const bool pub_lane = state_lane && publishes;
@@ -246,7 +257,7 @@
       rounds += cnt;
       if (__builtin_expect(pend_lo != 0u, 0)) {
         for (unsigned outer = 0;;) {
-          const int ab = __hip_atomic_load(abort_flag, __ATOMIC_RELAXED, __HIP_MEMORY_SCOPE_AGENT);
+          const int ab = __builtin_amdgcn_readfirstlane(__hip_atomic_load(abort_flag, __ATOMIC_RELAXED, __HIP_MEMORY_SCOPE_AGENT));
           if (ab != 0 || ++outer > (max_spins >> 4)) {
             timed_out = true;
             if (ab == 0) {
@@ -414,6 +425,9 @@
   char* const pubA = p0 ? pa1 : pa0;
   char* const pubB = p0 ? pa0 : pa1;
   int it = 0;
+  constexpr unsigned kTkStateMay = 1u << 30, kTkStateDecides = 1u << 31, kTkStateRuns = (1u << 30) - 1u;
+  int seg_end = n_iters;
+  unsigned tk_state = 3u;
   if (OPEN) {
     const bool decides = wg == wg_begin + n_wgs / 2;
     const unsigned* const stop_req = tail->stop_req;
@@ -428,17 +442,35 @@
     }
     if (decides && lane == 0 && !timed_out) reinterpret_cast<unsigned*>(err)[13] = tag0 + (unsigned)it;
   } else {
-    for (; it + 1 < n_iters && !timed_out; it += 2) {
-      step(tag0 + (unsigned)it, rdA_nbr, dstA, wrB_rec, areaA + lcap, it, srcA, pubB, wrA_rec);
-      if (timed_out) break;
-      step(tag0 + (unsigned)it + 1u, rdB_nbr, dstB, wrA_rec, areaB + lcap, it + 1, srcB, pubA, wrB_rec);
-    }
-    if (it < n_iters && !timed_out) step(tag0 + (unsigned)it, rdA_nbr, dstA, wrB_rec, areaA + lcap, it, srcA, pubB, wrA_rec);
+    if (kTakeOver && (tk_word & kTkMayTake) != 0u)
+      seg_end -= (int)kOpenMargin, tk_state = 2u | kTkStateMay | (wg == wg_begin + n_wgs / 2 ? kTkStateDecides : 0u);
+    for (;;) {
+      for (; it + 1 < seg_end && !timed_out; it += 2) {
+        step(tag0 + (unsigned)it, rdA_nbr, dstA, wrB_rec, areaA + lcap, it, srcA, pubB, wrA_rec);
+        if (timed_out) break;
+        step(tag0 + (unsigned)it + 1u, rdB_nbr, dstB, wrA_rec, areaB + lcap, it + 1, srcB, pubA, wrB_rec);
+      }
+      if (!kTakeOver || (tk_state & kTkStateMay) == 0u || timed_out) break;
+      if ((tk_state & 1u) == 0u) {
+        seg_end += (int)kOpenMargin, tk_state |= 1u;
+        if (tk_state & kTkStateDecides) takeover_decide(tk_word, (tk_state & kTkStateRuns) >> 1, err, tag0 + (unsigned)seg_end, lane);
+      } else {
+        unsigned n_next = 0u;
+        if (!takeover_read(n_next, err, tag0 + (unsigned)seg_end, max_spins)) {
+          timed_out = true;
+          break;
+        }
+        if (n_next == 0u) break;
+        seg_end += (int)n_next - (int)kOpenMargin, tk_state += 1u;
+      }
+    }
+    if (it < seg_end && !timed_out) step(tag0 + (unsigned)it, rdA_nbr, dstA, wrB_rec, areaA + lcap, it, srcA, pubB, wrA_rec);
   }
   asm volatile("s_waitcnt vmcnt(0)" ::: "memory");
 
   if (timed_out) {
     if (lane == 0) {
+      if (kTakeOver && (tk_state & kTkStateMay) != 0u && it >= seg_end) report_expired(err, 4, wg, it, 0ull, -1, 0u, tag0 + (unsigned)seg_end);
       give_up(abort_flag, err, torn);
       unsigned* const pg = tail->progress;
       if (pg) pg[wg - wg_begin] = 0x80000000u | (unsigned)(it + 1);
@@ -446,9 +478,16 @@
     return;
   }
 
-  if (state_lane) write_back_vertex(pv, x, w12, xb, wb12, x_prev, w_prev, data, vstate_out, bar_out, vprev, perm, tail);
-  if (active) hq_out[slot] = make_float4(q1, q23.x, q23.y, beta);
+  float4 *vs_o = vstate_out, *bar_o = bar_out, *hq_o = hq_out;
+  if (kTakeOver && (tk_state & 2u) == 0u) {
+    vs_o = const_cast<float4*>(vstate), bar_o = const_cast<float4*>(bar_in), hq_o = const_cast<float4*>(hq);
+    asm volatile("" : "+s"(vs_o), "+s"(bar_o), "+s"(hq_o));
+  }
+  if (state_lane) write_back_vertex(pv, x, w12, xb, wb12, x_prev, w_prev, data, vs_o, bar_o, vprev, perm, tail);
+  if (active) hq_o[slot] = make_float4(q1, q23.x, q23.y, beta);
   if (!ok && active) atomicOr(err, 1);
+  if (kTakeOver && (tk_state & kTkStateDecides) != 0u && (tk_state & kTkStateRuns) > 3u && lane == 0)
+    atomicAdd(tk_ring_of(err) + kTkCountWord, ((tk_state & kTkStateRuns) >> 1) - 1u);
 }
 
 }
@@ -514,10 +553,11 @@
     const int32_t* rec_off = a.rec_off;
     int rec_off_stride = a.rec_off_stride;
     unsigned* rot_word = place_pool ? a.rot_word : nullptr;
+    unsigned tk_word = (cooperative || probe || a.open_run || (dual >> 1) != 0) ? 0u : a.tk_word;
     const unsigned ldsv = pv_lds_bytes(lcap, slab_slots);
     void* vargs[] = {&wave_begin, &n_waves, &wgx, &lcap, &slab_slots, &w0, &w1, &w2, &w3, &w4, &w5, &hrec, &hq, &vstate,
                      &hq_out, &vstate_out, &vaux, &bin, &bout, &vprev, &xbuf, &rec_bytes, &dual, &tag0, &n_iters,
-                     &max_spins, &poll_gap, &pp, &err, &abort_flag, &perm, &tail, &probe, &place_pool, &rec_off, &rec_off_stride, &rot_word};
+                     &max_spins, &poll_gap, &pp, &err, &abort_flag, &perm, &tail, &probe, &place_pool, &rec_off, &rec_off_stride, &rot_word, &tk_word};
     const bool vr = (dual >> 1) != 0;
     if (!a.wg_rowpack) return (int)hipErrorInvalidConfiguration;
     const void* fv = probe ? (const void*)k_persistent_pv<true, true>
diff --git a/flame_amd/csrc/nltgv2_persistent_common.hpp b/flame_amd/csrc/nltgv2_persistent_common.hpp
--- a/flame_amd/csrc/nltgv2_persistent_common.hpp
+++ b/flame_amd/csrc/nltgv2_persistent_common.hpp
@@ -47,6 +47,61 @@
   if (stop_at == 0u) {
     const unsigned w = (unsigned)__builtin_amdgcn_readfirstlane((int)__hip_atomic_load(stop_word, __ATOMIC_RELAXED, __HIP_MEMORY_SCOPE_AGENT));
     if (w > tag0 && w - tag0 <= (unsigned)n_iters + kOpenMargin) stop_at = w;
+  }
+}
+
+constexpr unsigned kTkClaimSelf = 1u, kTkClaimPredecessor = 2u, kTkMaxRuns = 16u;
+static_assert(kTkMinIters >= (int)kOpenMargin + 2 && kTkMinIters % 2 == 0, "a run that takes part begins in front of its decision point, at an even iteration");
+__device__ __forceinline__ unsigned* tk_ring_of(int* const err) { return reinterpret_cast<unsigned*>(err) + kTkRingAtErrWord; }
+
+__device__ __forceinline__ bool takeover_claimed(unsigned* const ring, const unsigned seq, const int lane) {
+  unsigned* const claim = ring + (seq & (kTkRingSlots - 1u));
+  const unsigned mine = seq << 2;
+  unsigned c = (unsigned)__builtin_amdgcn_readfirstlane((int)__hip_atomic_load(claim, __ATOMIC_RELAXED, __HIP_MEMORY_SCOPE_AGENT));
+  if ((c & ~3u) != mine) {
+    unsigned old = c;
+    if (lane == 0) old = atomicCAS(claim, c, mine | kTkClaimSelf);
+    old = (unsigned)__builtin_amdgcn_readfirstlane((int)old);
+    c = old == c ? (mine | kTkClaimSelf) : old;
+  }
+  return c == (mine | kTkClaimPredecessor);
+}
+
+__device__ __forceinline__ void takeover_decide(const unsigned tk_word, const unsigned runs_done, int* err, const unsigned tag_bound,
+                                                const int lane) {
+  unsigned n_next = 0u;
+  asm volatile("" : "+s"(err));
+  if (runs_done < kTkMaxRuns) {
+    unsigned* const ring = tk_ring_of(err);
+    const unsigned seq_next = ((tk_word >> kTkSeqShift) + runs_done) & kTkSeqMask, cfg = (tk_word >> kTkCfgShift) & kTkCfgMask;
+    const unsigned slot = seq_next & (kTkRingSlots - 1u);
+    const unsigned* const d = ring + kTkDescWord0 + 4u * slot;
+    const unsigned s = (unsigned)__builtin_amdgcn_readfirstlane((int)__hip_atomic_load(d, __ATOMIC_RELAXED, __HIP_MEMORY_SCOPE_AGENT));
+    const unsigned n = (unsigned)__builtin_amdgcn_readfirstlane((int)__hip_atomic_load(d + 1, __ATOMIC_RELAXED, __HIP_MEMORY_SCOPE_AGENT));
+    const unsigned c = (unsigned)__builtin_amdgcn_readfirstlane((int)__hip_atomic_load(d + 2, __ATOMIC_RELAXED, __HIP_MEMORY_SCOPE_AGENT));
+    const unsigned k = (unsigned)__builtin_amdgcn_readfirstlane((int)__hip_atomic_load(d + 3, __ATOMIC_RELAXED, __HIP_MEMORY_SCOPE_AGENT));
+    if (s == seq_next && c == cfg && k == tk_check_word(s, n, c) && n >= (unsigned)kTkMinIters && (n & 1u) == 0u && n <= (1u << 24)) {
+      const unsigned was = (unsigned)__builtin_amdgcn_readfirstlane((int)__hip_atomic_load(ring + slot, __ATOMIC_RELAXED, __HIP_MEMORY_SCOPE_AGENT));
+      unsigned old = ~was;
+      if ((was & ~3u) != (seq_next << 2) && lane == 0) old = atomicCAS(ring + slot, was, (seq_next << 2) | kTkClaimPredecessor);
+      if ((unsigned)__builtin_amdgcn_readfirstlane((int)old) == was) n_next = n;
+    }
+  }
+  if (lane == 0)
+    __hip_atomic_store(reinterpret_cast<unsigned long long*>(err + 14), ((unsigned long long)tag_bound << 32) | n_next, __ATOMIC_RELAXED,
+                       __HIP_MEMORY_SCOPE_AGENT);
+}
+
+__device__ __forceinline__ bool takeover_read(unsigned& n_next, int* err, const unsigned tag_bound, const unsigned max_spins) {
+  asm volatile("" : "+s"(err));
+  for (unsigned spins = 0;; ++spins) {
+    const unsigned long long v = __hip_atomic_load(reinterpret_cast<unsigned long long*>(err + 14), __ATOMIC_RELAXED, __HIP_MEMORY_SCOPE_AGENT);
+    if ((unsigned)__builtin_amdgcn_readfirstlane((int)(unsigned)(v >> 32)) == tag_bound) {
+      n_next = (unsigned)__builtin_amdgcn_readfirstlane((int)(unsigned)v);
+      return true;
+    }
+    if (spins > max_spins) return false;
+    __builtin_amdgcn_s_sleep(2);
   }
 }
 
diff --git a/flame_amd/csrc/nltgv2_run.hip b/flame_amd/csrc/nltgv2_run.hip
--- a/flame_amd/csrc/nltgv2_run.hip
+++ b/flame_amd/csrc/nltgv2_run.hip
@@ -407,8 +407,17 @@
   return (form == 3 && groups[0].count <= 20 * cus) || (form == 4 && groups[0].count <= 14 * cus);
 }
 
+struct TkConfig {
+  SolverParams sp;
+  uint64_t topo, tail_epoch;
+  const void *place_pool, *rec_off, *rot_word, *tail;
+  int form, begin, count, xcds, dual, poll_gap, rec_off_stride, lcap, slab_slots;
+  unsigned spins;
+};
+
 int enqueue_run(flame_nltgv2_ctx* ctx, const flame_nltgv2_params* p, int n) {
   if (n <= 0) return 0;
+  bool clean = ctx->fused_valid;
   if (ctx->open_inflight) {
     const int rc0 = finish(ctx);
     if (rc0) return rc0;
@@ -432,6 +441,7 @@
   if (ctx->opt_mesh_state == 1 && ctx->canon_valid) {
     HIPCHK(ctx, hipEventRecord(ctx->ev_snap, ctx->stream));
     ctx->snap_topo = ctx->topo;
+    clean = false;
   }
   int rc = ensure_fused(ctx);
   if (rc) return rc;
@@ -439,6 +449,7 @@
     if (ctx->pending.ops.size() >= kMaxChain) {
       rc = finish(ctx);
     } else {
+      if (!ctx->pending.snapshotted) clean = false;
       rc = snapshot_chain_start(ctx);
     }
     if (rc) return rc;
@@ -461,14 +472,16 @@
         HIPCHK(ctx, hipMemsetAsync(ctx->place_base, 0, (size_t)2 * kPlacePages * 4096, ctx->stream));
         HIPCHK(ctx, hipMemsetAsync((int*)ctx->place_fill.p + 2 * kPlacePages, 0, 64, ctx->stream));
       }
-      HIPCHK(ctx, hipMemsetAsync((int*)ctx->err.p + 12, 0, 2 * sizeof(int), ctx->stream));
+      HIPCHK(ctx, hipMemsetAsync((int*)ctx->err.p + 12, 0, 4 * sizeof(int), ctx->stream));
       ctx->tag_next = 1;
+      clean = false;
     }
     ctx->xbuf_form = form;
     const uint32_t tag0 = ctx->tag_next + 2;
     const uint64_t key = ctx->topo * 1024 + (uint64_t)form * 64 + (ctx->opt_verify != 0 ? 16 : 0) + (ctx->opt_probe != 0 ? 8 : 0) +
                          (ctx->opt_dual == 2 ? 4 : ctx->opt_dual == 1 ? 2 : 0) + (ctx->opt_xcds > 0 ? 1 : 0);
     const RunTail* tail_dev = nullptr;
+    bool tail_plain = false;
     {
       RunTail want;
       std::memset(static_cast<void*>(&want), 0, sizeof want);
@@ -478,6 +491,7 @@
         rc = ensure(ctx, ctx->stop_dev, 64);
         if (rc) return rc;
         if (fresh) HIPCHK(ctx, hipMemsetAsync(ctx->stop_dev.p, 0, 64, ctx->stream));
+        clean = false;
         ctx->open_tag0 = tag0;
       }
       want.stop_req = open_run ? (const unsigned*)ctx->stop_dev.p : nullptr;
@@ -500,7 +514,9 @@
         HIPCHK(ctx, hipMemcpyAsync((char*)ctx->run_tail.p + kTailStride * (size_t)slot, &want, sizeof(RunTail), hipMemcpyHostToDevice, ctx->stream));
         ctx->tail_sent[slot] = want;
         ctx->tail_valid[slot] = true;
-      }
+        ++ctx->tail_epoch, clean = false;
+      }
+      tail_plain = !want.export_out && !want.photo.err && !want.progress && !want.stop_req;
       tail_dev = (const RunTail*)((const char*)ctx->run_tail.p + kTailStride * (size_t)slot);
     }
     int e = 0;
@@ -527,11 +543,13 @@
           if (ctx->place_state == 0) {
             rc = place_calibrate(ctx);
             if (rc) return rc;
+            clean = false;
           }
           const int per_xcd = (gr.count + xcds - 1) / xcds;
           if (ctx->place_state == 1 && (ctx->place_topo != ctx->topo || ctx->place_per_xcd != per_xcd)) {
             rc = place_records(ctx, per_xcd);
             if (rc) return rc;
+            clean = false;
           }
           if (ctx->place_state == 1) {
             ctx->f.place_pool = ctx->place_base, ctx->f.rec_off = (const int32_t*)ctx->place_rec_off.p;
@@ -560,11 +578,54 @@
         if (e != 0) break;
         continue;
       }
+      const bool cooperative = cooperative_allowed() && ctx->coop_checked_key != key;
+      const bool takes_part = form == 3 && ctx->opt_takeover != 0 && groups.size() == 1 && !cooperative && !open_run && ctx->want_open == 0 &&
+                              ctx->opt_probe == 0 && ctx->opt_verify == 0 && ctx->opt_fault == 0 && ctx->replaying == 0 && ctx->ctl_stream != nullptr;
+      bool desc_sent = false, may_take = false;
+      const uint32_t tk_seq = (ctx->tk_seq + 1) & kTkSeqMask;
+      ctx->f.tk_word = 0;
+      if (takes_part) {
+        unsigned* const ring = (unsigned*)ctx->err.p + kTkRingAtErrWord;
+        if (ctx->tk_ring_ready != ring) {
+          HIPCHK(ctx, hipMemsetAsync(ring, 0, sizeof(unsigned) * kTkRingWords, ctx->stream));
+          ctx->tk_ring_ready = ring, ctx->tk_count_seen = 0;
+          clean = false;
+        }
+        TkConfig cfg;
+        std::memset(static_cast<void*>(&cfg), 0, sizeof cfg);
+        cfg.sp = to_sp(p), cfg.topo = ctx->topo, cfg.tail_epoch = ctx->tail_epoch;
+        cfg.place_pool = ctx->f.place_pool, cfg.rec_off = ctx->f.rec_off, cfg.rot_word = ctx->f.rot_word, cfg.tail = tail_dev;
+        cfg.form = form, cfg.begin = gr.begin, cfg.count = gr.count, cfg.xcds = xcds, cfg.dual = dual, cfg.poll_gap = ctx->f.wg_poll_gap;
+        cfg.rec_off_stride = ctx->f.rec_off_stride, cfg.lcap = ctx->f.wg_lcap, cfg.slab_slots = ctx->f.wg_slab_slots, cfg.spins = spins_arg;
+        if (ctx->tk_config.size() != sizeof cfg || std::memcmp(ctx->tk_config.data(), &cfg, sizeof cfg) != 0) {
+          ctx->tk_config.assign(reinterpret_cast<const unsigned char*>(&cfg), reinterpret_cast<const unsigned char*>(&cfg) + sizeof cfg);
+          ctx->tk_cfg = (ctx->tk_cfg + 1) & kTkCfgMask;
+        }
+        const bool sized = (n & 1) == 0 && n >= kTkMinIters && tail_plain;
+        const bool behind_prev = ctx->tk_prev_valid && ctx->tk_prev_call + 1 == ctx->call_seq && ctx->tk_prev_may && ctx->pending.active;
+        may_take = sized && ctx->pending.active && ctx->pending.snapshotted && ctx->pending.ops.size() + 2 < kMaxChain;
+        if (sized && clean && behind_prev) {
+          const unsigned d[4] = {tk_seq, (unsigned)n, ctx->tk_cfg, tk_check_word(tk_seq, (unsigned)n, ctx->tk_cfg)};
+          HIPCHK(ctx, hipMemcpyAsync(ring + kTkDescWord0 + 4u * (tk_seq & (kTkRingSlots - 1u)), d, sizeof d, hipMemcpyHostToDevice, ctx->ctl_stream));
+          desc_sent = true;
+          ++ctx->tk_desc_pending;
+        }
+        ctx->f.tk_word = kTkTakesPart | (may_take ? kTkMayTake : 0u) | (desc_sent ? kTkContested : 0u) | (ctx->tk_cfg << kTkCfgShift) | (tk_seq << kTkSeqShift);
+      }
       ctx->f.open_run = open_run ? 1 : 0;
       e = launch_persistent_run(ctx->f, to_sp(p), form, gr.begin, gr.count, ctx->parity, tag0, n, pw, spins_arg, presleep, dual,
-                                xcds, tail_dev, cooperative_allowed() && ctx->coop_checked_key != key, ctx->stream);
+                                xcds, tail_dev, cooperative, ctx->stream);
       ctx->f.open_run = 0;
+      ctx->f.tk_word = 0;
+      ctx->tk_prev_valid = false;
+      if (e != 0 && desc_sent) {
+        (void)hipGetLastError();
+        ctx->last_hip = e;
+        ctx->have_graph = false;
+        return fail(ctx, FLAME_NLTGV2_ERR_HIP);
+      }
       if (e != 0) break;
+      if (takes_part) ctx->tk_seq = tk_seq, ctx->tk_prev_valid = true, ctx->tk_prev_call = ctx->call_seq, ctx->tk_prev_may = may_take;
     }
     ctx->run_event_bound = e == 0 && ctx->f.stop_event != nullptr;
     ctx->f.stop_event = nullptr;
@@ -642,9 +703,9 @@
 
 void trace_expired_wait(flame_nltgv2_ctx* ctx) {
   const int* e = ctx->h_err;
-  static const char* const kWhich[] = {"?", "rotation word", "XCC table", "step records"};
+  static const char* const kWhich[] = {"?", "rotation word", "XCC table", "step records", "take-over decision"};
   std::fprintf(stderr, "[flame_nltgv2] persistent run taken back (flags %d): first expired wait = %s, patch %d, step %d, lanes waiting %08x%08x, "
-               "first of them for record %d (tag seen %u, wanted %u), on XCC %d hw_id %08x\n", e[0], kWhich[e[1] & 3], e[2], e[3], (unsigned)e[5],
+               "first of them for record %d (tag seen %u, wanted %u), on XCC %d hw_id %08x\n", e[0], kWhich[(e[1] >= 1 && e[1] <= 4) ? e[1] : 0], e[2], e[3], (unsigned)e[5],
                (unsigned)e[4], e[6], (unsigned)e[7], (unsigned)e[8], e[9], (unsigned)e[10]);
   if (!ctx->progress.p || ctx->L.wg_count <= 0) return;
   std::vector<unsigned> pg((size_t)2 * ctx->L.wg_count);
@@ -686,6 +747,9 @@
     ctx->open_inflight = false, ctx->open_stop_sent = false;
   }
   HIPCHK(ctx, hipMemcpyAsync(ctx->h_err, ctx->err.p, kErrBytes, hipMemcpyDeviceToHost, ctx->stream));
+  const bool tk_count = ctx->tk_desc_pending > 0 && ctx->tk_ring_ready;
+  if (tk_count)
+    HIPCHK(ctx, hipMemcpyAsync(ctx->h_err + kErrBytes / sizeof(int), ctx->tk_ring_ready + kTkCountWord, sizeof(unsigned), hipMemcpyDeviceToHost, ctx->stream));
   bool behind = false;
   if (unpack_behind && ctx->pending.active && !ctx->canon_valid && !ctx->replaying) {
     const int rc = wait_raster(ctx);
@@ -699,6 +763,12 @@
     }
   }
   HIPCHK(ctx, wait_solver_stream(ctx));
+  if (tk_count) {
+    const uint32_t seen = (uint32_t)ctx->h_err[kErrBytes / sizeof(int)];
+    ctx->runs_taken_over += (int32_t)(seen - ctx->tk_count_seen);
+    ctx->tk_count_seen = seen, ctx->tk_desc_pending = 0;
+  }
+  ctx->tk_prev_valid = false;
   flame_nltgv2_ctx::PendingRun run;
   std::swap(run, ctx->pending);
   if (open_run && !run.ops.empty() && run.ops.back().open) {
diff --git a/flame_amd/regularizer.py b/flame_amd/regularizer.py
--- a/flame_amd/regularizer.py
+++ b/flame_amd/regularizer.py
@@ -12,7 +12,7 @@
 _IP = C.POINTER(C.c_int32)
 
 OPT_SOLVER, OPT_USE_HIPGRAPH, OPT_PERSISTENT, OPT_PROBE, OPT_VERIFY_RECORDS, OPT_PLACEMENT, OPT_SYNC_PATH, OPT_COST_SUM, OPT_MESH_STATE = 1, 2, 5, 12, 14, 16, 17, 18, 19
-OPT_BLOCK_WAVES, OPT_UNROLL, OPT_DUAL_PUBLISH, OPT_PRESLEEP, OPT_XCDS, OPT_FAULT_INJECT, OPT_POLL_GAP = 103, 104, 106, 108, 109, 110, 113
+OPT_BLOCK_WAVES, OPT_UNROLL, OPT_DUAL_PUBLISH, OPT_PRESLEEP, OPT_XCDS, OPT_FAULT_INJECT, OPT_POLL_GAP, OPT_TAKEOVER = 103, 104, 106, 108, 109, 110, 113, 114
 RUN_PATHS = {0: "none", 1: "persistent (the lane-per-half-edge form, retired in round 3)", 2: "per-step hipGraph", 3: "per-step eager", 4: "canonical 4-sweep",
              5: "persistent-tv", 6: "persistent-pv", 7: "persistent-pv2"}
 ERR_NAN = -5
@@ -103,7 +103,7 @@
         ("device_name", C.c_char * 64), ("gcn_arch", C.c_char * 32), ("last_run_path", C.c_int32), ("he_waves", C.c_int32), ("tv_waves", C.c_int32),
         ("tv_wave_capacity", C.c_int32), ("last_run_groups", C.c_int32), ("timeouts_recovered", C.c_int32),
         ("patches", C.c_int32), ("torn_records_detected", C.c_int32), ("last_sync_path", C.c_int32),
-        ("last_run_waves_per_cu", C.c_int32), ("reserved0", C.c_int32), ("reserved1", C.c_int32), ("replays_per_step", C.c_int32),
+        ("last_run_waves_per_cu", C.c_int32), ("runs_taken_over", C.c_int32), ("reserved1", C.c_int32), ("replays_per_step", C.c_int32),
     ]
 
 
diff --git a/include/flame_nltgv2.h b/include/flame_nltgv2.h
--- a/include/flame_nltgv2.h
+++ b/include/flame_nltgv2.h
@@ -232,7 +232,8 @@
   int32_t torn_records_detected;
   int32_t last_sync_path;
   int32_t last_run_waves_per_cu;
-  int32_t reserved0, reserved1;
+  int32_t runs_taken_over;
+  int32_t reserved1;
   int32_t replays_per_step;
 } flame_nltgv2_info;
 int flame_nltgv2_get_info(flame_nltgv2_ctx* ctx, flame_nltgv2_info* info);
```

Result: no change. 1.086 million (-0.1%).
